# brdav/refign

Hardware: AMD Instinct MI355X
Metric: image-pairs/s (align+seg fwd+bwd, 1080x1920) (higher is better)
Workload: dtype bf16

## Files before the change

include/refign_hip.h:

```cpp
#ifndef REFIGN_HIP_H
#define REFIGN_HIP_H

#ifdef __cplusplus
extern "C" {
#endif

#define RFN_OK 0
#define RFN_EINVAL (-1)
#define RFN_ELAUNCH (-2)
#define RFN_ENOTSUP (-3)
#define RFN_ENONDET (-4)

#define RFN_ABI_VERSION 4

typedef void* rfn_stream_t;

int rfn_abi_version(void);
const char* rfn_last_error(void);

int rfn_set_deterministic(int on);
int rfn_get_deterministic(void);

int rfn_corr_fwd_f32(const float* in1, const float* in2, float* out, int B, int C, int iH, int iW,
                     int kH, int kW, int patchH, int patchW, int padH, int padW, int dilH, int dilW,
// ... 7 lines not shown
                     rfn_stream_t stream);
int rfn_corr_bwd_f64(const double* in1, const double* in2, const double* grad_out, double* grad_in1,
                     double* grad_in2, int B, int C, int iH, int iW, int kH, int kW, int patchH, int patchW,
                     int padH, int padW, int dilH, int dilW, int dpH, int dpW, int dH, int dW,
                     rfn_stream_t stream);

int rfn_corr_fwd_f16(const void* in1, const void* in2, void* out, int B, int C, int iH, int iW,
                     int kH, int kW, int patchH, int patchW, int padH, int padW, int dilH, int dilW,
                     int dpH, int dpW, int dH, int dW, rfn_stream_t stream);
int rfn_corr_bwd_f16(const void* in1, const void* in2, const void* grad_out, void* grad_in1,
                     void* grad_in2, int B, int C, int iH, int iW, int kH, int kW, int patchH, int patchW,
                     int padH, int padW, int dilH, int dilW, int dpH, int dpW, int dH, int dW,
                     rfn_stream_t stream);

int rfn_local_corr_layer_f32(const float* feature_target, const float* feature_source, const float* flow,
                             float* out, int B, int C, int H, int W, rfn_stream_t stream);

long rfn_local_corr_layer_split_workspace_bytes(int B, int H, int W, int splits);
int rfn_local_corr_layer_split_f32(const float* feature_target, const float* feature_source, float* out,
                                   float* workspace, int B, int C, int H, int W, int splits, rfn_stream_t stream);

int rfn_global_corr_layer_f32(const float* feature_source, const float* feature_target, float* out,
                              float* workspace, int B, int C, int Hs, int Ws, int Ht, int Wt,
                              int cyclic_consistency, rfn_stream_t stream);

int rfn_warp_f32(const float* x, const float* flow, float* out, unsigned char* mask, int B, int C, int H,
                 int W, rfn_stream_t stream);
int rfn_warp_bwd_f32(const float* x, const float* flow, const float* grad_out, float* grad_x, float* grad_flow, int B,
                     int C, int H, int W, rfn_stream_t stream);

int rfn_area_resize_f32(const float* x, float* out, int planes, int H, int W, int OH, int OW, rfn_stream_t stream);

int rfn_l2norm_channels_f32(const float* x, float* out, int B, int C, int HW, rfn_stream_t stream);

int rfn_l2norm_channels_nhwc16_f32(const void* x, float* out, int B, int C, int HW, int dtype, rfn_stream_t stream);
int rfn_maxpool2x2_nhwc16(const void* x, void* y, int B, int H, int W, int C, int dtype, rfn_stream_t stream);
int rfn_retile_copy(const void* src, void* dst, int B, int h, int w, int k, int units16, int src_stride16, int backward,
                    rfn_stream_t stream);

unsigned long rfn_refine_workspace_bytes(int B);
int rfn_refine_f32(const float* logits_trg, const float* logits_ref, const unsigned char* warp_mask,
                   const float* certs, float* out, void* workspace, int B, int C, int H, int W, float gamma,
                   int flags, rfn_stream_t stream);

int rfn_label_majority(const long* gt, long* out, int B, int H, int W, int scale, int n_classes, int ignore_index,
                       float min_ratio, rfn_stream_t stream);

int rfn_align_tail_f32(const float* logits_ref, const float* flow_q, const float* logvar_q, float* warped,
                       unsigned char* mask, float* cert, float* flow_up, int B, int C, int H, int W, int h,
                       int w, rfn_stream_t stream);

int rfn_dwconv3x3_nhwc_fwd(const void* x, const float* weight, const float* bias, void* y, int B, int H, int W,
                           int C, int dilation, int dtype, int flip, rfn_stream_t stream);
int rfn_dwconv3x3_nhwc_fwd_stats(const void* x, const float* weight, const float* bias, void* y, double* sums, int B, int H,
                                 int W, int C, int dilation, int dtype, rfn_stream_t stream);
int rfn_dwconv3x3_nhwc_stats(const void* x, const float* weight, const float* bias, double* sums, int B, int H, int W, int C,
                             int dilation, int dtype, rfn_stream_t stream);
int rfn_dwconv3x3_bn_act_nhwc_fwd(const void* x, const float* weight, const float* bias, const float* gamma, const float* beta,
                                  const double* sums, float* running_mean, float* running_var, void* y, int B, int H, int W,
                                  int C, int dilation, float eps, float momentum, int relu, int dtype, rfn_stream_t stream);

int rfn_dwconv3x3_tri_usable(int B, int H, int W, int C, int g);
int rfn_dwconv3x3_tri_stats(const void* x, const float* weight3, const float* bias3, double* sums3, int B, int H, int W, int C, int g,
                            rfn_stream_t stream);
int rfn_dwconv3x3_tri_bn_act_fwd(const void* x, const float* weight3, const float* bias3, const float* const* gamma3,
                                 const float* const* beta3, const double* sums3, float* const* running_mean3,
                                 float* const* running_var3, void* const* y3, int B, int H, int W, int C, int g, const float* eps3,
                                 const float* momentum3, int relu, rfn_stream_t stream);
int rfn_dwconv3x3_tri_stats_f16(const void* x, const float* weight3, const float* bias3, double* sums3, int B, int H, int W, int C,
                                int g, rfn_stream_t stream);
int rfn_dwconv3x3_tri_bn_act_fwd_f16(const void* x, const float* weight3, const float* bias3, const float* const* gamma3,
                                     const float* const* beta3, const double* sums3, float* const* running_mean3,
                                     float* const* running_var3, void* const* y3, int B, int H, int W, int C, int g, const float* eps3,
                                     const float* momentum3, int relu, rfn_stream_t stream);
int rfn_dwconv3x3_gelu_nhwc_fwd(const void* x, const float* weight, const float* bias, void* y_pre, void* y_act, int B,
                                int H, int W, int C, int dtype, rfn_stream_t stream);
unsigned long rfn_dwconv3x3_bwd_weight_workspace_bytes(int C);
int rfn_dwconv3x3_nhwc_bwd_weight(const void* x, const void* grad_y, float* grad_weight, float* grad_bias,
                                  void* workspace, int B, int H, int W, int C, int dilation, int dtype, int flags,
                                  rfn_stream_t stream);
int rfn_dwconv3x3_nhwc_bwd(const void* x, const void* grad_y, const float* weight_tap_major, void* grad_x, float* grad_weight,
                           float* grad_bias, void* workspace, int B, int H, int W, int C, int dilation, int dtype, int flags,
                           rfn_stream_t stream);

int rfn_layernorm_fwd(const void* x, const float* gamma, const float* beta, void* y, float* mean, float* rstd,
                      long rows, int C, float eps, int in_dtype, int out_dtype, rfn_stream_t stream);
unsigned long rfn_layernorm_bwd_workspace_bytes(int C);
int rfn_layernorm_bwd(const void* x, const void* grad_y, const float* gamma, const float* mean, const float* rstd,
                      void* grad_x, float* grad_gamma, float* grad_beta, void* workspace, long rows, int C,
                      int x_dtype, int gy_dtype, int accumulate, rfn_stream_t stream);
int rfn_layernorm_bwd_add(const void* x, const void* grad_y, const void* add, const float* gamma, const float* mean,
                          const float* rstd, void* grad_x, float* grad_gamma, float* grad_beta, void* workspace, long rows, int C,
                          int x_dtype, int gy_dtype, int accumulate, rfn_stream_t stream);
int rfn_layernorm_bwd_add2(const void* x, const void* grad_y, const void* grad_y2, const void* add, const float* gamma,
                           const float* mean, const float* rstd, void* grad_x, float* grad_gamma, float* grad_beta, void* workspace,
                           long rows, int C, int x_dtype, int gy_dtype, int accumulate, rfn_stream_t stream);

int rfn_uncertainty9_weights_len(void);
int rfn_uncertainty9_frontend_f32(const float* corr, const float* weights, float* out, int B, int H, int W,
                                  rfn_stream_t stream);
int rfn_uncertainty9_frontend_f16mm(const float* corr, const float* weights, float* out, int B, int H, int W,
                                    rfn_stream_t stream);

unsigned long rfn_sum_rows_workspace_bytes(long S, long n);
int rfn_sum_rows(const void* x, float* out, void* workspace, long S, long n, int x_dtype, int accumulate,
                 rfn_stream_t stream);
int rfn_linear_param_grads(const void* grad_y, float* grad_bias, void* workspace, long T, long N, int acc_bias,
                           const void* w_partials, float* grad_weight, int S, long NK, int acc_weight, int dtype,
                           rfn_stream_t stream);

int rfn_multi_cast_chunk_elems(void);
int rfn_multi_permute_chunk_elems(void);
int rfn_multi_permute_cast_f32(const void* table, int nchunks, rfn_stream_t stream);
int rfn_multi_cast_f32_bf16(const void* table, int nchunks, rfn_stream_t stream);
int rfn_multi_cast_f32_f16(const void* table, int nchunks, rfn_stream_t stream);
int rfn_multi_ema_f32(const void* table, int nchunks, float momentum, rfn_stream_t stream);
int rfn_multi_transpose_cast_f32_bf16(const void* table, int ntiles, rfn_stream_t stream);
int rfn_multi_transpose_cast_f32_f16(const void* table, int ntiles, rfn_stream_t stream);
int rfn_multi_transpose_tile(void);
int rfn_multi_adamw_f32(const void* table, int nchunks, const float* group_args, int ngroups, rfn_stream_t stream);
int rfn_amp_unscale_f32(float* grads, long n, const float* scale, float* found_inf, rfn_stream_t stream);
int rfn_multi_adamw_amp_f32(const void* table, int nchunks, const double* group_args, int ngroups, const float* found_inf,
                            const float* step, rfn_stream_t stream);
int rfn_amp_update_scale(float* scale, int* growth_tracker, const float* found_inf, float* step, float growth_factor,
                         float backoff_factor, int growth_interval, rfn_stream_t stream);

int rfn_upsample_concat_nhwc(const void* src0, const void* src1, const void* src2, const void* src3, const int* hs,
                             const int* ws, const int* cs, int nlev, void* out, int n, int H, int W, int dtype,
                             rfn_stream_t stream);
int rfn_upsample_concat_nhwc_bwd(const void* grad_out, void* grad0, void* grad1, void* grad2, void* grad3, const int* hs,
                                 const int* ws, const int* cs, int nlev, int n, int H, int W, int dtype,
                                 rfn_stream_t stream);

int rfn_patchify_tokens(const void* src, void* dst, int B, int H, int W, int C, int r, int dtype, int inverse,
                        rfn_stream_t stream);

int rfn_patchify_tokens_cmajor(const void* src, void* dst, int B, int H, int W, int C, int r, int dtype, int inverse,
                               rfn_stream_t stream);

int rfn_gemm_nt(const void* X, const void* W, const void* bias, const void* res, const float* rowscale,
                int rows_per_sample, int act, void* Y, long M, long N, long K, long ldx, long ldw, long ldy, int dtype,
                rfn_stream_t stream);
int rfn_conv2d_nhwc(const void* X, const void* W, const void* bias, const void* res, int act, void* Y, int B, int H,
                    int Wd, int C, int N, int KH, int KW, int stride, int pad, int dil, long ldw, long ldy, int dtype,
                    rfn_stream_t stream);
int rfn_gemm_tn(const void* G, const void* X, float* P, long T, long N, long K, long ldg, long ldx, int rows_per_slab,
                int accumulate, float* grad_bias, const float* rowscale, int rows_per_sample, int dtype,
                rfn_stream_t stream);
int rfn_gemm_tn_grouped(int count, const void* const* G, const void* const* X, float* const* P, float* const* grad_bias,
                        const float* const* rowscale, const long* T, const long* N, const long* K, const long* ldg,
                        const long* ldx, const int* rows_per_slab, const int* rows_per_sample, int dtype, rfn_stream_t stream);

int rfn_attn_pack(const void* src, long batch_stride, long row_stride, int B, int heads, int nrows, int nblk, void* rpack,
                  void* tpack, const void* src2, void* rpack2, void* tpack2, rfn_stream_t stream);
int rfn_attn_fwd(const void* Q, long q_batch_stride, long q_row_stride, const void* k_rpack, const void* v_tpack, void* O,
                 long o_batch_stride, long o_row_stride, float* lse2, int B, int heads, int Nq, int Nkv, int nkblk,
                 int nqpad, float scale, int kv_pack_heads, int dtype, rfn_stream_t stream);
int rfn_attn_bwd_dq(const void* Q, long q_batch_stride, long q_row_stride, const void* dO, const void* O,
                    long o_batch_stride, long o_row_stride, const void* k_rpack, const void* v_rpack, const void* k_tpack,
                    const float* lse2, float* delta, void* dQ, long dq_batch_stride, long dq_row_stride, int B, int heads,
                    int Nq, int Nkv, int nkblk, int nqpad, float scale, int kv_pack_heads, int dtype,
                    rfn_stream_t stream);
int rfn_attn_bwd_dkv(const void* K, const void* V, long kv_batch_stride, long kv_row_stride, const void* q_rpack,
                     const void* q_tpack, const void* do_rpack, const void* do_tpack, const float* lse2,
                     const float* delta, float* accT, void* dKV, int B, int heads, int Nq, int Nkv, int nqblk, int nqpad,
                     int nkpad, int blocks_per_chunk, float scale, int dtype, rfn_stream_t stream);

int rfn_attn32_fwd(const float* Q, long q_batch_stride, long q_row_stride, const float* KV, long kv_batch_stride,
                   long kv_row_stride, float* O, long o_batch_stride, long o_row_stride, float* lse2, int B, int heads,
                   int head_dim, int Nq, int Nkv, int nqpad, float scale, rfn_stream_t stream);
int rfn_attn32_bwd(const float* Q, long q_batch_stride, long q_row_stride, const float* KV, long kv_batch_stride,
                   long kv_row_stride, const float* dO, const float* O, long o_batch_stride, long o_row_stride,
                   const float* lse2, float* delta, float* dQ, long dq_batch_stride, long dq_row_stride, float* dKV,
                   long dkv_batch_stride, long dkv_row_stride, int B, int heads, int head_dim, int Nq, int Nkv, int nqpad,
                   int query_chunks, float scale, rfn_stream_t stream);

int rfn_split3_bf16(const float* x, long x_row_stride, void* out, long out_row_stride, long term_stride, long rows, int K,
                    int Kp, int order, rfn_stream_t stream);
int rfn_split3_cat_bf16(const float* const* parts, const long* strides, const int* channels, int nparts, void* out, int B, int H,
                        int W, int Cp, rfn_stream_t stream);

int rfn_ffn_fc1_dw_gelu_bf16(const void* x, const void* w1, const void* b1, const float* wdw_tap, const float* bdw, void* a,
                             int views, int H, int W, int C, int HID, rfn_stream_t stream);
int rfn_ffn_fc1_dw_gelu_f16(const void* x, const void* w1, const void* b1, const float* wdw_tap, const float* bdw, void* a,
                            int views, int H, int W, int C, int HID, rfn_stream_t stream);

int rfn_bn_stats_fwd(const void* x, double* sums, long T, int C, int dtype, rfn_stream_t stream);
int rfn_bn_apply_fwd(const void* x, const float* gamma, const float* beta, void* y, const double* sums, float* running_mean,
                     float* running_var, long T, int C, float eps, float momentum, int relu, int dtype, rfn_stream_t stream);
int rfn_bn_apply_fwd_ld(const void* x, const float* gamma, const float* beta, void* y, long ld_y, const double* sums,
                        float* running_mean, float* running_var, long T, int C, float eps, float momentum, int relu, int dtype,
                        rfn_stream_t stream);
int rfn_bn_stats_bwd(const void* x, const void* grad_y, const double* fwd_sums, const float* gamma, const float* beta,
                     float* bwd_sums, long T, int C, float eps, int relu, int dtype, rfn_stream_t stream);
int rfn_bn_apply_bwd(const void* x, const void* grad_y, const double* fwd_sums, const float* bwd_sums, const float* gamma,
                     const float* beta, void* grad_x, long T, int C, float eps, int relu, int dtype, rfn_stream_t stream);
int rfn_bn_train_fwd(const void* x, const float* gamma, const float* beta, void* y, double* sums, float* running_mean,
                     float* running_var, long T, int C, float eps, float momentum, int relu, int dtype,
                     rfn_stream_t stream);
int rfn_bn_train_bwd(const void* x, const void* grad_y, const double* fwd_sums, const float* gamma, const float* beta,
                     void* grad_x, float* bwd_sums, long T, int C, float eps, int relu, int dtype, rfn_stream_t stream);

int rfn_upsample_ce(const void* logits, const long* target, const float* weight, float* grad_lo, double* loss_sum, int B,
                    int C, int h, int w, int H, int W, int ignore_index, int dtype, int round16, rfn_stream_t stream);

int rfn_slide_argmax_confmat(const void* crop_logits, int dtype, int B, int C, int h, int w, const int* boxes, int nbox, int H,
                             int W, const long* target, int ignore_index, unsigned char* labels, long* confmat,
                             rfn_stream_t stream);

int rfn_gemm_nt_o32(const void* X, const void* W, const float* bias, const float* res, const float* rowscale,
                    int rows_per_sample, int act, float* Y, long M, long N, long K, long ldx, long ldw, long ldy,
                    rfn_stream_t stream);
int rfn_conv2d_nhwc_o32(const void* X, const void* W, const float* bias, int act, float* Y, int B, int H, int Wd, int C, int N,
                        int KH, int KW, int stride, int pad, int dil, long ldw, long ldy, int transposed,
                        rfn_stream_t stream);
int rfn_conv2d_nhwc_dgrad(const void* GY, const void* Wt, void* DX, int B, int H, int W, int C, int N, int KH, int KW,
                          int stride, int pad, int dil, long ldw, long ldy, int dtype, rfn_stream_t stream);
int rfn_conv2d_nhwc_wgrad(const void* GY, const void* X, float* P, float* grad_bias, int B, int H, int W, int C, int N, int KH,
                          int KW, int stride, int pad, int dil, long ldg, long Kpad, int rows_per_slab, int accumulate,
                          int dtype, rfn_stream_t stream);

int rfn_dacs_mix_jitter(const float* src, const float* trg, const long* gt_src, const long* pseudo_label,
                        const float* pseudo_weight, float* mixed_img, long* mixed_lbl, float* mixed_weight, double* mean_ws,
                        int B, int H, int W, const long* class_bits, const int* jitter_on, const int* order,
                        const float* factor, const float* hue, const float* mean3, const float* std3,
                        rfn_stream_t stream);
int rfn_dacs_blur(const float* x, float* tmp, float* y, int B, int C, int H, int W, int ksize_y, int ksize_x, const int* blur_on,
                  const double* sigma_y, const double* sigma_x, rfn_stream_t stream);

int rfn_crop_label_hist_u8(const void* label, int H, int W, const int* boxes, int K, int* hist, rfn_stream_t stream);
int rfn_crop_flip_norm_u8(const void* image, const void* label, int C, int H, int W, int top, int left, int h, int w, int flip,
                          const float* mean3, const float* std3, float* out_image, long* out_label, rfn_stream_t stream);

int rfn_resize_crop_flip_norm_u8(const void* image_hwc, int H, int W, int Hd, int Wd, const int* bounds_x, const int* coef_x, int kmax_x,
                                 const int* bounds_y, const int* coef_y, int kmax_y, int top, int left, int h, int w, int flip,
                                 const float* mean3, const float* std3, float* out_image, rfn_stream_t stream);
int rfn_resize_u8(const void* image_hwc, int H, int W, int Hd, int Wd, const int* bounds_x, const int* coef_x, int kmax_x,
                  const int* bounds_y, const int* coef_y, int kmax_y, void* out_chw, rfn_stream_t stream);
int rfn_resize_nearest_u8(const void* label, int H, int W, int Hd, int Wd, const int* ytab, const int* xtab, void* out,
                          rfn_stream_t stream);

int rfn_resize_filter_u8(const void* image_hwc, int H, int W, int Hd, int Wd, int filter, const int* bounds_x, const int* coef_x,
                         int kmax_x, const int* bounds_y, const int* coef_y, int kmax_y, void* out_chw, rfn_stream_t stream);
int rfn_resize_filter_crop_flip_norm_pad_u8(const void* image_hwc, int H, int W, int Hd, int Wd, int filter, const int* bounds_x,
                                            const int* coef_x, int kmax_x, const int* bounds_y, const int* coef_y, int kmax_y, int top,
                                            int left, int h, int w, int flip, const float* mean3, const float* std3, float* out_image,
                                            int Hf, int Wf, rfn_stream_t stream);

int rfn_sparse_epe_f32(const float* flow, const float* conf, const float* pts_src, const float* pts_trg, const int* offsets, int B,
// ... 69 lines not shown
```

refign_amd/csrc/attn.hip:

```cpp
#include <cstdlib>

#include "common.h"
#include "mfma.h"

namespace rfn {

constexpr int kPackBlock = 4096;
constexpr float kLog2e = 1.4426950408889634f;

__global__ __launch_bounds__(256) void attn_pack_kernel(const uint16_t* __restrict__ src0, const uint16_t* __restrict__ src1,
                                                        long sb, long sr, int heads, int nrows, int nblk,
                                                        unsigned char* __restrict__ rpack0, unsigned char* __restrict__ tpack0,
                                                        unsigned char* __restrict__ rpack1, unsigned char* __restrict__ tpack1) {
  __shared__ unsigned tile[32][33];
  const uint16_t* src = blockIdx.z ? src1 : src0;
  unsigned char* rpack = blockIdx.z ? rpack1 : rpack0;
  unsigned char* tpack = blockIdx.z ? tpack1 : tpack0;
  const int blk = blockIdx.x, bh = blockIdx.y;
  const int b = bh / heads, hd = bh % heads;
  const int t = threadIdx.x, row = t >> 3, dc = t & 7;
  const int grow = blk * 32 + row;
  u32x4 v = {0u, 0u, 0u, 0u};
  if (grow < nrows) v = *(const u32x4*)(src + (long)b * sb + (long)grow * sr + hd * 64 + dc * 8);
  unsigned char* rb = rpack + ((long)bh * nblk + blk) * kPackBlock;
  if (rpack != nullptr) *(u32x4*)(rb + (dc * 32 + row) * 16) = v;
  if (tpack == nullptr) return;
  tile[row][dc * 4 + 0] = v[0];
  tile[row][dc * 4 + 1] = v[1];
  tile[row][dc * 4 + 2] = v[2];
  tile[row][dc * 4 + 3] = v[3];
  __syncthreads();
  const int rq = t >> 5, dp = t & 31;
  unsigned r0 = tile[4 * rq + 0][dp], r1 = tile[4 * rq + 1][dp], r2 = tile[4 * rq + 2][dp], r3 = tile[4 * rq + 3][dp];
  u32x4 o;
  o[0] = (r0 & 0xffffu) | (r1 << 16);
  o[1] = (r2 & 0xffffu) | (r3 << 16);
  o[2] = (r0 >> 16) | (r1 & 0xffff0000u);
  o[3] = (r2 >> 16) | (r3 & 0xffff0000u);
  unsigned char* tb = tpack + ((long)bh * nblk + blk) * kPackBlock;
  *(u32x4*)(tb + (rq * 64 + 2 * dp) * 8) = o;
}

template <int DT>
__device__ __forceinline__ void load_row_frags(const uint16_t* base, long row_stride, int row, int nrows, int g,
                                               typename Elem<DT>::vec8 (&f)[4]) {
  const bool ok = row < nrows;
  const uint16_t* p = base + (long)(ok ? row : 0) * row_stride + 8 * g;
#pragma unroll
  for (int ks = 0; ks < 4; ++ks) {
    u32x4 v = {0u, 0u, 0u, 0u};
    if (ok) v = *(const u32x4*)(p + 16 * ks);
    f[ks] = __builtin_bit_cast(typename Elem<DT>::vec8, v);
  }
}

template <int DT>
__device__ __forceinline__ void store_rows64(const f32x16 (&acc)[2], float mul, uint16_t* rowptr, bool ok, int g) {
#pragma unroll
  for (int db = 0; db < 2; ++db) {
    u32x2 pk[4];
#pragma unroll
    for (int k = 0; k < 4; ++k)
      pk[k] = pack4<DT>(acc[db][4 * k] * mul, acc[db][4 * k + 1] * mul, acc[db][4 * k + 2] * mul, acc[db][4 * k + 3] * mul);
#pragma unroll
    for (int p = 0; p < 2; ++p) {
      auto r0 = __builtin_amdgcn_permlane32_swap(pk[2 * p][0], pk[2 * p + 1][0], false, false);
      auto r1 = __builtin_amdgcn_permlane32_swap(pk[2 * p][1], pk[2 * p + 1][1], false, false);
      if (ok) {
        u32x4 o = {r0[0], r1[0], r0[1], r1[1]};
        *(u32x4*)(rowptr + db * 32 + 16 * p + 8 * g) = o;
      }
    }
  }
}

template <int DT>
__device__ __forceinline__ void to_operands(const float (&p)[16], typename Elem<DT>::vec8 (&b)[2]) {
#pragma unroll
  for (int m = 0; m < 2; ++m)
    b[m] = join8<DT>(pack4<DT>(p[8 * m], p[8 * m + 1], p[8 * m + 2], p[8 * m + 3]),
                     pack4<DT>(p[8 * m + 4], p[8 * m + 5], p[8 * m + 6], p[8 * m + 7]));
}

template <int DT>
__global__ __launch_bounds__(256) void attn_fwd_kernel(const uint16_t* __restrict__ Q, long qsb, long qsr,
                                                       const unsigned char* __restrict__ Kr,
                                                       const unsigned char* __restrict__ Vt, uint16_t* __restrict__ O,
                                                       long osb, long osr, float* __restrict__ lse2, int heads, int Nq,
                                                       int Nkv, int nblk, int nqpad, float scale, int pheads) {
  using E = Elem<DT>;
  using vec8 = typename E::vec8;
  constexpr int STAGE = 4 * kPackBlock;
  __shared__ __attribute__((aligned(16))) unsigned char smem[2 * STAGE];
  const int lane = threadIdx.x & 63, wave = threadIdx.x >> 6, g = lane >> 5, col = lane & 31;
  const int bh = blockIdx.y, b = bh / heads, hd = bh % heads;
  const int q = blockIdx.x * 128 + wave * 32 + col;
  const float c = scale * kLog2e;
// ... 346 lines not shown
        return join8<DT>(*(const u32x2*)(pq + (4 * m + g) * 512), *(const u32x2*)(pq + (4 * m + 2 + g) * 512));
      };
#pragma unroll
      for (int idx = 0; idx < 4; ++idx) tf[idx] = tfrag(idx);
      __builtin_amdgcn_sched_barrier(0);
      float p[16], ds[16];
#pragma unroll
      for (int r = 0; r < 16; ++r) {
        float pr = __builtin_amdgcn_exp2f(__builtin_fmaf(s[r], c, -l4[r >> 2][r & 3]));
        if (!kok) pr = 0.f;
        p[r] = pr;
        ds[r] = pr * (dp[r] - d4[r >> 2][r & 3]);
      }
      vec8 pb[2], sb[2];
      to_operands<DT>(p, pb);
      to_operands<DT>(ds, sb);
#pragma unroll
      for (int idx = 0; idx < 8; ++idx) {
        const int m = idx >> 2, db = (idx >> 1) & 1;
        if (idx & 1) dk[db] = E::mma(tf[idx & 3], sb[m], dk[db]);
        else dv[db] = E::mma(tf[idx & 3], pb[m], dv[db]);
        if (idx + 4 < 8) tf[idx & 3] = tfrag(idx + 4);
        __builtin_amdgcn_sched_barrier(0);
      }
    }
  }
  if (kok) {
    float* ak = accT + (long)blockIdx.y * chunk_stride + (long)bh * 2 * 64 * nkpad + key;
    float* av = ak + (long)64 * nkpad;
#pragma unroll
    for (int db = 0; db < 2; ++db)
#pragma unroll
      for (int r = 0; r < 16; ++r) {
        const int d = db * 32 + (r & 3) + 8 * (r >> 2) + 4 * g;
        if (chunk_stride != 0) {
          ak[(long)d * nkpad] = dk[db][r] * scale;
          av[(long)d * nkpad] = dv[db][r];
        } else {
          atomicAdd(ak + (long)d * nkpad, dk[db][r] * scale);
          atomicAdd(av + (long)d * nkpad, dv[db][r]);
        }
      }
  }
}

template <int DT>
__global__ __launch_bounds__(256) void attn_dkv_finish_kernel(const float* __restrict__ accT, uint16_t* __restrict__ dkv,
                                                              int heads, int Nkv, int nkpad, long total, int chunks = 1,
                                                              long chunk_stride = 0) {
  using S = typename Elem<DT>::scalar;
  const long i = (long)blockIdx.x * 256 + threadIdx.x;
  if (i >= total) return;
  const int d = (int)(i & 63);
  long r = i >> 6;
  const int hd = (int)(r % heads);
  r /= heads;
  const int which = (int)(r & 1);
  r >>= 1;
  const int key = (int)(r % Nkv);
  const int b = (int)(r / Nkv);
  const float* p = accT + (((long)(b * heads + hd) * 2 + which) * 64 + d) * nkpad + key;
  float v = p[0];
  for (int c = 1; c < chunks; ++c) v += p[(long)c * chunk_stride];
  const S o = (S)v;
  dkv[i] = __builtin_bit_cast(uint16_t, o);
}

}

extern "C" {

using namespace rfn;

#define ATTN_DT_OK(dt) RFN_REQUIRE((dt) == 1 || (dt) == 2, "attention: dtype %d (1 = bf16, 2 = f16)", (dt))

int rfn_attn_pack(const void* src, long batch_stride, long row_stride, int B, int heads, int nrows, int nblk, void* rpack,
                  void* tpack, const void* src2, void* rpack2, void* tpack2, rfn_stream_t stream) {
  RFN_REQUIRE(src && (rpack || tpack), "attn_pack: null pointer");
  RFN_REQUIRE(src2 == nullptr || rpack2 || tpack2, "attn_pack: second tensor without outputs");
  RFN_REQUIRE(B > 0 && heads > 0 && nrows > 0 && nblk * 32 >= nrows, "attn_pack: B=%d heads=%d rows=%d nblk=%d", B, heads,
              nrows, nblk);
  RFN_REQUIRE(row_stride % 8 == 0 && batch_stride % 8 == 0, "attn_pack: strides must be multiples of 8 elements");
  dim3 grid(nblk, B * heads, src2 ? 2 : 1);
  hipLaunchKernelGGL(attn_pack_kernel, grid, dim3(256), 0, (hipStream_t)stream, (const uint16_t*)src,
                     (const uint16_t*)src2, batch_stride, row_stride, heads, nrows, nblk, (unsigned char*)rpack,
                     (unsigned char*)tpack, (unsigned char*)rpack2, (unsigned char*)tpack2);
  return check_launch("attn_pack");
}

int rfn_attn_fwd(const void* Q, long q_batch_stride, long q_row_stride, const void* k_rpack, const void* v_tpack, void* O,
                 long o_batch_stride, long o_row_stride, float* lse2, int B, int heads, int Nq, int Nkv, int nkblk,
                 int nqpad, float scale, int kv_pack_heads, int dtype, rfn_stream_t stream) {
  ATTN_DT_OK(dtype);
  RFN_REQUIRE(Q && k_rpack && v_tpack && O && lse2, "attn_fwd: null pointer");
  RFN_REQUIRE(B > 0 && heads > 0 && Nq > 0 && Nkv > 0 && nkblk % 2 == 0 && nkblk * 32 >= Nkv && nqpad >= Nq,
              "attn_fwd: B=%d heads=%d Nq=%d Nkv=%d nkblk=%d nqpad=%d", B, heads, Nq, Nkv, nkblk, nqpad);
  RFN_REQUIRE(q_row_stride % 8 == 0 && o_row_stride % 8 == 0 && q_batch_stride % 8 == 0 && o_batch_stride % 8 == 0,
              "attn_fwd: strides must be multiples of 8 elements");
  RFN_REQUIRE(kv_pack_heads >= heads, "attn_fwd: kv_pack_heads");
  dim3 grid(cdiv(Nq, 128), B * heads);
  if (dtype == 1)
    hipLaunchKernelGGL(attn_fwd_kernel<1>, grid, dim3(256), 0, (hipStream_t)stream, (const uint16_t*)Q, q_batch_stride,
                       q_row_stride, (const unsigned char*)k_rpack, (const unsigned char*)v_tpack, (uint16_t*)O,
                       o_batch_stride, o_row_stride, lse2, heads, Nq, Nkv, nkblk, nqpad, scale, kv_pack_heads);
  else
    hipLaunchKernelGGL(attn_fwd_kernel<2>, grid, dim3(256), 0, (hipStream_t)stream, (const uint16_t*)Q, q_batch_stride,
                       q_row_stride, (const unsigned char*)k_rpack, (const unsigned char*)v_tpack, (uint16_t*)O,
                       o_batch_stride, o_row_stride, lse2, heads, Nq, Nkv, nkblk, nqpad, scale, kv_pack_heads);
  return check_launch("attn_fwd");
}

int rfn_attn_bwd_dq(const void* Q, long q_batch_stride, long q_row_stride, const void* dO, const void* O,
                    long o_batch_stride, long o_row_stride, const void* k_rpack, const void* v_rpack, const void* k_tpack,
                    const float* lse2, float* delta, void* dQ, long dq_batch_stride, long dq_row_stride, int B, int heads,
                    int Nq, int Nkv, int nkblk, int nqpad, float scale, int kv_pack_heads, int dtype,
                    rfn_stream_t stream) {
  ATTN_DT_OK(dtype);
  RFN_REQUIRE(Q && dO && O && k_rpack && v_rpack && k_tpack && lse2 && delta && dQ, "attn_bwd_dq: null pointer");
  RFN_REQUIRE(B > 0 && heads > 0 && Nq > 0 && Nkv > 0 && nkblk % 2 == 0 && nkblk * 32 >= Nkv && nqpad >= Nq,
              "attn_bwd_dq: B=%d heads=%d Nq=%d Nkv=%d nkblk=%d nqpad=%d", B, heads, Nq, Nkv, nkblk, nqpad);
  dim3 grid(cdiv(Nq, 128), B * heads);
#define RFN_DQ_LAUNCH(D)                                                                                                \
  hipLaunchKernelGGL(attn_bwd_dq_kernel<D>, grid, dim3(256), 0, (hipStream_t)stream, (const uint16_t*)Q, q_batch_stride, \
                     q_row_stride, (const uint16_t*)dO, (const uint16_t*)O, o_batch_stride, o_row_stride,               \
                     (const unsigned char*)k_rpack, (const unsigned char*)v_rpack, (const unsigned char*)k_tpack, lse2,  \
                     delta, (uint16_t*)dQ, dq_batch_stride, dq_row_stride, heads, Nq, Nkv, nkblk, nqpad, scale,          \
                     kv_pack_heads)
  if (dtype == 1) RFN_DQ_LAUNCH(1); else RFN_DQ_LAUNCH(2);
#undef RFN_DQ_LAUNCH
  return check_launch("attn_bwd_dq");
}

static int attn_bwd_dkv_impl(bool det, const void* K, const void* V, long kv_batch_stride, long kv_row_stride, const void* q_rpack,
                             const void* q_tpack, const void* do_rpack, const void* do_tpack, const float* lse2,
                             const float* delta, float* accT, void* dKV, int B, int heads, int Nq, int Nkv, int nqblk, int nqpad,
                             int nkpad, int blocks_per_chunk, float scale, int dtype, rfn_stream_t stream) {
  ATTN_DT_OK(dtype);
  RFN_REQUIRE(K && V && q_rpack && q_tpack && do_rpack && do_tpack && lse2 && delta && accT && dKV,
              "attn_bwd_dkv: null pointer");
  RFN_REQUIRE(B > 0 && heads > 0 && Nq > 0 && Nkv > 0 && nqblk * 32 >= Nq && nqpad >= nqblk * 32 && nkpad >= Nkv &&
                  nkpad % 32 == 0 && blocks_per_chunk > 0,
              "attn_bwd_dkv: B=%d heads=%d Nq=%d Nkv=%d nqblk=%d nqpad=%d nkpad=%d chunk=%d", B, heads, Nq, Nkv, nqblk,
              nqpad, nkpad, blocks_per_chunk);
  hipStream_t s = (hipStream_t)stream;
  const long image = (long)B * heads * 2 * 64 * nkpad, chunk_stride = det ? image : 0;
  if (!det)
    if (int rc = zero_async(accT, (size_t)image * sizeof(float), s)) return rc;
  dim3 grid(cdiv(Nkv, 256), cdiv(nqblk, blocks_per_chunk), B * heads);
  const int chunks = det ? (int)grid.y : 1;
  static const int ring = 2;
#define RFN_DKV_LAUNCH_(D, R)                                                                                           \
  hipLaunchKernelGGL((attn_bwd_dkv_kernel<D, R>), grid, dim3(512), 0, s, (const uint16_t*)K, (const uint16_t*)V,            \
                     kv_batch_stride, kv_row_stride, (const unsigned char*)q_rpack, (const unsigned char*)q_tpack,      \
                     (const unsigned char*)do_rpack, (const unsigned char*)do_tpack, lse2, delta, accT, heads, Nq, Nkv,  \
                     nqblk, nqpad, nkpad, blocks_per_chunk, scale, chunk_stride)
#define RFN_DKV_LAUNCH(D)                                                                                               \
  switch (ring) {                                                                                                       \
    case 4: RFN_DKV_LAUNCH_(D, 4); break;                                                                               \
    default: RFN_DKV_LAUNCH_(D, 2); break;                                                                              \
  }
  if (dtype == 1) { RFN_DKV_LAUNCH(1) } else { RFN_DKV_LAUNCH(2) }
#undef RFN_DKV_LAUNCH
#undef RFN_DKV_LAUNCH_
  int rc = check_launch("attn_bwd_dkv");
  if (rc != RFN_OK) return rc;
  const long total = (long)B * Nkv * 2 * heads * 64;
  if (dtype == 1)
    hipLaunchKernelGGL(attn_dkv_finish_kernel<1>, dim3(cdiv(total, 256)), dim3(256), 0, s, accT, (uint16_t*)dKV, heads,
                       Nkv, nkpad, total, chunks, chunk_stride);
  else
    hipLaunchKernelGGL(attn_dkv_finish_kernel<2>, dim3(cdiv(total, 256)), dim3(256), 0, s, accT, (uint16_t*)dKV, heads,
                       Nkv, nkpad, total, chunks, chunk_stride);
  return check_launch("attn_dkv_finish");
}

int rfn_attn_bwd_dkv(const void* K, const void* V, long kv_batch_stride, long kv_row_stride, const void* q_rpack,
                     const void* q_tpack, const void* do_rpack, const void* do_tpack, const float* lse2,
                     const float* delta, float* accT, void* dKV, int B, int heads, int Nq, int Nkv, int nqblk, int nqpad,
                     int nkpad, int blocks_per_chunk, float scale, int dtype, rfn_stream_t stream) {
  RFN_REFUSE_NONDET(true, "rfn_attn_bwd_dkv", "attn_bwd_dkv_kernel, fp32 atomics (use rfn_attn_bwd_dkv_det)");
  return attn_bwd_dkv_impl(false, K, V, kv_batch_stride, kv_row_stride, q_rpack, q_tpack, do_rpack, do_tpack, lse2, delta, accT,
                           dKV, B, heads, Nq, Nkv, nqblk, nqpad, nkpad, blocks_per_chunk, scale, dtype, stream);
}

int rfn_attn_bwd_dkv_det(const void* K, const void* V, long kv_batch_stride, long kv_row_stride, const void* q_rpack,
                         const void* q_tpack, const void* do_rpack, const void* do_tpack, const float* lse2,
                         const float* delta, float* accT, void* dKV, int B, int heads, int Nq, int Nkv, int nqblk, int nqpad,
                         int nkpad, int blocks_per_chunk, float scale, int dtype, rfn_stream_t stream) {
  return attn_bwd_dkv_impl(true, K, V, kv_batch_stride, kv_row_stride, q_rpack, q_tpack, do_rpack, do_tpack, lse2, delta, accT,
                           dKV, B, heads, Nq, Nkv, nqblk, nqpad, nkpad, blocks_per_chunk, scale, dtype, stream);
}

}
```

refign_amd/csrc/dwconv.hip:

```cpp
#include <hip/hip_bf16.h>

#include <type_traits>

#include "common.h"
#include "mfma.h"

namespace rfn {

template <typename T>
struct VecIO;

template <>
struct VecIO<float> {
  static constexpr int N = 4;
  typedef float4 Raw;
  __device__ static Raw load_raw(const float* p) { return *reinterpret_cast<const float4*>(p); }
  __device__ static void unpack(const Raw& t, float (&v)[4]) { v[0] = t.x; v[1] = t.y; v[2] = t.z; v[3] = t.w; }
  typedef float Pair __attribute__((ext_vector_type(2)));
  __device__ static void unpack2(const Raw& t, Pair (&v)[2]) { v[0] = Pair{t.x, t.y}; v[1] = Pair{t.z, t.w}; }
  __device__ static void load(const float* p, float (&v)[4]) {
    const float4 t = *reinterpret_cast<const float4*>(p);
    v[0] = t.x; v[1] = t.y; v[2] = t.z; v[3] = t.w;
  }
  __device__ static void store(float* p, const float (&v)[4]) {
    *reinterpret_cast<float4*>(p) = make_float4(v[0], v[1], v[2], v[3]);
  }
  __device__ static float rnd(float v) { return v; }
};

template <>
struct VecIO<__hip_bfloat16> {
  static constexpr int N = 8;
  typedef uint4 Raw;
  __device__ static Raw load_raw(const __hip_bfloat16* p) { return *reinterpret_cast<const uint4*>(p); }
  __device__ static void unpack(const Raw& t, float (&v)[8]) {
    const unsigned w[4] = {t.x, t.y, t.z, t.w};
#pragma unroll
    for (int i = 0; i < 4; ++i) {
      v[2 * i] = __uint_as_float(w[i] << 16);
      v[2 * i + 1] = __uint_as_float(w[i] & 0xffff0000u);
    }
  }
  typedef float Pair __attribute__((ext_vector_type(2)));
  __device__ static void unpack2(const Raw& t, Pair (&v)[4]) {
    const unsigned w[4] = {t.x, t.y, t.z, t.w};
#pragma unroll
    for (int i = 0; i < 4; ++i) v[i] = Pair{__uint_as_float(w[i] << 16), __uint_as_float(w[i] & 0xffff0000u)};
  }
  __device__ static void load(const __hip_bfloat16* p, float (&v)[8]) {
    const uint4 t = *reinterpret_cast<const uint4*>(p);
    const unsigned w[4] = {t.x, t.y, t.z, t.w};
#pragma unroll
    for (int i = 0; i < 4; ++i) {
      v[2 * i] = __uint_as_float(w[i] << 16);
      v[2 * i + 1] = __uint_as_float(w[i] & 0xffff0000u);
    }
  }
  __device__ static unsigned pack(float lo, float hi) { return bf16x2_bits(lo, hi); }
  __device__ static void store(__hip_bfloat16* p, const float (&v)[8]) {
    uint4 t;
    t.x = pack(v[0], v[1]); t.y = pack(v[2], v[3]); t.z = pack(v[4], v[5]); t.w = pack(v[6], v[7]);
    *reinterpret_cast<uint4*>(p) = t;
  }
  __device__ static float rnd(float v) { return __uint_as_float(bf16_bits(v) << 16); }
};

template <>
struct VecIO<_Float16> {
  static constexpr int N = 8;
  typedef uint4 Raw;
  __device__ static Raw load_raw(const _Float16* p) { return *reinterpret_cast<const uint4*>(p); }
  __device__ static void unpack(const Raw& t, float (&v)[8]) {
    const unsigned w[4] = {t.x, t.y, t.z, t.w};
#pragma unroll
    for (int i = 0; i < 4; ++i) {
      v[2 * i] = f16_lo(w[i]);
      v[2 * i + 1] = f16_hi(w[i]);
    }
  }
  typedef float Pair __attribute__((ext_vector_type(2)));
  __device__ static void unpack2(const Raw& t, Pair (&v)[4]) {
    const unsigned w[4] = {t.x, t.y, t.z, t.w};
#pragma unroll
    for (int i = 0; i < 4; ++i) v[i] = Pair{f16_lo(w[i]), f16_hi(w[i])};
  }
  __device__ static void load(const _Float16* p, float (&v)[8]) { unpack(load_raw(p), v); }
// ... 497 lines not shown
      for (int p = 0; p < kPX; ++p)
        xraw[p] = mask_raw(IO::load_raw(xp + (size_t)min(w0 + p * dil, W - 1) * C), w0 + p * dil < W);
#pragma unroll
      for (int p = 0; p < kPX; ++p) IO::unpack2(xraw[p], xv[p]);
    }
    f32x2 acc[GX ? kPX : 1][V2];
    if constexpr (GX) {
#pragma unroll
      for (int p = 0; p < kPX; ++p)
#pragma unroll
        for (int i = 0; i < V2; ++i) acc[p][i] = f32x2{0.0f, 0.0f};
    }
#pragma unroll
    for (int ky = 0; ky < 3; ++ky) {
      const int yy = h + (ky - 1) * dil;
      const bool rowok = yy >= 0 && yy < H;
      const T* gr = gy + img + (size_t)min(max(yy, 0), H - 1) * W * C;
      typename IO::Raw raw[kPX + 2];
#pragma unroll
      for (int j = 0; j < kPX + 2; ++j) {
        const int xx = w0 + (j - 1) * dil;
        raw[j] = mask_raw(IO::load_raw(gr + (size_t)min(max(xx, 0), W - 1) * C), rowok && xx >= 0 && xx < W);
      }
#pragma unroll
      for (int j = 0; j < kPX + 2; ++j) {
        f32x2 v[V2];
        IO::unpack2(raw[j], v);
        if (ky == 1 && j >= 1 && j <= kPX) {
#pragma unroll
          for (int i = 0; i < V2; ++i) ab[i] += v[i];
        }
#pragma unroll
        for (int kx = 0; kx < 3; ++kx) {
          const int p = j - kx;
          if (p < 0 || p >= kPX) continue;
#pragma unroll
          for (int i = 0; i < V2; ++i) {
            if constexpr (GX) acc[p][i] = __builtin_elementwise_fma(wr[ky * 3 + kx][i], v[i], acc[p][i]);
            aw[ky * 3 + kx][i] = __builtin_elementwise_fma(xv[p][i], v[i], aw[ky * 3 + kx][i]);
          }
        }
      }
    }
    if constexpr (GX) {
      T* gp = gx + img + (size_t)h * W * C;
#pragma unroll
      for (int p = 0; p < kPX; ++p)
        if (w0 + p * dil < W) {
          float o[V];
#pragma unroll
          for (int i = 0; i < V2; ++i) { o[2 * i] = acc[p][i].x; o[2 * i + 1] = acc[p][i].y; }
          IO::store(gp + (size_t)(w0 + p * dil) * C, o);
        }
    }
  }
  __shared__ float red[5][256][V];
  float* wrow = ws + (size_t)wsrow * 10 * C;
  for (int pass = 0; pass < 2; ++pass) {
    __syncthreads();
#pragma unroll
    for (int kk = 0; kk < 5; ++kk) {
      const int k = pass * 5 + kk;
#pragma unroll
      for (int i = 0; i < V; ++i) {
        const f32x2 t = (k < 9) ? aw[k < 9 ? 8 - k : 0][i / 2] : ab[i / 2];
        red[kk][threadIdx.x][i] = (i & 1) ? t.y : t.x;
      }
    }
    __syncthreads();
    for (int o = threadIdx.x; o < 5 * cvb * V; o += 256) {
      const int kk = o / (cvb * V), rem = o - kk * cvb * V, cvj = rem / V, i = rem - cvj * V;
      if (cvbase + cvj >= CV) continue;
      float sum = 0.0f;
      for (int p = 0; p < pl; ++p) sum += red[kk][p * cvb + cvj][i];
      wrow[(size_t)(pass * 5 + kk) * C + (cvbase + cvj) * V + i] = sum;
    }
  }
}

__global__ __launch_bounds__(256) void dwconv3x3_bwd_weight_reduce_kernel(const float* __restrict__ ws,
                                                                          float* __restrict__ dw,
                                                                          float* __restrict__ db, int C, int stripes,
                                                                          int flags) {
  __shared__ float part[8][32];
  const int lane = threadIdx.x & 31, seg = threadIdx.x >> 5;
  const int idx = blockIdx.x * 32 + lane;
  float s = 0.0f;
  if (idx < 10 * C) {
#pragma unroll 4
    for (int t = seg; t < stripes; t += 8) s += ws[(size_t)t * 10 * C + idx];
  }
  part[seg][lane] = s;
  __syncthreads();
  if (seg != 0 || idx >= 10 * C) return;
  s = ((part[0][lane] + part[1][lane]) + (part[2][lane] + part[3][lane])) +
      ((part[4][lane] + part[5][lane]) + (part[6][lane] + part[7][lane]));
  float* dst;
  if (idx < 9 * C) {
    const int k = idx / C, c = idx - k * C;
    dst = (flags & 2) ? dw + c * 9 + k : dw + idx;
  } else {
    if (db == nullptr) return;
    dst = db + (idx - 9 * C);
  }
  *dst = (flags & 1) ? *dst + s : s;
}

static inline int pick_cvb(int CV) { return CV >= 64 ? 64 : (CV >= 32 ? 32 : (CV >= 16 ? 16 : 8)); }

struct SlicedGeom {
  bool on;
  int cvb, grid;
};
static inline SlicedGeom sliced_geom(int CV, long nslots) {
  static const int enabled = 1;
  static const int per_xcd = 64;
  if (!enabled || CV % 8 != 0 || CV / 8 < 16 || CV / 8 > 64) return SlicedGeom{false, 0, 0};
  const int cvb = CV / 8, pl = 256 / cvb;
  const int j = (int)std::max<long>(1, std::min<long>(cdiv(nslots, pl), per_xcd));
  return SlicedGeom{true, cvb, 8 * j};
}
constexpr int kMaxStripes = 128;

template <typename T>
static int launch_fwd_gelu(const void* x, const float* w, const float* bias, void* y, void* ya, int B, int H, int W,
                           int C, hipStream_t st, float xs = 1.f, float oq = 1.f) {
  constexpr int V = VecIO<T>::N;
  const int CV = C / V;
  const long nquads = (long)B * H * ((W + kPX - 1) / kPX);
  if (SlicedGeom sg = sliced_geom(CV, nquads); sg.on) {
    hipLaunchKernelGGL((dwconv3x3_fwd_kernel<T, false, true>), dim3(sg.grid), dim3(256), 0, st, (const T*)x, w, bias,
                       (T*)y, B, H, W, C, 1, sg.cvb, (T*)ya, xs, oq, 1);
    return check_launch("dwconv3x3_fwd_kernel<gelu, sliced>");
  }
  const int cvb = pick_cvb(CV), gx = cdiv(CV, cvb), pl = 256 / cvb;
  const int gy = (int)std::max<long>(1, std::min<long>(cdiv(nquads, pl), (256L * 16) / gx));
  hipLaunchKernelGGL((dwconv3x3_fwd_kernel<T, false, true>), dim3(gx, gy), dim3(256), 0, st, (const T*)x, w, bias,
                     (T*)y, B, H, W, C, 1, cvb, (T*)ya, xs, oq);
  return check_launch("dwconv3x3_fwd_kernel<gelu>");
}

struct RollGeom {
  bool sliced;
  int cvb, gx, gy, seg, rows;
  long nitems;
};
static RollGeom roll_geom(int B, int H, int W, int C, int dil) {
  RollGeom g{};
  const int CV = C / kRV, Hd = cdiv(H, dil);
  const int WQ = dil * cdiv(cdiv(W, dil), kPX);
  const SlicedGeom sg = sliced_geom(C / 8, 1L << 30);
  int pl;
  long lanes;
  if (sg.on) {
    g.sliced = true, g.cvb = 2 * sg.cvb, pl = 256 / g.cvb;
    lanes = (long)(sg.grid / 8) * pl;
  } else {
    g.cvb = pick_cvb(CV), g.gx = cdiv(CV, g.cvb), pl = 256 / g.cvb;
    lanes = (256L * 16) / g.gx * pl;
  }
  const long per_seg = (long)B * dil * WQ;
  const long want = std::max<long>(1, cdiv(4 * lanes, per_seg));
  g.seg = (int)std::min<long>(Hd, std::max<long>(8, cdiv(Hd, want)));
  g.nitems = per_seg * cdiv(Hd, g.seg);
  if (sg.on) {
    g.rows = (int)std::max<long>(1, std::min<long>(cdiv(g.nitems, pl), sg.grid / 8));
    g.gx = 8 * g.rows, g.gy = 1;
  } else {
    g.rows = g.gy = (int)std::max<long>(1, std::min<long>(cdiv(g.nitems, pl), (256L * 16) / g.gx));
  }
  return g;
}

template <typename T, int STATS, bool BNE>
static int launch_roll(const void* x, const float* w, const float* bias, void* y, double* sums, int B, int H, int W, int C,
                       int dil, hipStream_t st, BnEpi bn, double* spart) {
  static void* zero_line = nullptr;
  if (zero_line == nullptr && hipGetSymbolAddress(&zero_line, HIP_SYMBOL(g_zero_line_dw)) != hipSuccess)
    return fail(RFN_ELAUNCH, "dwconv3x3_roll_kernel: zero line symbol");
  const RollGeom g = roll_geom(B, H, W, C, dil);
  RFN_REQUIRE(g.nitems < (1L << 30) && (long)dil * W * C * (long)sizeof(T) < (1L << 32),
              "dwconv3x3_roll_kernel: B=%d H=%d W=%d C=%d dilation=%d too large", B, H, W, C, dil);
  hipLaunchKernelGGL((dwconv3x3_roll_kernel<T, STATS, BNE, kRollDepth<T>>), dim3(g.gx, g.gy), dim3(256), 0, st, (const T*)x, w, bias, (T*)y, B, H,
                     W, C, dil, g.cvb, g.seg, g.sliced ? 1 : 0, sums, bn, spart, (const void*)zero_line);
  if (int rc = check_launch("dwconv3x3_roll_kernel")) return rc;
  if (spart != nullptr) return ordered_colsum_f64(spart, sums, g.rows, 2 * C, st);
  return RFN_OK;
}

template <typename T, int STATS, bool BNE>
static int launch_fwd_stats(const void* x, const float* w, const float* bias, void* y, double* sums, int B, int H, int W, int C,
                            int dil, hipStream_t st, BnEpi bn = BnEpi{}, double* spart = nullptr) {
  if constexpr (STATS == 2 || BNE) {
    return launch_roll<T, STATS, BNE>(x, w, bias, y, sums, B, H, W, C, dil, st, bn, spart);
  } else {
    constexpr int V = VecIO<T>::N;
    const int CV = C / V;
    const int WQ = dil * (((W + dil - 1) / dil + kPX - 1) / kPX);
    int rows;
    if (SlicedGeom sg = sliced_geom(CV, (long)B * dil * ((H + dil - 1) / dil) * WQ); sg.on) {
      hipLaunchKernelGGL((dwconv3x3_fwd_kernel<T, false, false, STATS>), dim3(sg.grid), dim3(256), 0, st, (const T*)x, w, bias,
                         (T*)y, B, H, W, C, dil, sg.cvb, (T*)nullptr, 1.f, 1.f, 1, sums, spart);
      if (int rc = check_launch("dwconv3x3_fwd_kernel<sliced, stats>")) return rc;
      rows = sg.grid / 8;
    } else {
      const int cvb = pick_cvb(CV), gx = cdiv(CV, cvb), pl = 256 / cvb;
      const long nquads = (long)B * H * WQ;
      const int gy = (int)std::max<long>(1, std::min<long>(cdiv(nquads, pl), (256L * 16) / gx));
      hipLaunchKernelGGL((dwconv3x3_fwd_kernel<T, false, false, STATS>), dim3(gx, gy), dim3(256), 0, st, (const T*)x, w, bias,
                         (T*)y, B, H, W, C, dil, cvb, (T*)nullptr, 1.f, 1.f, 0, sums, spart);
      if (int rc = check_launch("dwconv3x3_fwd_kernel<stats>")) return rc;
      rows = gy;
    }
    if (spart != nullptr) return ordered_colsum_f64(spart, sums, rows, 2 * C, st);
    return RFN_OK;
  }
}

static int dw_stats_rows(int B, int H, int W, int C, int dil) {
  const int CV = C / 8;
  const int WQ = dil * (((W + dil - 1) / dil + kPX - 1) / kPX);
  const int roll = roll_geom(B, H, W, C, dil).rows;
  if (SlicedGeom sg = sliced_geom(CV, (long)B * dil * ((H + dil - 1) / dil) * WQ); sg.on) return std::max(roll, sg.grid / 8);
  const int cvb = pick_cvb(CV), gx = cdiv(CV, cvb), pl = 256 / cvb;
  return std::max(roll, (int)std::max<long>(1, std::min<long>(cdiv((long)B * H * WQ, pl), (256L * 16) / gx)));
}

template <typename T>
static int launch_fwd(const void* x, const float* w, const float* bias, void* y, int B, int H, int W, int C, int dil,
                      int flip, hipStream_t st) {
  constexpr int V = VecIO<T>::N;
  const int CV = C / V;
  const int WQ = dil * (((W + dil - 1) / dil + kPX - 1) / kPX);
  if (SlicedGeom sg = sliced_geom(CV, (long)B * dil * ((H + dil - 1) / dil) * WQ); sg.on) {
    if (flip)
      hipLaunchKernelGGL((dwconv3x3_fwd_kernel<T, true>), dim3(sg.grid), dim3(256), 0, st, (const T*)x, w, bias, (T*)y, B,
                         H, W, C, dil, sg.cvb, (T*)nullptr, 1.f, 1.f, 1);
    else
      hipLaunchKernelGGL((dwconv3x3_fwd_kernel<T, false>), dim3(sg.grid), dim3(256), 0, st, (const T*)x, w, bias, (T*)y,
                         B, H, W, C, dil, sg.cvb, (T*)nullptr, 1.f, 1.f, 1);
    return check_launch("dwconv3x3_fwd_kernel<sliced>");
  }
  const int cvb = pick_cvb(CV), gx = cdiv(CV, cvb), pl = 256 / cvb;
  const long nquads = (long)B * H * WQ;
  const int gy = (int)std::max<long>(1, std::min<long>(cdiv(nquads, pl), (256L * 16) / gx));
  if (flip)
    hipLaunchKernelGGL((dwconv3x3_fwd_kernel<T, true>), dim3(gx, gy), dim3(256), 0, st, (const T*)x, w, bias, (T*)y, B,
                       H, W, C, dil, cvb);
  else
    hipLaunchKernelGGL((dwconv3x3_fwd_kernel<T, false>), dim3(gx, gy), dim3(256), 0, st, (const T*)x, w, bias, (T*)y,
                       B, H, W, C, dil, cvb);
  return check_launch("dwconv3x3_fwd_kernel");
}

template <typename T>
static int launch_bwd(const void* x, const void* gy, const float* w, void* gx, float* dw, float* db, float* ws, int B, int H,
                      int W, int C, int dil, int flags, hipStream_t st) {
  constexpr int V = BwdIO<T>::N, V16 = 16 / (int)sizeof(T);
  const int CV = C / V;
  const int WQ = dil * (((W + dil - 1) / dil + kPX - 1) / kPX);
  int rows;
  if (SlicedGeom sg = sliced_geom(C / V16, 1L << 30); sg.on) {
    const int cvb = sg.cvb * (V16 / V), pl = 256 / cvb;
    rows = (int)std::max<long>(1, std::min<long>(cdiv((long)B * dil * ((H + dil - 1) / dil) * WQ, pl), sg.grid / 8));
    if (gx != nullptr)
      hipLaunchKernelGGL((dwconv3x3_bwd_kernel<T, true>), dim3(8 * rows), dim3(256), 0, st, (const T*)x, (const T*)gy, w, (T*)gx,
                         ws, B, H, W, C, dil, cvb, 1);
    else
      hipLaunchKernelGGL((dwconv3x3_bwd_kernel<T, false>), dim3(8 * rows), dim3(256), 0, st, (const T*)x, (const T*)gy, w,
                         (T*)nullptr, ws, B, H, W, C, dil, cvb, 1);
  } else {
    int cvb = pick_cvb(CV);
    while (cvb > 8 && cdiv(CV, cvb) < 4) cvb >>= 1;
    const int gxb = cdiv(CV, cvb), pl = 256 / cvb;
    const long nquads = (long)B * H * WQ;
    rows = (int)std::max<long>(1, std::min<long>(std::min<long>(kMaxStripes, cdiv(nquads, pl)), std::max<long>(1, (256L * 8) / gxb)));
    if (gx != nullptr)
      hipLaunchKernelGGL((dwconv3x3_bwd_kernel<T, true>), dim3(gxb, rows), dim3(256), 0, st, (const T*)x, (const T*)gy, w,
                         (T*)gx, ws, B, H, W, C, dil, cvb, 0);
    else
      hipLaunchKernelGGL((dwconv3x3_bwd_kernel<T, false>), dim3(gxb, rows), dim3(256), 0, st, (const T*)x, (const T*)gy, w,
                         (T*)nullptr, ws, B, H, W, C, dil, cvb, 0);
  }
  if (int rc = check_launch("dwconv3x3_bwd_kernel")) return rc;
  hipLaunchKernelGGL(dwconv3x3_bwd_weight_reduce_kernel, dim3(cdiv(10L * C, 32)), dim3(256), 0, st, ws, dw, db, C, rows, flags);
  return check_launch("dwconv3x3_bwd_weight_reduce_kernel");
}


constexpr int kTriPitch = 80, kTriMaxPix = 944, kTriScratch = 4 * 4 * 16 * 4;

struct TriArgs {
  const float* w;
  const float* bias;
  double* sums;
  const float* gamma[3];
  const float* beta[3];
  float* running_mean[3];
  float* running_var[3];
  float eps[3], momentum[3];
  void* y[3];
  int relu, ablate;
};

template <int M, int MODE, typename T>
__device__ __forceinline__ void tri_branch(const unsigned char* __restrict__ img, float* __restrict__ scratch, const TriArgs& a,
                                           int b, int B, int H, int W, int C, int g, int py, int px, int Hs, int Ws, int c0, int cv,
                                           int pl, bool first_block, bool stat_block) {
  typedef float f2 __attribute__((ext_vector_type(2)));
  constexpr int k = M - 1;
  const int c = c0 + cv * 8;
  f2 wr[9][4], bs[4];
#pragma unroll
  for (int t = 0; t < 9; ++t) {
    const float* wp = a.w + ((size_t)k * 9 + t) * C + c;
    const float4 lo = *reinterpret_cast<const float4*>(wp), hi = *reinterpret_cast<const float4*>(wp + 4);
    wr[t][0] = f2{lo.x, lo.y}; wr[t][1] = f2{lo.z, lo.w}; wr[t][2] = f2{hi.x, hi.y}; wr[t][3] = f2{hi.z, hi.w};
  }
#pragma unroll
  for (int i = 0; i < 4; ++i)
    bs[i] = a.bias != nullptr ? f2{a.bias[(size_t)k * C + c + 2 * i], a.bias[(size_t)k * C + c + 2 * i + 1]} : f2{0.f, 0.f};
  float bsc[8], bsh[8], st0[8], st1[8];
  if constexpr (MODE == 1) {
    const double* sm = a.sums + (size_t)k * (2 * C + 1);
    const double cnt = sm[2 * C], inv = 1.0 / cnt;
#pragma unroll
    for (int i = 0; i < 8; ++i) {
      const double m = sm[c + i] * inv;
      const float var = (float)fmax(sm[C + c + i] * inv - m * m, 0.0), mean = (float)m;
      const float ga = a.gamma[k] != nullptr ? a.gamma[k][c + i] : 1.f, be = a.beta[k] != nullptr ? a.beta[k][c + i] : 0.f;
      bsc[i] = rsqrtf(var + a.eps[k]) * ga;
      bsh[i] = be - mean * bsc[i];
      if (stat_block && pl == 0 && a.running_mean[k] != nullptr) {
        const float n = (float)cnt;
        a.running_mean[k][c + i] = (1.f - a.momentum[k]) * a.running_mean[k][c + i] + a.momentum[k] * mean;
        a.running_var[k][c + i] = (1.f - a.momentum[k]) * a.running_var[k][c + i] + a.momentum[k] * var * (n / fmaxf(n - 1.f, 1.f));
      }
    }
  } else {
#pragma unroll
    for (int i = 0; i < 8; ++i) st0[i] = st1[i] = 0.f;
  }
  const int QW = (Ws + 3) >> 2, nq = Hs * QW;
  for (int q = pl; q < nq; q += 64) {
    const int ys = q / QW, x0 = 4 * (q - ys * QW);
    f2 acc[4][4];
#pragma unroll
    for (int p = 0; p < 4; ++p)
#pragma unroll
      for (int i = 0; i < 4; ++i) acc[p][i] = bs[i];
#pragma unroll
    for (int ky = 0; ky < 3; ++ky) {
      const int yy = ys + (ky - 1) * M;
      const bool rowok = yy >= 0 && yy < Hs;
      const unsigned char* rowp = img + (size_t)min(max(yy, 0), Hs - 1) * Ws * kTriPitch + cv * 16;
#pragma unroll
      for (int o = 0; o < 4 + 2 * M; ++o) {
        const int xx = x0 - M + o;
        uint4 raw = *reinterpret_cast<const uint4*>(rowp + min(max(xx, 0), Ws - 1) * kTriPitch);
        if (!(rowok && xx >= 0 && xx < Ws)) raw = make_uint4(0u, 0u, 0u, 0u);
        f2 v[4];
        VecIO<T>::unpack2(raw, v);
#pragma unroll
        for (int p = 0; p < 4; ++p) {
          const int d = o - p;
          if (d != 0 && d != M && d != 2 * M) continue;
          const int kx = d / M;
#pragma unroll
// ... 190 lines not shown
  return dtype == 1 ? launch_fwd_stats<__hip_bfloat16, 1, false>(x, weight, bias, y, sums, B, H, W, C, dilation, st)
                    : launch_fwd_stats<_Float16, 1, false>(x, weight, bias, y, sums, B, H, W, C, dilation, st);
}

unsigned long rfn_dwconv3x3_stats_det_workspace_bytes(int B, int H, int W, int C, int dilation) {
  if (B <= 0 || H <= 0 || W <= 0 || C <= 0 || C % 8 != 0 || dilation <= 0) return 0;
  return (unsigned long)dw_stats_rows(B, H, W, C, dilation) * 2 * C * sizeof(double);
}

int rfn_dwconv3x3_nhwc_fwd_stats_det(const void* x, const float* weight, const float* bias, void* y, double* sums, void* workspace,
                                     int B, int H, int W, int C, int dilation, int dtype, rfn_stream_t stream) {
  RFN_REQUIRE(x && weight && y && sums && workspace, "rfn_dwconv3x3_nhwc_fwd_stats_det: null pointer");
  RFN_REQUIRE(B > 0 && H > 0 && W > 0 && C > 0 && dilation > 0, "rfn_dwconv3x3_nhwc_fwd_stats_det: bad size");
  RFN_REQUIRE((dtype == 1 || dtype == 2) && C % 8 == 0, "rfn_dwconv3x3_nhwc_fwd_stats_det: bf16 / f16 (dtype 1 / 2), C %% 8 == 0");
  hipStream_t st = (hipStream_t)stream;
  return dtype == 1 ? launch_fwd_stats<__hip_bfloat16, 1, false>(x, weight, bias, y, sums, B, H, W, C, dilation, st, BnEpi{}, (double*)workspace)
                    : launch_fwd_stats<_Float16, 1, false>(x, weight, bias, y, sums, B, H, W, C, dilation, st, BnEpi{}, (double*)workspace);
}

int rfn_dwconv3x3_nhwc_stats_det(const void* x, const float* weight, const float* bias, double* sums, void* workspace, int B, int H,
                                 int W, int C, int dilation, int dtype, rfn_stream_t stream) {
  RFN_REQUIRE(x && weight && sums && workspace, "rfn_dwconv3x3_nhwc_stats_det: null pointer");
  RFN_REQUIRE(B > 0 && H > 0 && W > 0 && C > 0 && dilation > 0, "rfn_dwconv3x3_nhwc_stats_det: bad size");
  RFN_REQUIRE((dtype == 1 || dtype == 2) && C % 8 == 0, "rfn_dwconv3x3_nhwc_stats_det: bf16 / f16 (dtype 1 / 2), C %% 8 == 0");
  hipStream_t st = (hipStream_t)stream;
  return dtype == 1 ? launch_fwd_stats<__hip_bfloat16, 2, false>(x, weight, bias, nullptr, sums, B, H, W, C, dilation, st, BnEpi{}, (double*)workspace)
                    : launch_fwd_stats<_Float16, 2, false>(x, weight, bias, nullptr, sums, B, H, W, C, dilation, st, BnEpi{}, (double*)workspace);
}

int rfn_dwconv3x3_nhwc_stats(const void* x, const float* weight, const float* bias, double* sums, int B, int H, int W, int C,
                             int dilation, int dtype, rfn_stream_t stream) {
  RFN_REQUIRE(x && weight && sums, "rfn_dwconv3x3_nhwc_stats: null pointer");
  RFN_REQUIRE(B > 0 && H > 0 && W > 0 && C > 0 && dilation > 0, "rfn_dwconv3x3_nhwc_stats: bad size");
  RFN_REQUIRE((dtype == 1 || dtype == 2) && C % 8 == 0, "rfn_dwconv3x3_nhwc_stats: bf16 / f16 (dtype 1 / 2), C %% 8 == 0");
  RFN_REFUSE_NONDET(true, "rfn_dwconv3x3_nhwc_stats", "dwconv3x3_roll_kernel<stats>, fp64 atomics (use rfn_dwconv3x3_nhwc_stats_det)");
  hipStream_t st = (hipStream_t)stream;
  if (int rc = zero_async(sums, (2 * (size_t)C + 1) * sizeof(double), st)) return rc;
  return dtype == 1 ? launch_fwd_stats<__hip_bfloat16, 2, false>(x, weight, bias, nullptr, sums, B, H, W, C, dilation, st)
                    : launch_fwd_stats<_Float16, 2, false>(x, weight, bias, nullptr, sums, B, H, W, C, dilation, st);
}

int rfn_dwconv3x3_bn_act_nhwc_fwd(const void* x, const float* weight, const float* bias, const float* gamma, const float* beta,
                                  const double* sums, float* running_mean, float* running_var, void* y, int B, int H, int W,
                                  int C, int dilation, float eps, float momentum, int relu, int dtype, rfn_stream_t stream) {
  RFN_REQUIRE(x && weight && sums && y, "rfn_dwconv3x3_bn_act_nhwc_fwd: null pointer");
  RFN_REQUIRE(B > 0 && H > 0 && W > 0 && C > 0 && dilation > 0, "rfn_dwconv3x3_bn_act_nhwc_fwd: bad size");
  RFN_REQUIRE((dtype == 1 || dtype == 2) && C % 8 == 0 && (relu == 0 || relu == 1),
              "rfn_dwconv3x3_bn_act_nhwc_fwd: bf16 / f16, C %% 8 == 0, relu 0 / 1");
  BnEpi bn{gamma, beta, running_mean, running_var, eps, momentum, relu};
  if (dtype == 2)
    return launch_fwd_stats<_Float16, 0, true>(x, weight, bias, y, const_cast<double*>(sums), B, H, W, C, dilation,
                                               (hipStream_t)stream, bn);
  return launch_fwd_stats<__hip_bfloat16, 0, true>(x, weight, bias, y, const_cast<double*>(sums), B, H, W, C, dilation,
                                                   (hipStream_t)stream, bn);
}

int rfn_dwconv3x3_gelu_nhwc_fwd(const void* x, const float* weight, const float* bias, void* y_pre, void* y_act, int B,
                                int H, int W, int C, int dtype, rfn_stream_t stream) {
  RFN_REQUIRE(x && weight && y_act, "rfn_dwconv3x3_gelu_nhwc_fwd: null pointer");
  RFN_REQUIRE(B > 0 && H > 0 && W > 0 && C > 0, "rfn_dwconv3x3_gelu_nhwc_fwd: bad size");
  if (dtype == 0) {
    RFN_REQUIRE(C % 4 == 0, "rfn_dwconv3x3_gelu_nhwc_fwd: C must be a multiple of 4 for f32 (got %d)", C);
    return launch_fwd_gelu<float>(x, weight, bias, y_pre, y_act, B, H, W, C, (hipStream_t)stream);
  }
  RFN_REQUIRE(C % 8 == 0, "rfn_dwconv3x3_gelu_nhwc_fwd: C must be a multiple of 8 for 16-bit activations (got %d)", C);
  return dt_one(dtype, "rfn_dwconv3x3_gelu_nhwc_fwd", [&](auto t) {
    return launch_fwd_gelu<typename decltype(t)::type>(x, weight, bias, y_pre, y_act, B, H, W, C, (hipStream_t)stream);
  });
}

int rfn_dwconv3x3_gelu_nhwc_fwd_f8(const void* x8, const float* weight, const float* bias, void* y8, int B, int H, int W, int C,
                                   float x_scale, float out_q, rfn_stream_t stream) {
  RFN_REQUIRE(x8 && weight && y8, "rfn_dwconv3x3_gelu_nhwc_fwd_f8: null pointer");
  RFN_REQUIRE(B > 0 && H > 0 && W > 0 && C > 0 && C % 8 == 0, "rfn_dwconv3x3_gelu_nhwc_fwd_f8: bad size (C %% 8)");
  return launch_fwd_gelu<f8e4m3>(x8, weight, bias, nullptr, y8, B, H, W, C, (hipStream_t)stream, x_scale, out_q);
}

unsigned long rfn_dwconv3x3_bwd_weight_workspace_bytes(int C) {
  return (unsigned long)kMaxStripes * 10ul * (unsigned long)(C > 0 ? C : 0) * sizeof(float);
}

static int dw_bwd(const char* who, const void* x, const void* grad_y, const float* weight, void* grad_x, float* grad_weight,
                  float* grad_bias, void* workspace, int B, int H, int W, int C, int dilation, int dtype, int flags,
                  hipStream_t st) {
  RFN_REQUIRE(x && grad_y && grad_weight && workspace, "%s: null pointer", who);
  RFN_REQUIRE(B > 0 && H > 0 && W > 0 && C > 0 && dilation > 0, "%s: bad size", who);
  if (dtype == 0) {
    RFN_REQUIRE(C % 4 == 0, "%s: C must be a multiple of 4 for f32", who);
    return launch_bwd<float>(x, grad_y, weight, grad_x, grad_weight, grad_bias, (float*)workspace, B, H, W, C, dilation, flags, st);
  }
  RFN_REQUIRE(C % 8 == 0, "%s: C must be a multiple of 8 for 16-bit activations", who);
  return dt_one(dtype, who, [&](auto t) {
    return launch_bwd<typename decltype(t)::type>(x, grad_y, weight, grad_x, grad_weight, grad_bias, (float*)workspace, B, H, W, C,
                                                  dilation, flags, st);
  });
}

int rfn_dwconv3x3_nhwc_bwd_weight(const void* x, const void* grad_y, float* grad_weight, float* grad_bias,
                                  void* workspace, int B, int H, int W, int C, int dilation, int dtype, int flags,
                                  rfn_stream_t stream) {
  return dw_bwd("rfn_dwconv3x3_nhwc_bwd_weight", x, grad_y, nullptr, nullptr, grad_weight, grad_bias, workspace, B, H, W, C,
                dilation, dtype, flags, (hipStream_t)stream);
}

int rfn_dwconv3x3_nhwc_bwd(const void* x, const void* grad_y, const float* weight_tap_major, void* grad_x, float* grad_weight,
                           float* grad_bias, void* workspace, int B, int H, int W, int C, int dilation, int dtype, int flags,
                           rfn_stream_t stream) {
  RFN_REQUIRE(weight_tap_major && grad_x, "rfn_dwconv3x3_nhwc_bwd: null pointer");
  return dw_bwd("rfn_dwconv3x3_nhwc_bwd", x, grad_y, weight_tap_major, grad_x, grad_weight, grad_bias, workspace, B, H, W, C,
                dilation, dtype, flags, (hipStream_t)stream);
}

}
```

refign_amd/csrc/layernorm.hip:

```cpp
#include <hip/hip_bf16.h>

#include "common.h"
#include "mfma.h"

namespace rfn {

constexpr int kLnMaxPerLane = 16;
constexpr int kLnMaxBlocks = 256;

template <typename T>
__device__ __forceinline__ float ld(const T* p);
template <>
__device__ __forceinline__ float ld<float>(const float* p) { return *p; }
template <>
__device__ __forceinline__ float ld<__hip_bfloat16>(const __hip_bfloat16* p) {
  return __uint_as_float(((unsigned)*reinterpret_cast<const unsigned short*>(p)) << 16);
}
template <>
__device__ __forceinline__ float ld<_Float16>(const _Float16* p) { return (float)*p; }
template <typename T>
__device__ __forceinline__ void st(T* p, float v);
template <>
__device__ __forceinline__ void st<_Float16>(_Float16* p, float v) { *p = (_Float16)v; }
template <>
__device__ __forceinline__ void st<float>(float* p, float v) { *p = v; }
template <>
__device__ __forceinline__ void st<__hip_bfloat16>(__hip_bfloat16* p, float v) {
  *reinterpret_cast<unsigned short*>(p) = (unsigned short)bf16_bits(v);
}

template <>
__device__ __forceinline__ void st<f8e4m3>(f8e4m3* p, float v) { p->v = (unsigned char)(quant4(v, 0.f, 0.f, 0.f) & 0xffu); }

template <typename TI, typename TO, int NPL>
__global__ __launch_bounds__(256) void layernorm_fwd_kernel(const TI* __restrict__ x, const float* __restrict__ gamma,
                                                            const float* __restrict__ beta, TO* __restrict__ y,
                                                            float* __restrict__ mean, float* __restrict__ rstd,
                                                            long rows, int C, float eps) {
  const int lane = threadIdx.x & 63, wave = threadIdx.x >> 6;
  float g[NPL], b[NPL];
#pragma unroll
  for (int i = 0; i < NPL; ++i) {
    const int c = lane + 64 * i;
    g[i] = c < C ? gamma[c] : 0.0f;
    b[i] = c < C ? beta[c] : 0.0f;
  }
  const float invC = 1.0f / (float)C;
  for (long r = (long)blockIdx.x * 4 + wave; r < rows; r += (long)gridDim.x * 4) {
    const TI* xr = x + r * C;
    float v[NPL];
    float s = 0.0f;
#pragma unroll
    for (int i = 0; i < NPL; ++i) {
      const int c = lane + 64 * i;
      v[i] = c < C ? ld<TI>(xr + c) : 0.0f;
      s += v[i];
    }
    const float mu = wave_sum(s) * invC;
    float q = 0.0f;
#pragma unroll
    for (int i = 0; i < NPL; ++i) {
      const int c = lane + 64 * i;
      const float d = c < C ? v[i] - mu : 0.0f;
      q = fmaf(d, d, q);
    }
    const float rs = rsqrtf(wave_sum(q) * invC + eps);
    TO* yr = y + r * C;
#pragma unroll
    for (int i = 0; i < NPL; ++i) {
      const int c = lane + 64 * i;
      if (c < C) st<TO>(yr + c, fmaf((v[i] - mu) * rs, g[i], b[i]));
    }
    if (lane == 0) {
      mean[r] = mu;
      rstd[r] = rs;
    }
  }
}

template <typename TX, typename TG, int NPL>
__global__ __launch_bounds__(256) void layernorm_bwd_kernel(const TX* __restrict__ x, const TG* __restrict__ gy,
                                                            const float* __restrict__ gamma,
                                                            const float* __restrict__ mean,
                                                            const float* __restrict__ rstd, TX* __restrict__ dx,
                                                            float* __restrict__ ws, long rows, int C) {
  const int lane = threadIdx.x & 63, wave = threadIdx.x >> 6;
  float gm[NPL], dg[NPL], db[NPL];
#pragma unroll
  for (int i = 0; i < NPL; ++i) {
    const int c = lane + 64 * i;
    gm[i] = c < C ? gamma[c] : 0.0f;
// ... 180 lines not shown
  }
  const float invC = 1.0f / (float)C;
  for (long r0 = ((long)blockIdx.x * 4 + wave) * RPW; r0 < rows; r0 += (long)gridDim.x * 4 * RPW) {
    const long r = r0 + grp;
    const bool valid = r < rows;
    const float mu = valid ? mean[r] : 0.0f, rs = valid ? rstd[r] : 0.0f;
    float xh[NV][8], gg[NV][8], av[NV][8];
    float s1 = 0.0f, s2 = 0.0f;
#pragma unroll
    for (int j = 0; j < NV; ++j) {
      float xv[8], gv[8];
      if (valid && act[j]) {
        ld8<TX>(x + r * C + (sub + LPR * j) * 8, xv);
        ld8<TG>(gy + r * C + (sub + LPR * j) * 8, gv);
        if (gy2 != nullptr) {
          float g2[8];
          ld8<TG>(gy2 + r * C + (sub + LPR * j) * 8, g2);
#pragma unroll
          for (int i = 0; i < 8; ++i) gv[i] += g2[i];
        }
        if (add != nullptr) ld8<TX>(add + r * C + (sub + LPR * j) * 8, av[j]);
      } else {
#pragma unroll
        for (int i = 0; i < 8; ++i) { xv[i] = mu; gv[i] = 0.0f; }
      }
#pragma unroll
      for (int i = 0; i < 8; ++i) {
        xh[j][i] = (xv[i] - mu) * rs;
        gg[j][i] = gv[i] * gm[j][i];
        s1 += gg[j][i];
        s2 = fmaf(gg[j][i], xh[j][i], s2);
        dg[j][i] = fmaf(gv[i], xh[j][i], dg[j][i]);
        db[j][i] += gv[i];
      }
    }
    s1 = group_sum<LPR>(s1) * invC;
    s2 = group_sum<LPR>(s2) * invC;
#pragma unroll
    for (int j = 0; j < NV; ++j)
      if (valid && act[j]) {
        float o[8];
#pragma unroll
        for (int i = 0; i < 8; ++i) o[i] = rs * (gg[j][i] - s1 - xh[j][i] * s2);
        if (add != nullptr) {
#pragma unroll
          for (int i = 0; i < 8; ++i) o[i] += av[j][i];
        }
        st8<TX>(dx + r * C + (sub + LPR * j) * 8, o);
      }
  }
#pragma unroll
  for (int j = 0; j < NV; ++j)
#pragma unroll
    for (int i = 0; i < 8; ++i) {
#pragma unroll
      for (int o = LPR; o < 64; o <<= 1) {
        dg[j][i] += __shfl_xor(dg[j][i], o, 64);
        db[j][i] += __shfl_xor(db[j][i], o, 64);
      }
    }
  __shared__ float red[4][2][64 * 8 * NV];
  if (grp == 0) {
#pragma unroll
    for (int j = 0; j < NV; ++j)
#pragma unroll
      for (int i = 0; i < 8; ++i) {
        const int c = (sub + LPR * j) * 8 + i;
        red[wave][0][c] = dg[j][i];
        red[wave][1][c] = db[j][i];
      }
  }
  __syncthreads();
  float* row = ws + (size_t)blockIdx.x * 2 * C;
  for (int c = threadIdx.x; c < 2 * C; c += 256) {
    const int which = c / C, cc = c % C;
    row[c] = red[0][which][cc] + red[1][which][cc] + red[2][which][cc] + red[3][which][cc];
  }
}

__global__ __launch_bounds__(256) void layernorm_bwd_reduce_kernel(const float* __restrict__ ws,
                                                                   float* __restrict__ dgamma,
                                                                   float* __restrict__ dbeta, int C, int nblocks,
                                                                   int accumulate) {
  __shared__ float part[4][64];
  const int col = blockIdx.x * 64 + (threadIdx.x & 63), seg = threadIdx.x >> 6;
  float s = 0.0f;
  if (col < 2 * C) {
#pragma unroll 8
    for (int b = seg; b < nblocks; b += 4) s += ws[(size_t)b * 2 * C + col];
  }
  part[seg][threadIdx.x & 63] = s;
  __syncthreads();
  if (seg == 0 && col < 2 * C) {
    const float t = (part[0][threadIdx.x] + part[1][threadIdx.x]) + (part[2][threadIdx.x] + part[3][threadIdx.x]);
    float* dst = col < C ? dgamma + col : dbeta + (col - C);
    *dst = accumulate ? *dst + t : t;
  }
}

static inline int ln_grid(long rows, int cap) { return (int)std::max<long>(1, std::min<long>(cdiv(rows, 4), cap)); }

template <typename TI, typename TO>
static int ln_fwd_dispatch(const void* x, const float* g, const float* b, void* y, float* mean, float* rstd, long rows,
                           int C, float eps, hipStream_t st, float oscale = 1.f) {
  if (C % 8 == 0) {
#define RFN_LN_FWDV(LPR, NV)                                                                                         \
  hipLaunchKernelGGL((layernorm_fwd_vec_kernel<TI, TO, LPR, NV>),                                                    \
                     dim3((int)std::max<long>(1, std::min<long>(cdiv(rows, 4 * (64 / LPR)), 256 * 16))), dim3(256), \
                     0, st, (const TI*)x, g, b, (TO*)y, mean, rstd, rows, C, eps, oscale)
    if (C <= 64) RFN_LN_FWDV(8, 1);
    else if (C <= 128) RFN_LN_FWDV(16, 1);
    else if (C <= 256) RFN_LN_FWDV(32, 1);
    else if (C <= 512) RFN_LN_FWDV(64, 1);
    else RFN_LN_FWDV(64, 2);
#undef RFN_LN_FWDV
    return check_launch("layernorm_fwd_vec_kernel");
  }
  const int grid = ln_grid(rows, 256 * 16), npl = cdiv(C, 64);
#define RFN_LN_FWD(N)                                                                                             \
  hipLaunchKernelGGL((layernorm_fwd_kernel<TI, TO, N>), dim3(grid), dim3(256), 0, st, (const TI*)x, g, b, (TO*)y, \
                     mean, rstd, rows, C, eps)
  if (npl <= 1) RFN_LN_FWD(1);
  else if (npl <= 2) RFN_LN_FWD(2);
  else if (npl <= 4) RFN_LN_FWD(4);
  else if (npl <= 8) RFN_LN_FWD(8);
  else RFN_LN_FWD(16);
#undef RFN_LN_FWD
  return check_launch("layernorm_fwd_kernel");
}

template <typename TX, typename TG>
static int ln_bwd_dispatch(const void* x, const void* gy, const float* g, const float* mean, const float* rstd,
                           void* dx, float* dgamma, float* dbeta, float* ws, long rows, int C, int accumulate,
                           hipStream_t st, const void* add = nullptr, const void* gy2 = nullptr) {
  if ((add != nullptr || gy2 != nullptr) && C % 8 != 0) return fail(RFN_EINVAL, "rfn_layernorm_bwd_add: C %% 8 != 0");
  int grid = ln_grid(rows, kLnMaxBlocks);
  const int npl = cdiv(C, 64);
  if (C % 8 == 0) {
#define RFN_LN_BWDV(LPR, NV)                                                                                        \
  grid = (int)std::max<long>(1, std::min<long>(cdiv(rows, 4 * (64 / LPR)), kLnMaxBlocks));                         \
  hipLaunchKernelGGL((layernorm_bwd_vec_kernel<TX, TG, LPR, NV>), dim3(grid), dim3(256), 0, st, (const TX*)x,      \
                     (const TG*)gy, g, mean, rstd, (TX*)dx, ws, rows, C, (const TX*)add, (const TG*)gy2)
    if (C <= 64) { RFN_LN_BWDV(8, 1); }
    else if (C <= 128) { RFN_LN_BWDV(16, 1); }
    else if (C <= 256) { RFN_LN_BWDV(32, 1); }
    else if (C <= 512) { RFN_LN_BWDV(64, 1); }
    else { RFN_LN_BWDV(64, 2); }
#undef RFN_LN_BWDV
  } else {
#define RFN_LN_BWD(N)                                                                                              \
  hipLaunchKernelGGL((layernorm_bwd_kernel<TX, TG, N>), dim3(grid), dim3(256), 0, st, (const TX*)x, (const TG*)gy, \
                     g, mean, rstd, (TX*)dx, ws, rows, C)
  if (npl <= 1) RFN_LN_BWD(1);
  else if (npl <= 2) RFN_LN_BWD(2);
  else if (npl <= 4) RFN_LN_BWD(4);
  else if (npl <= 8) RFN_LN_BWD(8);
  else RFN_LN_BWD(16);
#undef RFN_LN_BWD
  }
  if (int rc = check_launch("layernorm_bwd_kernel")) return rc;
  hipLaunchKernelGGL(layernorm_bwd_reduce_kernel, dim3(cdiv(2L * C, 64)), dim3(256), 0, st, ws, dgamma, dbeta, C,
                     grid, accumulate);
  return check_launch("layernorm_bwd_reduce_kernel");
}

}

using namespace rfn;

extern "C" {

unsigned long rfn_layernorm_bwd_workspace_bytes(int C) {
  return (unsigned long)kLnMaxBlocks * 2ul * (unsigned long)(C > 0 ? C : 0) * sizeof(float);
}

int rfn_layernorm_fwd(const void* x, const float* gamma, const float* beta, void* y, float* mean, float* rstd,
                      long rows, int C, float eps, int in_dtype, int out_dtype, rfn_stream_t stream) {
  RFN_REQUIRE(x && gamma && beta && y && mean && rstd, "rfn_layernorm_fwd: null pointer");
  RFN_REQUIRE(rows > 0 && C > 0 && C <= 64 * kLnMaxPerLane, "rfn_layernorm_fwd: need 0 < C <= 1024 (got %d)", C);
  hipStream_t st = (hipStream_t)stream;
  return dt_pair(in_dtype, out_dtype, "rfn_layernorm_fwd", [&](auto ti, auto to) {
    return ln_fwd_dispatch<typename decltype(ti)::type, typename decltype(to)::type>(x, gamma, beta, y, mean, rstd, rows, C, eps, st);
  });
}

int rfn_layernorm_bwd_add(const void* x, const void* grad_y, const void* add, const float* gamma, const float* mean,
                          const float* rstd, void* grad_x, float* grad_gamma, float* grad_beta, void* workspace, long rows, int C,
                          int x_dtype, int gy_dtype, int accumulate, rfn_stream_t stream) {
  RFN_REQUIRE(x && grad_y && gamma && mean && rstd && grad_x && grad_gamma && grad_beta && workspace,
              "rfn_layernorm_bwd_add: null pointer");
  RFN_REQUIRE(rows > 0 && C > 0 && C % 8 == 0 && C <= 64 * kLnMaxPerLane, "rfn_layernorm_bwd_add: need C %% 8 == 0, C <= 1024 (got %d)", C);
  hipStream_t st = (hipStream_t)stream;
  float* ws = (float*)workspace;
  return dt_pair(x_dtype, gy_dtype, "rfn_layernorm_bwd_add", [&](auto tx, auto tg) {
    return ln_bwd_dispatch<typename decltype(tx)::type, typename decltype(tg)::type>(x, grad_y, gamma, mean, rstd, grad_x, grad_gamma,
                                                                                      grad_beta, ws, rows, C, accumulate, st, add);
  });
}

int rfn_layernorm_bwd_add2(const void* x, const void* grad_y, const void* grad_y2, const void* add, const float* gamma,
                           const float* mean, const float* rstd, void* grad_x, float* grad_gamma, float* grad_beta, void* workspace,
                           long rows, int C, int x_dtype, int gy_dtype, int accumulate, rfn_stream_t stream) {
  RFN_REQUIRE(x && grad_y && gamma && mean && rstd && grad_x && grad_gamma && grad_beta && workspace,
              "rfn_layernorm_bwd_add2: null pointer");
  RFN_REQUIRE(rows > 0 && C > 0 && C % 8 == 0 && C <= 64 * kLnMaxPerLane, "rfn_layernorm_bwd_add2: need C %% 8 == 0, C <= 1024 (got %d)", C);
  hipStream_t st = (hipStream_t)stream;
  float* ws = (float*)workspace;
  return dt_pair(x_dtype, gy_dtype, "rfn_layernorm_bwd_add2", [&](auto tx, auto tg) {
    return ln_bwd_dispatch<typename decltype(tx)::type, typename decltype(tg)::type>(x, grad_y, gamma, mean, rstd, grad_x, grad_gamma,
                                                                                      grad_beta, ws, rows, C, accumulate, st, add, grad_y2);
  });
}

int rfn_layernorm_fwd_f8(const void* x_bf16, const float* gamma, const float* beta, void* y8, long rows, int C, float eps,
                         float out_q, rfn_stream_t stream) {
  RFN_REQUIRE(x_bf16 && gamma && beta && y8, "rfn_layernorm_fwd_f8: null pointer");
  RFN_REQUIRE(rows > 0 && C > 0 && C % 8 == 0 && C <= 64 * kLnMaxPerLane, "rfn_layernorm_fwd_f8: need C %% 8 == 0, C <= 1024 (got %d)", C);
  return ln_fwd_dispatch<__hip_bfloat16, f8e4m3>(x_bf16, gamma, beta, y8, nullptr, nullptr, rows, C, eps, (hipStream_t)stream,
                                                 out_q);
}

int rfn_layernorm_bwd(const void* x, const void* grad_y, const float* gamma, const float* mean, const float* rstd,
                      void* grad_x, float* grad_gamma, float* grad_beta, void* workspace, long rows, int C,
                      int x_dtype, int gy_dtype, int accumulate, rfn_stream_t stream) {
  RFN_REQUIRE(x && grad_y && gamma && mean && rstd && grad_x && grad_gamma && grad_beta && workspace,
              "rfn_layernorm_bwd: null pointer");
  RFN_REQUIRE(rows > 0 && C > 0 && C <= 64 * kLnMaxPerLane, "rfn_layernorm_bwd: need 0 < C <= 1024 (got %d)", C);
  hipStream_t st = (hipStream_t)stream;
  float* ws = (float*)workspace;
  return dt_pair(x_dtype, gy_dtype, "rfn_layernorm_bwd", [&](auto tx, auto tg) {
    return ln_bwd_dispatch<typename decltype(tx)::type, typename decltype(tg)::type>(x, grad_y, gamma, mean, rstd, grad_x, grad_gamma,
                                                                                      grad_beta, ws, rows, C, accumulate, st);
  });
}

}
```

refign_amd/csrc/mfma_gemm.hip:

```cpp
#include <hip/hip_bf16.h>

#include <algorithm>
#include <cstdio>
#include <cstdlib>
#include <type_traits>

#include "common.h"
#include "mfma.h"

namespace rfn {

template <int I, int N, typename F> __device__ __forceinline__ void static_for(F&& f) {
  if constexpr (I < N) {
    f(std::integral_constant<int, I>{});
    static_for<I + 1, N>(f);
  }
}

struct GemmEpi {
  const uint16_t* bias;
  const uint16_t* res;
  const float* rowscale;
  int rows_per_sample;
  int act;
};

__device__ __forceinline__ float gelu_grad(float z) {
  const float x = fabsf(z) * 0.70710678118654752440f;
  const float t = 1.0f / (1.0f + 0.3275911f * x);
  const float e = __expf(-x * x);
  const float poly = t * (0.254829592f + t * (-0.284496736f + t * (1.421413741f + t * (-1.453152027f + t * 1.061405429f))));
  const float erf_abs = 1.0f - poly * e;
  const float cdf = 0.5f * (1.0f + (z < 0.f ? -erf_abs : erf_abs));
  return cdf + z * 0.3989422804014327f * e;
}

__device__ __forceinline__ float apply_act(float v, int act) {
  if (act == 1) return fmaxf(v, 0.f);
  if (act == 3) return v > 0.f ? v : 0.1f * v;
  return v;
}

int launch_conv3x3_halo(const void* X, const void* W, const void* bias, void* Y, int B, int H, int Wd, int C, int N, long ldw,
                        long ldy, int act, int dtype, int out32, hipStream_t s);

struct ConvGeom {
  int H, W, C, OH, OW, KH, KW, stride, pad, dil;
  int C8;
  unsigned c8_magic;
  unsigned kw_magic;
  const void* zero;
  int transposed, sshift;
};


template <int DT, int BM, int BN, int BK, int NS, bool GATHER, int NW = 4, bool OUT32 = false>
__global__ __launch_bounds__(NW * 64) void gemm_nt_kernel(const uint16_t* __restrict__ X, const uint16_t* __restrict__ W,
                                                      uint16_t* __restrict__ Y, int M, int N, int K, long ldx, long ldw,
                                                      long ldy, int tiles_n, int total_tiles, GemmEpi epi, ConvGeom cg) {
  using E = Elem<DT>;
  using vec8 = typename E::vec8;
  static_assert(BK == 32 || BK == 64, "K-step of 32 or 64");
  static_assert(NW == 4 || NW == 8, "4 or 8 waves");
  constexpr int WNW = NW / 2;
  constexpr int IB = BN / (32 * WNW);
  constexpr int JB = BM / 64;
  constexpr int ROWB = BK * 2;
  constexpr int PPR = BK / 8;
  constexpr int RPI = 64 / PPR;
  constexpr int XBYTES = BM * ROWB, WBYTES = BN * ROWB, STAGE = XBYTES + WBYTES;
  constexpr int XI = BM / (NW * RPI), WI = BN / (NW * RPI);
  constexpr int IPS = XI + WI;
  auto swizzle = [](int r) { return BK == 64 ? (r >> 1) & 7 : (r >> 2) & 3; };
  __shared__ __attribute__((aligned(16))) unsigned char smem[NS * STAGE];

  const int lane = threadIdx.x & 63, wave = threadIdx.x >> 6;
  const int wm = wave / WNW, wn = wave % WNW;
  const int G = gridDim.x;
  const int wg = xcd_remap(blockIdx.x, G);
  const int t_begin = wg;
  if (t_begin >= total_tiles) return;
  const int ntiles = (total_tiles - wg + G - 1) / G;
  const int nk = K / BK;

  const int drow = lane / PPR;
  const int dpiece = (lane % PPR) ^ swizzle(RPI * wave + drow);
  const unsigned char* xsrc[XI];
  const unsigned char* wsrc[WI];
  int iy0[GATHER ? XI : 1], ix0[GATHER ? XI : 1];
// ... 394 lines not shown
#pragma unroll
    for (int u = 0; u < GPT; ++u) {
      const int item = u * 256 + threadIdx.x, q = item / GP, cp = item % GP;
      const u32x4 o = transpose4(greg[u]);
      *(u32x4*)(gs + (q * BN + 2 * cp) * 8) = o;
      if (do_bias) {
        float f[4];
        unpack4<DT>(u32x2{o[0], o[1]}, f);
        bsum[0] += (f[0] + f[1]) + (f[2] + f[3]);
        unpack4<DT>(u32x2{o[2], o[3]}, f);
        bsum[1] += (f[0] + f[1]) + (f[2] + f[3]);
      }
    }
#pragma unroll
    for (int u = 0; u < XPT; ++u) {
      const int item = u * 256 + threadIdx.x, q = item / XP, cp = item % XP;
      *(u32x4*)(xs + (q * BK + 2 * cp) * 8) = transpose4(xreg[u]);
    }
  };

  f32x16 acc[IB][JB];
#pragma unroll
  for (int i = 0; i < IB; ++i)
#pragma unroll
    for (int j = 0; j < JB; ++j)
#pragma unroll
      for (int r = 0; r < 16; ++r) acc[i][j][r] = 0.f;

  const int g = lane >> 5, col = lane & 31;
  const int nit = (int)((tend - t0 + BT - 1) / BT);
  load_stage(0);
  write_stage(0);
  __syncthreads();
  for (int it = 0; it < nit; ++it) {
    const int buf = it & 1;
    if (it + 1 < nit) load_stage(it + 1);
    const unsigned char* gs = smem + buf * STAGE;
    const unsigned char* xs = gs + GBYTES;
#pragma unroll
    for (int ks = 0; ks < 2; ++ks) {
      const int qa = 4 * ks + g, qb = 4 * ks + 2 + g;
      typename E::vec8 af[IB], bf[JB];
#pragma unroll
      for (int i = 0; i < IB; ++i) {
        const int c = wn * (BN / 2) + i * 32 + col;
        af[i] = join8<DT>(*(const u32x2*)(gs + (qa * BN + c) * 8), *(const u32x2*)(gs + (qb * BN + c) * 8));
      }
#pragma unroll
      for (int j = 0; j < JB; ++j) {
        const int c = wk * (BK / 2) + j * 32 + col;
        bf[j] = join8<DT>(*(const u32x2*)(xs + (qa * BK + c) * 8), *(const u32x2*)(xs + (qb * BK + c) * 8));
      }
#pragma unroll
      for (int i = 0; i < IB; ++i)
#pragma unroll
        for (int j = 0; j < JB; ++j) acc[i][j] = E::mma(af[i], bf[j], acc[i][j]);
    }
    if (it + 1 < nit) write_stage(buf ^ 1);
    __syncthreads();
  }

  tn_store<IB, JB>(acc, P, accumulate, tt, N, K, wn, wk, g, col);
  if (do_bias) {
    float* red = (float*)smem;
    red[threadIdx.x * 2] = bsum[0];
    red[threadIdx.x * 2 + 1] = bsum[1];
    __syncthreads();
    if (threadIdx.x < BN) {
      const int cp = threadIdx.x >> 1, e = threadIdx.x & 1;
      float sum = 0.f;
      for (int t = cp; t < 256; t += GP) sum += red[t * 2 + e];
      if (accumulate == 2) gbias[(long)tt.slab * N + n0 + threadIdx.x] = sum;
      else atomicAdd(gbias + n0 + threadIdx.x, sum);
    }
  }
}

__device__ __forceinline__ u32x2 lds_read_tr16(unsigned addr) {
  u32x2 r;
  asm volatile("ds_read_b64_tr_b16 %0, %1" : "=v"(r) : "v"(addr) : "memory");
  return r;
}

template <int DT, int BN, int BK, int BT, bool GATHER = false, bool SEG = false>
__device__ __forceinline__ void gemm_tn_dma_body(const uint16_t* __restrict__ G, const uint16_t* __restrict__ X,
                                                 float* __restrict__ P, int T, int N, int K, long ldg, long ldx,
                                                 int R, int tiles_k, int accumulate, float* __restrict__ gbias,
                                                 const float* __restrict__ rowscale, int rows_per_sample,
                                                 const void* zero, const WgradGeom& wg, int bid, int nblocks) {
  using E = Elem<DT>;
  constexpr int IB = BN / 64, JB = BK / 64;
  constexpr int GROW = BN * 2, XROW = BK * 2;
  constexpr int GBYTES = BT * GROW, XBYTES = BT * XROW, STAGE = GBYTES + XBYTES;
  constexpr int GPPR = BN / 8, XPPR = BK / 8;
  constexpr int GI = BT * GPPR / 256, XI = BT * XPPR / 256;
  static_assert(GI >= 1 && XI >= 1 && (BN == 64 || BN == 128) && (BK == 64 || BK == 128), "tile");
  constexpr int kMaxScales = 64;
  __shared__ __attribute__((aligned(16))) unsigned char smem[2 * STAGE];
  __shared__ float sscale[kMaxScales];

  const int lane = threadIdx.x & 63, wave = threadIdx.x >> 6;
  const int wn = wave >> 1, wk = wave & 1;
  const TnTile tt = tn_tile<BN, BK>(bid, nblocks, N, tiles_k, R, T);
  const int slab = tt.slab, n0 = tt.n0, k0 = tt.k0;
  const long t0 = tt.t0, tend = tt.tend;
  static_assert(!(SEG && GATHER), "sample segments: plain operands only");
  auto gswz = [](int r) { return BN == 64 ? ((r >> 1) & 1) << 2 : (r & 3) << 2; };
  auto xswz = [](int r) { return BK == 64 ? ((r >> 1) & 1) << 2 : (r & 3) << 2; };

  const long s0 = SEG ? t0 / rows_per_sample : 0;
  auto seg_end = [&](long a) { return SEG ? min(tend, (a / rows_per_sample + 1) * rows_per_sample) : tend; };
  int nit = 0;
  if constexpr (SEG) {
    const long s1 = (tend - 1) / rows_per_sample;
    if ((int)threadIdx.x <= (int)(s1 - s0) && threadIdx.x < kMaxScales) sscale[threadIdx.x] = rowscale[s0 + threadIdx.x];
    for (long a = t0; a < tend;) {
      const long e = seg_end(a);
      nit += (int)((e - a + BT - 1) / BT);
      a = e;
    }
  } else {
    nit = (int)((tend - t0 + BT - 1) / BT);
  }
  TnTap tap[GATHER ? XI : 1];
  TnRow px[GATHER ? XI : 1];
  if constexpr (GATHER) {
#pragma unroll
    for (int u = 0; u < XI; ++u) {
      const int q = XI * wave + u, r = q * (64 / XPPR) + lane / XPPR, c = lane % XPPR;
      tap[u] = tn_tap(wg, (unsigned)(k0 + 8 * (c ^ xswz(r))));
      px[u].seek(wg, t0 + r);
    }
  }
  long itb = t0, iend = seg_end(t0);
  auto issue = [&](int it, int buf) {
    unsigned char* gs = smem + buf * STAGE;
    unsigned char* xs = gs + GBYTES;
    const long tb = SEG ? itb : t0 + (long)it * BT;
    const long tlim = SEG ? iend : tend;
    if constexpr (SEG) {
      itb += BT;
      if (itb >= iend) {
        itb = iend;
        iend = seg_end(iend);
      }
    }
#pragma unroll
    for (int u = 0; u < GI; ++u) {
      const int q = GI * wave + u, r = q * (64 / GPPR) + lane / GPPR, c = lane % GPPR;
      const long t = tb + r;
      const void* src = t < tlim ? (const void*)(G + t * ldg + n0 + 8 * (c ^ gswz(r))) : zero;
      lds_dma16(src, gs + q * 1024);
    }
#pragma unroll
    for (int u = 0; u < XI; ++u) {
      const int q = XI * wave + u, r = q * (64 / XPPR) + lane / XPPR, c = lane % XPPR;
      const long t = tb + r;
      const void* src;
      if constexpr (GATHER) {
        const int iy = px[u].oy * wg.stride + tap[u].dy, ix = px[u].ox * wg.stride + tap[u].dx;
        const bool ok = t < tend && tap[u].ok && (unsigned)iy < (unsigned)wg.H && (unsigned)ix < (unsigned)wg.W;
        src = ok ? (const void*)(X + (((long)px[u].b * wg.H + iy) * wg.W + ix) * wg.C + tap[u].c) : zero;
        px[u].advance(wg, BT);
      } else {
        src = t < tlim ? (const void*)(X + t * ldx + k0 + 8 * (c ^ xswz(r))) : zero;
      }
      lds_dma16(src, xs + q * 1024);
    }
  };

  f32x16 acc[IB][JB];
#pragma unroll
  for (int i = 0; i < IB; ++i)
#pragma unroll
    for (int j = 0; j < JB; ++j)
#pragma unroll
      for (int r = 0; r < 16; ++r) acc[i][j][r] = 0.f;
  float bsum[IB];
#pragma unroll
  for (int i = 0; i < IB; ++i) bsum[i] = 0.f;
  const bool do_bias = gbias != nullptr && k0 == 0 && wk == 0;
// ... 59 lines not shown
      for (int i = 0; i < IB; ++i) asm volatile("" : "+v"(a0[set][i]), "+v"(a1[set][i]));
#pragma unroll
      for (int j = 0; j < JB; ++j) asm volatile("" : "+v"(b0[set][j]), "+v"(b1[set][j]));
#pragma unroll
      for (int i = 0; i < IB; ++i) {
        if (do_bias) {
          float f[8];
          unpack4<DT>(a0[set][i], *(float(*)[4])&f[0]);
          unpack4<DT>(a1[set][i], *(float(*)[4])&f[4]);
          bsum[i] += ((f[0] + f[1]) + (f[2] + f[3])) + ((f[4] + f[5]) + (f[6] + f[7]));
        }
        af[i] = join8<DT>(a0[set][i], a1[set][i]);
      }
#pragma unroll
      for (int j = 0; j < JB; ++j) bf[j] = join8<DT>(b0[set][j], b1[set][j]);
#pragma unroll
      for (int i = 0; i < IB; ++i)
#pragma unroll
        for (int j = 0; j < JB; ++j) acc[i][j] = E::mma(af[i], bf[j], acc[i][j]);
    });
    if constexpr (SEG) {
      ctb += BT;
      if (ctb >= cend) {
        const float sc = sscale[min((long)(kMaxScales - 1), (cend - 1) / rows_per_sample - s0)];
#pragma unroll
        for (int i = 0; i < IB; ++i) {
          btot[i] = fmaf(sc, bsum[i], btot[i]);
          bsum[i] = 0.f;
#pragma unroll
          for (int j = 0; j < JB; ++j)
#pragma unroll
            for (int r = 0; r < 16; ++r) {
              tot[i][j][r] = fmaf(sc, acc[i][j][r], tot[i][j][r]);
              acc[i][j][r] = 0.f;
            }
        }
        ctb = cend;
        cend = seg_end(cend);
      }
    }
  }
  if constexpr (SEG) {
#pragma unroll
    for (int i = 0; i < IB; ++i) {
      bsum[i] = btot[i];
#pragma unroll
      for (int j = 0; j < JB; ++j) acc[i][j] = tot[i][j];
    }
  }

  tn_store<IB, JB>(acc, P, accumulate, tt, N, K, wn, wk, g, col);
  if (do_bias) {
#pragma unroll
    for (int i = 0; i < IB; ++i) {
      const float sum = half_sum(bsum[i]);
      if (g == 0) {
        if (accumulate == 2) gbias[(long)slab * N + n0 + wn * (BN / 2) + i * 32 + col] = sum;
        else atomicAdd(gbias + n0 + wn * (BN / 2) + i * 32 + col, sum);
      }
    }
  }
}

template <int DT, int BN, int BK, int BT, bool GATHER = false, bool SEG = false>
__global__ __launch_bounds__(256) void gemm_tn_dma_kernel(const uint16_t* __restrict__ G, const uint16_t* __restrict__ X,
                                                          float* __restrict__ P, int T, int N, int K, long ldg, long ldx,
                                                          int R, int tiles_k, int accumulate, float* __restrict__ gbias,
                                                          const float* __restrict__ rowscale, int rows_per_sample,
                                                          const void* zero, WgradGeom wg = WgradGeom{}) {
  gemm_tn_dma_body<DT, BN, BK, BT, GATHER, SEG>(G, X, P, T, N, K, ldg, ldx, R, tiles_k, accumulate, gbias, rowscale,
                                                rows_per_sample, zero, wg, (int)blockIdx.x, (int)gridDim.x);
}

constexpr int kTnGroupMax = 8;
struct TnProblem {
  const uint16_t* G;
  const uint16_t* X;
  float* P;
  float* gbias;
  const float* rowscale;
  long ldg, ldx;
  int T, N, K, R, tiles_k, rows_per_sample, first, nblk;
};
struct TnGroup {
  TnProblem p[kTnGroupMax];
  int count;
};

template <int DT, bool SEG>
__global__ __launch_bounds__(256) void gemm_tn_group_kernel(TnGroup grp, const void* zero) {
  int i = 0;
#pragma unroll
  for (int k = 1; k < kTnGroupMax; ++k)
    if (k < grp.count && (int)blockIdx.x >= grp.p[k].first) i = k;
  const TnProblem& q = grp.p[i];
  gemm_tn_dma_body<DT, 64, 64, 64, false, SEG>(q.G, q.X, q.P, q.T, q.N, q.K, q.ldg, q.ldx, q.R, q.tiles_k, 1, q.gbias, q.rowscale,
                                               q.rows_per_sample, zero, WgradGeom{}, (int)blockIdx.x - q.first, q.nblk);
}

__device__ uint4 g_zero_page[4];
static const void* zero_page() {
  static void* page = nullptr;
  if (page == nullptr && hipGetSymbolAddress(&page, HIP_SYMBOL(g_zero_page)) != hipSuccess) page = nullptr;
  return page;
}

int launch_nt2(const void* X, const void* W, void* Y, long M, long N, long K, long ldx, long ldw, long ldy, const void* bias,
               const void* res, const float* rowscale, int rows_per_sample, int bn2, long t2, hipStream_t s);

template <int DT, bool GATHER>
static int launch_nt(const void* X, const void* W, void* Y, long M, long N, long K, long ldx, long ldw, long ldy,
                     const GemmEpi& epi, ConvGeom cg, hipStream_t s, bool out32 = false) {
  if (GATHER) {
    cg.zero = zero_page();
    if (cg.zero == nullptr) return fail(RFN_ELAUNCH, "conv2d_nhwc: zero page symbol");
  }
  if constexpr (!GATHER && DT == 1) {
    constexpr long g2_min = 200;
    const int bn2 = N % 320 == 0 ? 320 : (N % 256 == 0 && K >= 256 ? 256 : 0);
    const long t2 = bn2 ? (long)cdiv(M, 192) * (N / bn2) : 0;
    if (bn2 && !out32 && K >= 192 && K % 64 == 0 && epi.act == 0 && t2 >= g2_min &&
        (M + 192) * ldy * 2 < (1L << 32) && ldx < (1L << 22) && ldw < (1L << 22) && (((size_t)X | (size_t)W | (size_t)Y) & 15) == 0 &&
        (epi.res == nullptr || ((size_t)epi.res & 15) == 0)) {
      return launch_nt2(X, W, Y, M, N, K, ldx, ldw, ldy, epi.bias, epi.res, epi.rowscale, epi.rows_per_sample, bn2, t2, s);
    }
  }
  constexpr long min_tiles = 2000;
  int bn = (N % 128 == 0) ? 128 : 64, bm = 128;
  if ((long)cdiv(M, 128) * cdiv(N, bn) < min_tiles) {
    bn = 64;
    if ((long)cdiv(M, 128) * cdiv(N, 64) < min_tiles) bm = 64;
  }
  if (N % 256 == 0 && (long)cdiv(M, 256) * (N / 256) >= (K >= 1024 ? 128 : 256)) bm = bn = 256;
  const int tiles_m = cdiv(M, bm), tiles_n = cdiv(N, bn);
  const long total = (long)tiles_m * tiles_n;
  const int ring = 2 * (bm + bn) * 128;
  const int per_cu = std::max(1, std::min(160 * 1024 / ring, 4));
  const bool persistent = K <= 256;
  const int slots = persistent ? 256 * per_cu : 0x7fffffff;
  dim3 grid((unsigned)std::min<long>(total, slots));
#define RFN_NT(BM_, BN_, NW_, OUT32_, GRID_, TILES_N_, TOTAL_)                                                            \
  hipLaunchKernelGGL((gemm_nt_kernel<DT, BM_, BN_, 64, 2, GATHER, NW_, OUT32_>), GRID_, dim3(64 * NW_), 0, s,              \
                     (const uint16_t*)X, (const uint16_t*)W, (uint16_t*)Y, (int)M, (int)N, (int)K, ldx, ldw, ldy, TILES_N_, \
                     (int)(TOTAL_), epi, cg)
  if (out32) {
    bn = (N % 128 == 0) ? 128 : 64;
    bm = bn;
    const int tn = cdiv(N, bn);
    const long tot = (long)cdiv(M, bm) * tn;
    dim3 g32((unsigned)tot);
    if (bn == 128) RFN_NT(128, 128, 4, true, g32, tn, tot);
    else RFN_NT(64, 64, 4, true, g32, tn, tot);
    return check_launch("gemm_nt (fp32 result)");
  }
  if (bm == 256) {
    grid = dim3((unsigned)std::min<long>(total, persistent ? 256 : 0x7fffffff));
    RFN_NT(256, 256, 8, false, grid, tiles_n, total);
  } else if (bn == 128) {
    RFN_NT(128, 128, 4, false, grid, tiles_n, total);
  } else if (bm == 128) {
    RFN_NT(128, 64, 4, false, grid, tiles_n, total);
  } else {
    RFN_NT(64, 64, 4, false, grid, tiles_n, total);
  }
#undef RFN_NT
  return check_launch("gemm_nt");
}

template <int DT, bool GATHER = false>
static int launch_tn(const void* G, const void* X, float* P, long T, long N, long K, long ldg, long ldx, int R,
                     int accumulate, float* gbias, const float* rowscale, int rps, hipStream_t s,
                     WgradGeom wg = WgradGeom{}) {
  const int S = cdiv(T, R);
// ... 113 lines not shown
  RFN_REQUIRE(X && W && Y, "conv2d_nhwc_o32: null operand");
  RFN_REQUIRE(B > 0 && H > 0 && Wd > 0 && C > 0 && C % 8 == 0 && N > 0 && N % 8 == 0, "conv2d_nhwc_o32: sizes (C %% 8, N %% 8)");
  RFN_REQUIRE(KH > 0 && KW > 0 && stride > 0 && dil > 0 && pad >= 0 && (!transposed || (stride & (stride - 1)) == 0),
              "conv2d_nhwc_o32: geometry");
  RFN_REQUIRE(act == 0 || act == 1 || act == 3, "conv2d_nhwc_o32: act");
  const ConvGeom cg = transposed ? conv_geom_dgrad(H, Wd, N, KH, KW, stride, pad, dil) : conv_geom(H, Wd, C, KH, KW, stride, pad, dil);
  RFN_REQUIRE(cg.H > 0 && cg.W > 0 && cg.OH > 0 && cg.OW > 0, "conv2d_nhwc_o32: empty output");
  const long K = conv_kpad(KH, KW, cg.C), M = (long)B * cg.OH * cg.OW, cols = transposed ? C : N;
  RFN_REQUIRE(ldw % 8 == 0 && ldw >= K && ldy % 4 == 0 && ldy >= cols && M < (1L << 31) && K / 8 < 65536, "conv2d_nhwc_o32: ld");
  GemmEpi epi{(const uint16_t*)bias, nullptr, nullptr, 1, act};
  hipStream_t s = (hipStream_t)stream;
  if (!transposed && KH == 3 && KW == 3 && stride == 1 && pad == 1 && dil == 1) {
    const int rc = launch_conv3x3_halo(X, W, bias, Y, B, H, Wd, C, N, ldw, ldy, act, 1, 1, s);
    if (rc != 1) return rc;
  }
  return launch_nt<1, true>(X, W, Y, M, cols, K, 0, ldw, ldy, epi, cg, s, true);
}

int rfn_conv2d_nhwc_dgrad(const void* GY, const void* Wt, void* DX, int B, int H, int Wd, int C, int N, int KH, int KW,
                          int stride, int pad, int dil, long ldw, long ldy, int dtype, rfn_stream_t stream) {
  using namespace rfn;
  RFN_REQUIRE(GY && Wt && DX, "conv2d_nhwc_dgrad: null operand");
  RFN_REQUIRE(dtype == 1 || dtype == 2, "conv2d_nhwc_dgrad: dtype %d (1 = bf16, 2 = f16)", dtype);
  RFN_REQUIRE(B > 0 && H > 0 && Wd > 0 && C > 0 && C % 8 == 0 && N > 0 && N % 8 == 0, "conv2d_nhwc_dgrad: B=%d H=%d W=%d C=%d "
              "N=%d (C %% 8, N %% 8)", B, H, Wd, C, N);
  RFN_REQUIRE(KH > 0 && KW > 0 && stride > 0 && (stride & (stride - 1)) == 0 && dil > 0 && pad >= 0,
              "conv2d_nhwc_dgrad: kernel %dx%d stride %d (power of two) pad %d dil %d", KH, KW, stride, pad, dil);
  const ConvGeom cg = conv_geom_dgrad(H, Wd, N, KH, KW, stride, pad, dil);
  const int OH = cg.H, OW = cg.W;
  RFN_REQUIRE(OH > 0 && OW > 0, "conv2d_nhwc_dgrad: empty output");
  const long K = conv_kpad(KH, KW, N), M = (long)B * H * Wd;
  RFN_REQUIRE(ldw % 8 == 0 && ldw >= K && ldy % 8 == 0 && ldy >= C, "conv2d_nhwc_dgrad: ldw=%ld (>= %ld, padded k) ldy=%ld", ldw,
              K, ldy);
  RFN_REQUIRE(M < (1L << 31) && K / 8 < 65536 && (long)OH * OW * N < (1L << 31), "conv2d_nhwc_dgrad: extent");
  GemmEpi epi{nullptr, nullptr, nullptr, 1, 0};
  hipStream_t s = (hipStream_t)stream;
  return dtype == 1 ? launch_nt<1, true>(GY, Wt, DX, M, C, K, 0, ldw, ldy, epi, cg, s)
                    : launch_nt<2, true>(GY, Wt, DX, M, C, K, 0, ldw, ldy, epi, cg, s);
}

int rfn_conv2d_nhwc_wgrad(const void* GY, const void* X, float* P, float* grad_bias, int B, int H, int Wd, int C, int N, int KH,
                          int KW, int stride, int pad, int dil, long ldg, long Kpad, int rows_per_slab, int accumulate,
                          int dtype, rfn_stream_t stream) {
  using namespace rfn;
  RFN_REQUIRE(GY && X && P, "conv2d_nhwc_wgrad: null operand");
  RFN_REQUIRE(dtype == 1 || dtype == 2, "conv2d_nhwc_wgrad: dtype %d", dtype);
  RFN_REQUIRE(B > 0 && H > 0 && Wd > 0 && C > 0 && C % 2 == 0 && N > 0 && N % 64 == 0, "conv2d_nhwc_wgrad: B=%d H=%d W=%d C=%d N=%d "
              "(C %% 2, N %% 64)", B, H, Wd, C, N);
  RFN_REQUIRE(KH > 0 && KW > 0 && stride > 0 && dil > 0 && pad >= 0, "conv2d_nhwc_wgrad: kernel %dx%d stride %d pad %d dil %d", KH,
              KW, stride, pad, dil);
  const WgradGeom wg = wgrad_geom(H, Wd, C, KH, KW, stride, pad, dil);
  RFN_REQUIRE(wg.OH > 0 && wg.OW > 0, "conv2d_nhwc_wgrad: empty output");
  const long T = (long)B * wg.OH * wg.OW;
  RFN_REQUIRE(Kpad % 64 == 0 && Kpad >= (long)KH * KW * C && ldg % 2 == 0 && ldg >= N, "conv2d_nhwc_wgrad: Kpad=%ld ldg=%ld", Kpad, ldg);
  RFN_REQUIRE(T < (1L << 31) && (long)B * H * Wd * C < (1L << 31) && rows_per_slab > 0 && rows_per_slab % 32 == 0,
              "conv2d_nhwc_wgrad: extent / rows_per_slab");
  RFN_REQUIRE(Kpad < 65536, "conv2d_nhwc_wgrad: Kpad=%ld", Kpad);
  RFN_REQUIRE(accumulate >= 0 && accumulate <= 2, "conv2d_nhwc_wgrad: accumulate %d (0, 1 or 2)", accumulate);
  RFN_REFUSE_NONDET(accumulate == 1 || (grad_bias != nullptr && accumulate != 2), "rfn_conv2d_nhwc_wgrad",
                    "gemm_tn kernels, fp32 atomics (use accumulate = 2)");
  hipStream_t s = (hipStream_t)stream;
  return dtype == 1 ? launch_tn<1, true>(GY, X, P, T, N, Kpad, ldg, 0, rows_per_slab, accumulate, grad_bias, nullptr, 0, s, wg)
                    : launch_tn<2, true>(GY, X, P, T, N, Kpad, ldg, 0, rows_per_slab, accumulate, grad_bias, nullptr, 0, s, wg);
}

int rfn_gemm_tn(const void* G, const void* X, float* P, long T, long N, long K, long ldg, long ldx, int rows_per_slab,
                int accumulate, float* grad_bias, const float* rowscale, int rows_per_sample, int dtype,
                rfn_stream_t stream) {
  using namespace rfn;
  RFN_REQUIRE(G && X && P, "gemm_tn: null operand");
  RFN_REQUIRE(rowscale == nullptr || rows_per_sample > 0, "gemm_tn: rowscale needs rows_per_sample");
  RFN_REQUIRE(dtype == 1 || dtype == 2, "gemm_tn: dtype %d", dtype);
  RFN_REQUIRE(T > 0 && T < (1L << 31) && rows_per_slab > 0 && rows_per_slab % 32 == 0,
              "gemm_tn: T=%ld rows_per_slab=%d (%% 32)", T, rows_per_slab);
  RFN_REQUIRE(N % 64 == 0 && K % 64 == 0 && ldg % 2 == 0 && ldx % 2 == 0, "gemm_tn: N=%ld K=%ld (%% 64)", N, K);
  RFN_REQUIRE(accumulate >= 0 && accumulate <= 2, "gemm_tn: accumulate %d (0, 1 or 2)", accumulate);
  RFN_REFUSE_NONDET(accumulate == 1 || (grad_bias != nullptr && accumulate != 2), "rfn_gemm_tn",
                    "gemm_tn kernels, fp32 atomics (use accumulate = 2)");
  hipStream_t s = (hipStream_t)stream;
  return dtype == 1 ? launch_tn<1>(G, X, P, T, N, K, ldg, ldx, rows_per_slab, accumulate, grad_bias, rowscale, rows_per_sample, s)
                    : launch_tn<2>(G, X, P, T, N, K, ldg, ldx, rows_per_slab, accumulate, grad_bias, rowscale, rows_per_sample, s);
}

int rfn_gemm_tn_grouped(int count, const void* const* G, const void* const* X, float* const* P, float* const* grad_bias,
                        const float* const* rowscale, const long* T, const long* N, const long* K, const long* ldg,
                        const long* ldx, const int* rows_per_slab, const int* rows_per_sample, int dtype, rfn_stream_t stream) {
  using namespace rfn;
  RFN_REQUIRE(count > 0 && count <= kTnGroupMax, "gemm_tn_grouped: 1 .. %d problems (got %d)", kTnGroupMax, count);
  RFN_REQUIRE(G && X && P && grad_bias && rowscale && T && N && K && ldg && ldx && rows_per_slab && rows_per_sample,
              "gemm_tn_grouped: null array");
  RFN_REQUIRE(dtype == 1 || dtype == 2, "gemm_tn_grouped: dtype %d", dtype);
  RFN_REFUSE_NONDET(true, "rfn_gemm_tn_grouped", "gemm_tn_group_kernel, fp32 atomics (use rfn_gemm_tn with accumulate = 2)");
  TnGroup grp{};
  grp.count = count;
  long blocks = 0;
  const bool seg = rowscale[0] != nullptr;
  for (int i = 0; i < count; ++i) {
    RFN_REQUIRE(G[i] && X[i] && P[i], "gemm_tn_grouped: null operand in problem %d", i);
    RFN_REQUIRE((rowscale[i] != nullptr) == seg, "gemm_tn_grouped: problems with and without a row scale in one group");
    RFN_REQUIRE(T[i] > 0 && T[i] < (1L << 31) && rows_per_slab[i] > 0 && rows_per_slab[i] % 32 == 0,
                "gemm_tn_grouped: T=%ld rows_per_slab=%d (%% 32)", T[i], rows_per_slab[i]);
    RFN_REQUIRE(N[i] % 64 == 0 && K[i] % 64 == 0 && N[i] > 0 && K[i] > 0, "gemm_tn_grouped: N=%ld K=%ld (%% 64)", N[i], K[i]);
    RFN_REQUIRE(ldx[i] % 8 == 0 && ldg[i] % 8 == 0 && ((size_t)X[i] & 15) == 0 && ((size_t)G[i] & 15) == 0,
                "gemm_tn_grouped: operands must be 16-byte aligned with row pitches that are multiples of 8");
    const long S = cdiv(T[i], (long)rows_per_slab[i]);
    if (seg) {
      RFN_REQUIRE(rows_per_sample[i] > 0, "gemm_tn_grouped: rowscale needs rows_per_sample");
      const long span = ((long)rows_per_slab[i] + rows_per_sample[i] - 1) / rows_per_sample[i] + 1;
      RFN_REQUIRE(span <= 64, "gemm_tn_grouped: more than 64 samples per slab");
    }
    const int nblk = (int)((N[i] / 64) * (K[i] / 64) * S);
    grp.p[i] = TnProblem{(const uint16_t*)G[i], (const uint16_t*)X[i], P[i], grad_bias[i], rowscale[i], ldg[i], ldx[i], (int)T[i],
                         (int)N[i], (int)K[i], rows_per_slab[i], (int)(K[i] / 64), rows_per_sample[i], (int)blocks, nblk};
    blocks += nblk;
    RFN_REQUIRE(blocks < (1L << 31), "gemm_tn_grouped: grid too large");
  }
  const void* zero = zero_page();
  if (zero == nullptr) return fail(RFN_ELAUNCH, "gemm_tn_grouped: zero page symbol");
  hipStream_t s = (hipStream_t)stream;
  dim3 grid((unsigned)blocks), block(256);
  if (dtype == 1) {
    if (seg) hipLaunchKernelGGL((gemm_tn_group_kernel<1, true>), grid, block, 0, s, grp, zero);
    else hipLaunchKernelGGL((gemm_tn_group_kernel<1, false>), grid, block, 0, s, grp, zero);
  } else {
    if (seg) hipLaunchKernelGGL((gemm_tn_group_kernel<2, true>), grid, block, 0, s, grp, zero);
    else hipLaunchKernelGGL((gemm_tn_group_kernel<2, false>), grid, block, 0, s, grp, zero);
  }
  return check_launch("gemm_tn_group_kernel");
}

}
```

refign_amd/dwconv.py:

```python
import os

import torch

from . import _lib, determinism
from ._tensor import DTYPE_CODE, ptr, require_device_tensor, workspace
from .params import as_dtype, derived, grad_sink

_DW_WS_STRIPES = 128


def _fwd(x, w_tap, bias, dilation, flip, stats=None):
    B, H, W, C = x.shape
    y = torch.empty_like(x)
    lib = _lib.load_library()
    if stats is not None and determinism.enabled():
        ws = workspace(lib.rfn_dwconv3x3_stats_det_workspace_bytes(B, H, W, C, dilation), x.device)
        _lib.call("rfn_dwconv3x3_nhwc_fwd_stats_det", x.device, ptr(x), ptr(w_tap), ptr(bias), ptr(y), ptr(stats), ptr(ws), B,
                  H, W, C, dilation, DTYPE_CODE[x.dtype])
        return y
    if stats is not None:
        _lib.call("rfn_dwconv3x3_nhwc_fwd_stats", x.device, ptr(x), ptr(w_tap), ptr(bias), ptr(y), ptr(stats), B, H, W, C,
                  dilation, DTYPE_CODE[x.dtype])
        return y
    _lib.call("rfn_dwconv3x3_nhwc_fwd", x.device, ptr(x), ptr(w_tap), ptr(bias), ptr(y), B, H, W, C, dilation, DTYPE_CODE[x.dtype],
              1 if flip else 0)
    return y


class _DWConv3x3(torch.autograd.Function):
    @staticmethod
    def forward(ctx, x, weight, bias, dilation, stats=None):
        if x.dtype not in DTYPE_CODE:
            x = x.float()
        x = require_device_tensor(x.contiguous(), "x")
        C = x.shape[-1]
        w_tap = derived(weight, "tap_major_f32", lambda t: t.float().reshape(C, 9).t().contiguous(),
                        lambda t: t.reshape(C, 9).t())
        b32 = None if bias is None else as_dtype(bias, torch.float32).detach().contiguous()
        ctx.save_for_backward(x, w_tap)
        ctx.dilation, ctx.has_bias = dilation, bias is not None
        ctx.wshape, ctx.wdtype = weight.shape, weight.dtype
        ctx.weight, ctx.bias = weight, bias
        return _fwd(x, w_tap, b32, dilation, False, stats)

    @staticmethod
    def backward(ctx, gy):
        x, w_tap = ctx.saved_tensors
        return _dwconv_backward(ctx, x, w_tap, gy.to(x.dtype).contiguous()) + (None,)


class _DWConv3x3Gelu(torch.autograd.Function):

    @staticmethod
    def forward(ctx, x, weight, bias, with_z=False):
        if x.dtype not in DTYPE_CODE:
            x = x.float()
        x = require_device_tensor(x.contiguous(), "x")
        B, H, W, C = x.shape
        w_tap = derived(weight, "tap_major_f32", lambda t: t.float().reshape(C, 9).t().contiguous(),
                        lambda t: t.reshape(C, 9).t())
        b32 = None if bias is None else as_dtype(bias, torch.float32).detach().contiguous()
        need = any(ctx.needs_input_grad)
        with_z = with_z and need
        ctx.set_materialize_grads(False)
        z = torch.empty_like(x) if need else None
        a = torch.empty_like(x)
        _lib.call("rfn_dwconv3x3_gelu_nhwc_fwd", x.device, ptr(x), ptr(w_tap), ptr(b32), ptr(z), ptr(a), B, H, W, C,
                  DTYPE_CODE[x.dtype])
        if need:
            ctx.save_for_backward(x, w_tap, z)
            ctx.has_bias, ctx.wshape, ctx.wdtype = bias is not None, weight.shape, weight.dtype
            ctx.weight, ctx.bias, ctx.dilation = weight, bias, 1
        if with_z:
            ctx.mark_non_differentiable(a)
            ctx.with_z = True
            return a, z
        ctx.with_z = False
        return a

    @staticmethod
    def backward(ctx, *grads):
        x, w_tap, z = ctx.saved_tensors
        if ctx.with_z:
            if grads[1] is None:
                return None, None, None, None
            gz = grads[1].to(z.dtype).contiguous()
        else:
            gz = torch.ops.aten.gelu_backward(grads[0].to(z.dtype).contiguous(), z)
        ctx.saved = (x, w_tap)
        return _dwconv_backward(ctx, x, w_tap, gz)[:3] + (None,)


def _dwconv_backward(ctx, x, w_tap, gy):
    B, H, W, C = x.shape
    gx = gw = gb = None
    need_params = ctx.needs_input_grad[1] or (ctx.has_bias and ctx.needs_input_grad[2])
    if ctx.needs_input_grad[0] and not need_params:
        gx = _fwd(gy, w_tap, None, ctx.dilation, True)
    if need_params:
        sw, sb = grad_sink(ctx.weight), grad_sink(ctx.bias) if ctx.has_bias else None
        direct = sw is not None and (sb is not None or not ctx.has_bias)
        if direct:
            dw, db = sw, sb
        else:
            dw = torch.empty((9, C), dtype=torch.float32, device=x.device)
            db = torch.empty((C,), dtype=torch.float32, device=x.device) if ctx.has_bias else None
        ws = workspace(_DW_WS_STRIPES * 10 * C * 4, x.device)
        tail = (ptr(dw), ptr(db), ptr(ws), B, H, W, C, ctx.dilation, DTYPE_CODE[x.dtype], 3 if direct else 0)
        if ctx.needs_input_grad[0]:
            gx = torch.empty_like(x)
            _lib.call("rfn_dwconv3x3_nhwc_bwd", x.device, ptr(x), ptr(gy), ptr(w_tap), ptr(gx), *tail)
        else:
            _lib.call("rfn_dwconv3x3_nhwc_bwd_weight", x.device, ptr(x), ptr(gy), *tail)
        if not direct:
            gw = dw.t().reshape(ctx.wshape).to(ctx.wdtype)
            gb = db
    return gx, gw, gb, None


def dwconv3x3_gelu_tokens(x, weight, bias, H, W, with_z=False):
    B, N, C = x.shape
    out = _DWConv3x3Gelu.apply(x.reshape(B, H, W, C), weight, bias, with_z)
    if isinstance(out, tuple):
        return out[0].reshape(B, N, C), out[1].reshape(B, N, C)
    return (out.reshape(B, N, C), None) if with_z else out.reshape(B, N, C)


FUSED_FFN = os.environ.get("RFN_FUSED_FFN", "1") != "0"


@torch.no_grad()
def ffn_fc1_dw_gelu(x, fc1, dw, H, W):
    B, N, C = x.shape
    HID = fc1.weight.shape[0]
    if not (FUSED_FFN and x.is_cuda and x.dtype in (torch.bfloat16, torch.float16) and x.is_contiguous() and N == H * W and C % 64 == 0
            and HID % 128 == 0 and fc1.bias is not None and dw.bias is not None and dw.weight.shape == (HID, 1, 3, 3)
            and dw.padding == (1, 1) and dw.stride == (1, 1) and dw.dilation == (1, 1)):
        return None
    w1, b1 = as_dtype(fc1.weight, x.dtype), as_dtype(fc1.bias, x.dtype)
    w_tap = derived(dw.weight, "tap_major_f32", lambda t: t.float().reshape(HID, 9).t().contiguous(), lambda t: t.reshape(HID, 9).t())
    bdw = as_dtype(dw.bias, torch.float32).detach().contiguous()
    a = torch.empty((B, N, HID), dtype=x.dtype, device=x.device)
    _lib.call("rfn_ffn_fc1_dw_gelu_f16" if x.dtype == torch.float16 else "rfn_ffn_fc1_dw_gelu_bf16", x.device, ptr(x), ptr(w1),
              ptr(b1), ptr(w_tap), ptr(bdw), ptr(a), B, H, W, C, HID)
    return a


def dwconv3x3_nhwc(x, weight, bias=None, dilation=1, stats=None):
    if x.dim() != 4 or weight.shape[0] != x.shape[-1]:
        raise RuntimeError("dwconv3x3_nhwc: x must be (B,H,W,C) and weight (C,1,3,3)")
    if stats is not None and not (x.dtype in (torch.bfloat16, torch.float16) and x.shape[-1] % 8 == 0 and stats.dtype == torch.float64
                                  and stats.is_contiguous() and stats.numel() == 2 * x.shape[-1] + 1):
        raise RuntimeError("dwconv3x3_nhwc(stats=...): bf16 / fp16 input with C % 8 == 0 and a float64 buffer of 2 C + 1 elements")
    return _DWConv3x3.apply(x, weight, bias, int(dilation), stats)


def _stats_only(x, w_tap, b32, dilation):
    B, H, W, C = x.shape
    sums = torch.empty(2 * C + 1, dtype=torch.float64, device=x.device)
    if determinism.enabled():
        ws = workspace(_lib.load_library().rfn_dwconv3x3_stats_det_workspace_bytes(B, H, W, C, dilation), x.device)
        _lib.call("rfn_dwconv3x3_nhwc_stats_det", x.device, ptr(x), ptr(w_tap), ptr(b32), ptr(sums), ptr(ws), B, H, W, C,
                  dilation, DTYPE_CODE[x.dtype])
    else:
        _lib.call("rfn_dwconv3x3_nhwc_stats", x.device, ptr(x), ptr(w_tap), ptr(b32), ptr(sums), B, H, W, C, dilation,
                  DTYPE_CODE[x.dtype])
    return sums


@torch.no_grad()
def dwconv3x3_stats_nhwc(x, weight, bias, dilation):
    C = x.shape[-1]
    w_tap = derived(weight, "tap_major_f32", lambda t: t.float().reshape(C, 9).t().contiguous(),
                    lambda t: t.reshape(C, 9).t())
    b32 = None if bias is None else as_dtype(bias, torch.float32).detach().contiguous()
    return _stats_only(x, w_tap, b32, int(dilation))


@torch.no_grad()
def dwconv3x3_bn_act_nhwc(x, weight, bias, dilation, bn, relu):
    from . import bn as bnk
    B, H, W, C = x.shape
    w_tap = derived(weight, "tap_major_f32", lambda t: t.float().reshape(C, 9).t().contiguous(),
                    lambda t: t.reshape(C, 9).t())
    b32 = None if bias is None else as_dtype(bias, torch.float32).detach().contiguous()
    g = None if bn.weight is None else as_dtype(bn.weight, torch.float32).detach().contiguous()
    be = None if bn.bias is None else as_dtype(bn.bias, torch.float32).detach().contiguous()
    y = torch.empty_like(x)
    sums = _stats_only(x, w_tap, b32, int(dilation))
# ... 66 lines not shown
```

refign_amd/layernorm.py:

```python
import torch
import torch.nn as nn
import torch.nn.functional as F

from . import _lib
from ._tensor import DTYPE_CODE, ptr, workspace
from .params import as_dtype, grad_sink

_LN_WS_ROWS = 256


class _LayerNormFn(torch.autograd.Function):
    @staticmethod
    def forward(ctx, x, weight, bias, eps, out_dtype):
        C = x.shape[-1]
        x2 = x.contiguous().view(-1, C)
        rows = x2.shape[0]
        w32 = as_dtype(weight, torch.float32).detach().contiguous()
        b32 = as_dtype(bias, torch.float32).detach().contiguous()
        y = torch.empty((rows, C), dtype=out_dtype, device=x.device)
        mean = torch.empty(rows, dtype=torch.float32, device=x.device)
        rstd = torch.empty(rows, dtype=torch.float32, device=x.device)
        _lib.call("rfn_layernorm_fwd", x.device, ptr(x2), ptr(w32), ptr(b32), ptr(y), ptr(mean), ptr(rstd), rows, C, float(eps),
                  DTYPE_CODE[x2.dtype], DTYPE_CODE[out_dtype])
        ctx.save_for_backward(x2, w32, mean, rstd)
        ctx.shape, ctx.wdtype = x.shape, weight.dtype
        ctx.weight, ctx.bias = weight, bias
        return y.view(x.shape)

    @staticmethod
    def backward(ctx, gy):
        return _ln_backward(ctx, gy, None)


def _ln_backward(ctx, gy, add, gy_b=None):
        x2, w32, mean, rstd = ctx.saved_tensors
        rows, C = x2.shape
        if gy is None:
            gy, gy_b = gy_b, None
        if gy is None:
            return (add, None, None, None, None)
        if gy.dtype not in DTYPE_CODE:
            gy = gy.float()
        gy2 = gy.contiguous().view(rows, C)
        if gy_b is not None:
            if C % 8 == 0:
                gy_b = gy_b.to(gy2.dtype).contiguous().view(rows, C)
            else:
                gy2, gy_b = gy2 + gy_b.to(gy2.dtype).contiguous().view(rows, C), None
        dx = torch.empty_like(x2)
        if add is not None:
            add = add.to(x2.dtype).contiguous().view(rows, C)
        sg, sb = grad_sink(ctx.weight), grad_sink(ctx.bias)
        direct = sg is not None and sb is not None
        dg = sg if direct else torch.empty(C, dtype=torch.float32, device=x2.device)
        db = sb if direct else torch.empty(C, dtype=torch.float32, device=x2.device)
        ws = workspace(_LN_WS_ROWS * 2 * C * 4, x2.device)
        tail = (ptr(w32), ptr(mean), ptr(rstd), ptr(dx), ptr(dg), ptr(db), ptr(ws), rows, C, DTYPE_CODE[x2.dtype],
                DTYPE_CODE[gy2.dtype], 1 if direct else 0)
        if gy_b is not None:
            _lib.call("rfn_layernorm_bwd_add2", x2.device, ptr(x2), ptr(gy2), ptr(gy_b), ptr(add), *tail)
            add = None
        elif add is not None and C % 8 == 0:
            _lib.call("rfn_layernorm_bwd_add", x2.device, ptr(x2), ptr(gy2), ptr(add), *tail)
            add = None
        else:
            _lib.call("rfn_layernorm_bwd", x2.device, ptr(x2), ptr(gy2), *tail)
        if add is not None:
            dx = dx + add
        if direct:
            return dx.view(ctx.shape), None, None, None, None
        return dx.view(ctx.shape), dg.to(ctx.wdtype), db.to(ctx.wdtype), None, None


class _LayerNormPassFn(torch.autograd.Function):

    @staticmethod
    def forward(ctx, x, weight, bias, eps, out_dtype):
        y = _LayerNormFn.forward(ctx, x, weight, bias, eps, out_dtype)
        return y, x.view_as(x)

    @staticmethod
    def backward(ctx, gy, gx_res):
        return _ln_backward(ctx, gy, gx_res)


class _LayerNormPass2Fn(torch.autograd.Function):

    @staticmethod
    def forward(ctx, x, weight, bias, eps, out_dtype):
        y = _LayerNormFn.forward(ctx, x, weight, bias, eps, out_dtype)
        return y, y.view_as(y), x.view_as(x)

    @staticmethod
    def backward(ctx, gy, gy_b, gx_res):
        return _ln_backward(ctx, gy, gx_res, gy_b)


def layer_norm_pass2(x, weight, bias, eps=1e-5):
    out_dtype = torch.get_autocast_dtype("cuda") if torch.is_autocast_enabled("cuda") else x.dtype
    if out_dtype not in DTYPE_CODE:
        out_dtype = x.dtype
    return _LayerNormPass2Fn.apply(x, weight, bias, eps, out_dtype)


def layer_norm_pass(x, weight, bias, eps=1e-5):
    out_dtype = torch.get_autocast_dtype("cuda") if torch.is_autocast_enabled("cuda") else x.dtype
    if out_dtype not in DTYPE_CODE:
        out_dtype = x.dtype
    return _LayerNormPassFn.apply(x, weight, bias, eps, out_dtype)


def layer_norm(x, weight, bias, eps=1e-5, out_dtype=None):
    if x.dtype not in DTYPE_CODE:
        x = x.float()
    if out_dtype is None:
        out_dtype = torch.get_autocast_dtype("cuda") if torch.is_autocast_enabled("cuda") else x.dtype
        if out_dtype not in DTYPE_CODE:
            out_dtype = x.dtype
    return _LayerNormFn.apply(x, weight, bias, eps, out_dtype)


class LayerNorm(nn.LayerNorm):
    def forward(self, x):
        if x.is_cuda and len(self.normalized_shape) == 1 and self.normalized_shape[0] <= 1024 \
                and self.weight is not None and self.bias is not None:
            return layer_norm(x, self.weight, self.bias, self.eps)
        return F.layer_norm(x, self.normalized_shape, self.weight, self.bias, self.eps)
```

refign_amd/mfma.py:

```python
import ctypes
import os

import torch

from . import _lib, determinism
from ._tensor import ptr
from ._tensor import DTYPE_CODE16 as _DT16

ENABLED = True

LIBRARY_CALLS = {}
_NOTE = True


def note_library(kind, *tensors):
    if not _NOTE or not tensors or not tensors[0].is_cuda:
        return
    key = (kind, str(tensors[0].dtype).replace("torch.", ""), tuple(tuple(t.shape) for t in tensors))
    n = LIBRARY_CALLS.get(key)
    if n is None and len(LIBRARY_CALLS) < 4096:
        if os.environ.get("RFN_LOG_LIBRARY", "0") == "1":
            print(f"[refign_amd] library fallback: {kind} {key[1]} {key[2]}", flush=True)
        LIBRARY_CALLS[key] = 1
    elif n is not None:
# ... 124 lines not shown
        want = min(want, max(4, _TN_ATOMICS // nk, -(-_TN_MIN_WGS // max(tiles, 1))))
    rows = -(-T // want)
    rows = max(256, -(-rows // 32) * 32)
    return rows


def _tn_domain(g, x, rowscale, rows_per_sample):
    if not (ENABLED and g.is_cuda and g.dtype in _DT16 and x.dtype == g.dtype and g.dim() == 2 and x.dim() == 2
            and g.stride(1) == 1 and x.stride(1) == 1 and g.stride(0) % 2 == 0 and x.stride(0) % 2 == 0
            and g.data_ptr() % 4 == 0 and x.data_ptr() % 4 == 0):
        return False
    T, N = g.shape
    K = x.shape[1]
    if x.shape[0] != T or N % 64 != 0 or K % 64 != 0 or T == 0:
        return False
    if rowscale is not None and not (rowscale.dtype == torch.float32 and rowscale.is_contiguous() and rows_per_sample > 0
                                     and rowscale.numel() * rows_per_sample >= T):
        return False
    return True


def gemm_tn(g, x, rows_per_slab=None, out=None, bias_out=None, rowscale=None, rows_per_sample=0):
    if not _tn_domain(g, x, rowscale, rows_per_sample):
        return None
    T, N = g.shape
    K = x.shape[1]
    if rows_per_slab is None:
        tile = 128 if (N % 128 == 0 and K % 128 == 0) else 64
        rows_per_slab = slab_rows(T, (N // tile) * (K // tile), N * K)
    S = -(-T // rows_per_slab)
    if out is not None:
        if not (out.dtype == torch.float32 and out.is_contiguous() and out.numel() == N * K and
                (bias_out is None or (bias_out.dtype == torch.float32 and bias_out.is_contiguous()
                                      and bias_out.numel() == N))):
            return None
        if determinism.enabled():
            return _gemm_tn_det(g, x, int(rows_per_slab), S, out, bias_out, rowscale, rows_per_sample)
        part = out
    else:
        part = torch.empty((S, N, K), dtype=torch.float32, device=g.device)
    _lib.call("rfn_gemm_tn", g.device, ptr(g), ptr(x), ptr(part), T, N, K, g.stride(0), x.stride(0), int(rows_per_slab),
              0 if out is None else 1, ptr(bias_out) if out is not None else None, ptr(rowscale), int(rows_per_sample),
              _DT16[g.dtype])
    return part


def _gemm_tn_det(g, x, rows_per_slab, S, out, bias_out, rowscale, rows_per_sample):
    from .params import sum_rows
    T, N = g.shape
    K = x.shape[1]
    part = torch.empty((S, N * K), dtype=torch.float32, device=g.device)
    bpart = torch.empty((S, N), dtype=torch.float32, device=g.device) if bias_out is not None else None
    _lib.call("rfn_gemm_tn", g.device, ptr(g), ptr(x), ptr(part), T, N, K, g.stride(0), x.stride(0), rows_per_slab, 2,
              ptr(bpart), ptr(rowscale), int(rows_per_sample), _DT16[g.dtype])
    sum_rows(part, out=out.view(-1), accumulate=True)
    if bpart is not None:
        sum_rows(bpart, out=bias_out.view(-1), accumulate=True)
    return out


GROUP_WGRADS = True
_TN_GROUP_MAX = 8
_WGRAD_QUEUE = None


def defer_gemm_tn(g, x, out, bias_out=None, rowscale=None, rows_per_sample=0):
    q = _WGRAD_QUEUE
    if q is None or determinism.enabled() or not _tn_domain(g, x, rowscale, rows_per_sample):
        return False
    T, N = g.shape
    K = x.shape[1]
    if not (out.dtype == torch.float32 and out.is_contiguous() and out.numel() == N * K and
            (bias_out is None or (bias_out.dtype == torch.float32 and bias_out.is_contiguous() and bias_out.numel() == N))):
        return False
    if g.stride(0) % 8 or x.stride(0) % 8 or g.data_ptr() % 16 or x.data_ptr() % 16:
        return False
    rows = slab_rows(T, (N // 64) * (K // 64), N * K)
    if rowscale is not None and (rows + rows_per_sample - 1) // rows_per_sample + 1 > 64:
        return False
    q.append((g, x, out, bias_out, rowscale, int(rows_per_sample), int(rows)))
    return True


def flush_wgrads():
    q = _WGRAD_QUEUE
    if not q:
        return
    items, q[:] = list(q), []
    classes = {}
    for it in items:
        classes.setdefault((it[4] is not None, it[0].dtype, it[0].device), []).append(it)
    vp, lg, it_ = ctypes.c_void_p, ctypes.c_long, ctypes.c_int
    for (seg, dt, dev), lst in classes.items():
        for a in range(0, len(lst), _TN_GROUP_MAX):
            grp = lst[a:a + _TN_GROUP_MAX]
            n = len(grp)
            arr = lambda ty, vals: (ty * n)(*vals)
            G = arr(vp, [t[0].data_ptr() for t in grp])
            X = arr(vp, [t[1].data_ptr() for t in grp])
            P = arr(vp, [t[2].data_ptr() for t in grp])
            Bv = arr(vp, [None if t[3] is None else t[3].data_ptr() for t in grp])
            R = arr(vp, [None if t[4] is None else t[4].data_ptr() for t in grp])
            T = arr(lg, [t[0].shape[0] for t in grp])
            N = arr(lg, [t[0].shape[1] for t in grp])
            K = arr(lg, [t[1].shape[1] for t in grp])
            ldg = arr(lg, [t[0].stride(0) for t in grp])
            ldx = arr(lg, [t[1].stride(0) for t in grp])
            rps = arr(it_, [t[6] for t in grp])
            rsa = arr(it_, [t[5] for t in grp])
            cast = lambda a_: ctypes.cast(a_, vp)
            _lib.call("rfn_gemm_tn_grouped", dev, n, cast(G), cast(X), cast(P), cast(Bv), cast(R), cast(T), cast(N), cast(K),
                      cast(ldg), cast(ldx), cast(rps), cast(rsa), _DT16[dt])


class deferred_wgrads:

    def __enter__(self):
        global _WGRAD_QUEUE
        self._outer = _WGRAD_QUEUE
        if GROUP_WGRADS and ENABLED and self._outer is None:
            _WGRAD_QUEUE = []
        return self

    def __exit__(self, *exc):
        global _WGRAD_QUEUE
        if self._outer is None and _WGRAD_QUEUE is not None:
            try:
                if exc[0] is None:
                    flush_wgrads()
            finally:
                _WGRAD_QUEUE = None
        return False


class _WgradMark(torch.autograd.Function):

    @staticmethod
    def forward(ctx, x):
        return x.view_as(x)

    @staticmethod
    def backward(ctx, g):
        flush_wgrads()
        return g


def wgrad_mark(x):
    return _WgradMark.apply(x) if (GROUP_WGRADS and torch.is_grad_enabled() and x.requires_grad) else x


_PACK_BLOCK = 4096


def _pack(src, batch_stride, row_stride, B, heads, nrows, nblk, want_r=True, want_t=True, src2=None):
    dev = src.device
    nbytes = B * heads * nblk * _PACK_BLOCK
    new = lambda want: torch.empty(nbytes, dtype=torch.uint8, device=dev) if want else None
    r, t = new(want_r), new(want_t)
    r2, t2 = (new(want_r), new(want_t)) if src2 is not None else (None, None)
    _lib.call("rfn_attn_pack", dev, ptr(src), batch_stride, row_stride, B, heads, nrows, nblk, ptr(r), ptr(t), ptr(src2),
              ptr(r2), ptr(t2))
    return (r, t), (r2, t2)


def _attn_ok(q, kv, heads):
    if not (ENABLED and q.is_cuda and q.dtype in _DT16 and kv.dtype == q.dtype and q.dim() == 3 and kv.dim() == 3):
        return False
    B, N, C = q.shape
    return (C == heads * 64 and kv.shape[0] == B and kv.shape[2] == 2 * C and q.is_contiguous() and kv.is_contiguous()
            and q.data_ptr() % 16 == 0 and kv.data_ptr() % 16 == 0)


def _dims(q, kv):
    B, N, C = q.shape
    Nkv = kv.shape[1]
    nkblk = -(-Nkv // 32)
    nkblk += nkblk & 1
    nqblk = -(-N // 32)
    return B, N, C, Nkv, nkblk, nqblk, nqblk * 32


def _fwd(q, kv, heads, scale, need_bwd):
    B, N, C, Nkv, nkblk, nqblk, nqpad = _dims(q, kv)
    dev = q.device
    (kvr, kvt), _ = _pack(kv, kv.stride(0), kv.stride(1), B, 2 * heads, Nkv, nkblk)
    voff = heads * nkblk * _PACK_BLOCK
    o = torch.empty_like(q)
    lse2 = torch.empty((B * heads, nqpad), dtype=torch.float32, device=dev)
    _lib.call("rfn_attn_fwd", dev, ptr(q), q.stride(0), q.stride(1), kvr.data_ptr(), kvt.data_ptr() + voff, ptr(o), o.stride(0),
              o.stride(1), ptr(lse2), B, heads, N, Nkv, nkblk, nqpad, float(scale), 2 * heads, _DT16[q.dtype])
    return o, lse2, (kvr, kvt)


def _chunk_blocks(nqblk, Nkv, BH):
    kblocks = -(-Nkv // 256)
    chunks = max(1, 128 // max(1, kblocks * BH))
    return max(4, -(-nqblk // chunks))


class _AttnFn(torch.autograd.Function):
    @staticmethod
    def forward(ctx, q, kv, heads, scale):
        need = q.requires_grad or kv.requires_grad
        o, lse2, packs = _fwd(q, kv, heads, scale, need)
        if need:
            ctx.save_for_backward(q, kv, o, lse2, *packs)
            ctx.heads, ctx.scale = heads, scale
        return o

    @staticmethod
    def backward(ctx, do):
        q, kv, o, lse2, kvr, kvt = ctx.saved_tensors
        heads, scale = ctx.heads, ctx.scale
        B, N, C, Nkv, nkblk, nqblk, nqpad = _dims(q, kv)
        dev = q.device
        if do.dtype != q.dtype:
            do = do.to(q.dtype)
        if not do.is_contiguous():
            do = do.contiguous()
        dt = _DT16[q.dtype]
        dq = torch.empty_like(q)
        delta = torch.empty_like(lse2)
        voff = heads * nkblk * _PACK_BLOCK
        _lib.call("rfn_attn_bwd_dq", dev, ptr(q), q.stride(0), q.stride(1), ptr(do), ptr(o), o.stride(0), o.stride(1),
                  kvr.data_ptr(), kvr.data_ptr() + voff, kvt.data_ptr(), ptr(lse2), ptr(delta), ptr(dq), dq.stride(0),
                  dq.stride(1), B, heads, N, Nkv, nkblk, nqpad, float(scale), 2 * heads, dt)
        (qr, qt), (gr, gt) = _pack(q, q.stride(0), q.stride(1), B, heads, N, nqblk, src2=do)
        nkpad = -(-Nkv // 32) * 32
        chunk = _chunk_blocks(nqblk, Nkv, B * heads)
        det = determinism.enabled()
        images = -(-nqblk // chunk) if det else 1
        accT = torch.empty(images * B * heads * 2 * 64 * nkpad, dtype=torch.float32, device=dev)
        dkv = torch.empty_like(kv)
        k_view, v_view = kv[:, :, :C], kv[:, :, C:]
        _lib.call("rfn_attn_bwd_dkv_det" if det else "rfn_attn_bwd_dkv", dev, ptr(k_view), ptr(v_view), kv.stride(0), kv.stride(1),
                  ptr(qr), ptr(qt), ptr(gr), ptr(gt), ptr(lse2), ptr(delta), ptr(accT), ptr(dkv), B, heads, N, Nkv, nqblk, nqpad,
                  nkpad, chunk, float(scale), dt)
        return dq, dkv, None, None


def attention(q, kv, heads, scale):
    if not _attn_ok(q, kv, heads):
        return None
    return _AttnFn.apply(q, kv, heads, scale)
```

refign_amd/seg.py:

```python
import math
import os
import random
from functools import partial, wraps
from typing import Callable, List, Optional, Union

import torch
import torch.nn as nn
import torch.nn.functional as F

from . import f8 as _f8
from . import linear as _linear
from . import determinism, mfma
from ._tensor import const_tensor
from ._tensor import DTYPE_CODE as _CE_DT
from .align import BaseHead
from .conv import Conv2d, patch_conv_tokens
from .layernorm import LayerNorm
from .layers import MLP, ConvBNReLU, DropPath
from .linear import Linear
from .upcat import upsample_concat
from .upsample import interpolate_bilinear

_MIT = {
    'mit_b0': ([32, 64, 160, 256], [2, 2, 2, 2]),
    'mit_b1': ([64, 128, 320, 512], [2, 2, 2, 2]),
    'mit_b2': ([64, 128, 320, 512], [3, 4, 6, 3]),
    'mit_b3': ([64, 128, 320, 512], [3, 4, 18, 3]),
    'mit_b4': ([64, 128, 320, 512], [3, 8, 27, 3]),
    'mit_b5': ([64, 128, 320, 512], [3, 6, 40, 3]),
}
_MIT_HEADS = [1, 2, 5, 8]
_MIT_SR = [8, 4, 2, 1]


_GRAD_READY_CB = None


class _GradMark(torch.autograd.Function):

    @staticmethod
    def forward(ctx, x, tag):
        ctx.tag = tag
        return x.view_as(x)

    @staticmethod
    def backward(ctx, g):
        cb = _GRAD_READY_CB
        if cb is not None:
            cb(ctx.tag)
        return g, None


def grad_mark(x, tag):
    return _GradMark.apply(x, tag) if (torch.is_grad_enabled() and x.requires_grad) else x


class DWConv(nn.Module):

    def __init__(self, dim=768):
        super().__init__()
        self.dwconv = nn.Conv2d(dim, dim, 3, 1, 1, bias=True, groups=dim)

    def forward(self, x, H, W):
        B, N, C = x.shape
        if x.is_cuda and C % 8 == 0:
            from .dwconv import dwconv3x3_tokens
            return dwconv3x3_tokens(x, self.dwconv.weight, self.dwconv.bias, H, W)
        y = self.dwconv(x.transpose(1, 2).reshape(B, C, H, W))
        return y.flatten(2).transpose(1, 2)


class Mlp(nn.Module):

    def __init__(self, in_features, hidden_features=None, out_features=None, act_layer=nn.GELU, drop=0.):
        super().__init__()
        out_features = out_features or in_features
        hidden_features = hidden_features or in_features
        self.fc1 = Linear(in_features, hidden_features)
        self.dwconv = DWConv(hidden_features)
        self.act = act_layer()
        self.fc2 = Linear(hidden_features, out_features)
        self.drop = nn.Dropout(drop)

    def forward(self, x, H, W, res=None, rowscale=None):
        if x.is_cuda and not torch.is_grad_enabled() and x.dtype in (torch.bfloat16, torch.float16) and type(self.act) is nn.GELU \
                and self.act.approximate == 'none' and self.drop.p == 0. and type(self.fc1) is Linear and not _f8.active():
            from .dwconv import ffn_fc1_dw_gelu
            a = ffn_fc1_dw_gelu(x, self.fc1, self.dwconv.dwconv, H, W)
            if a is not None:
                return self.fc2(a, res=res, rowscale=rowscale) if res is not None else self.fc2(a)
        x = self.fc1(x)
        if x.is_cuda and x.shape[-1] % 8 == 0 and type(self.act) is nn.GELU and self.act.approximate == 'none':
            from .dwconv import dwconv3x3_gelu_tokens
            dw = self.dwconv.dwconv
            if torch.is_grad_enabled() and x.requires_grad and self.drop.p == 0. and x.dtype in (torch.bfloat16, torch.float16) \
                    and os.environ.get("RFN_FUSED_GELU_BWD", "1") == "1":
                a, z = dwconv3x3_gelu_tokens(x, dw.weight, dw.bias, H, W, with_z=True)
                if res is not None:
                    return self.fc2(a, res=res, rowscale=rowscale, z=z)
                return self.fc2(a, z=z)
            x = self.drop(dwconv3x3_gelu_tokens(x, dw.weight, dw.bias, H, W))
        else:
            x = self.drop(self.act(self.dwconv(x, H, W)))
        if res is not None and self.drop.p == 0.:
            return self.fc2(x, res=res, rowscale=rowscale)
        y = self.drop(self.fc2(x))
        return y if res is None else _residual(res, y, rowscale)


_SDPA_BACKEND = None
_FUSED_UPCAT = True


def _fused_upcat_here():
    return _FUSED_UPCAT
_SR_AS_LINEAR = True


class Attention(nn.Module):

    def __init__(self, dim, num_heads=8, qkv_bias=False, qk_scale=None, attn_drop=0., proj_drop=0., sr_ratio=1):
        super().__init__()
        assert dim % num_heads == 0, f'dim {dim} should be divided by num_heads {num_heads}.'
        self.dim, self.num_heads = dim, num_heads
        self.scale = qk_scale or (dim // num_heads) ** -0.5
        self.q = Linear(dim, dim, bias=qkv_bias)
        self.kv = Linear(dim, dim * 2, bias=qkv_bias)
        self.attn_drop = nn.Dropout(attn_drop)
        self.proj = Linear(dim, dim)
# ... 673 lines not shown
```

Before: 16.92.

## Fold LN/dwconv column reductions into grouped wgrad launch and fuse accT zeroing into pack

Layernorm and depthwise-conv backward now write per-block partials and defer their column-sum reductions into a queue. These are then executed inside the grouped TN weight-gradient GEMM launch, cutting the number of small reduction kernels. The attention backward also clears the fp32 dK/dV accumulator inside the pack kernel rather than with a separate memset. A flush is added at grad-mark points, so the deferred work runs before the gradient-ready callbacks, at the cost of more complex ordering and extra host bookkeeping.

```diff
diff --git a/include/refign_hip.h b/include/refign_hip.h
--- a/include/refign_hip.h
+++ b/include/refign_hip.h
@@ -113,6 +113,9 @@
 int rfn_dwconv3x3_nhwc_bwd(const void* x, const void* grad_y, const float* weight_tap_major, void* grad_x, float* grad_weight,
                            float* grad_bias, void* workspace, int B, int H, int W, int C, int dilation, int dtype, int flags,
                            rfn_stream_t stream);
+int rfn_dwconv3x3_bwd_partial_rows(int B, int H, int W, int C, int dilation, int dtype);
+int rfn_dwconv3x3_nhwc_bwd_partial(const void* x, const void* grad_y, const float* weight_tap_major, void* grad_x, void* workspace,
+                                   int B, int H, int W, int C, int dilation, int dtype, rfn_stream_t stream);
 
 int rfn_layernorm_fwd(const void* x, const float* gamma, const float* beta, void* y, float* mean, float* rstd,
                       long rows, int C, float eps, int in_dtype, int out_dtype, rfn_stream_t stream);
@@ -126,6 +129,10 @@
 int rfn_layernorm_bwd_add2(const void* x, const void* grad_y, const void* grad_y2, const void* add, const float* gamma,
                            const float* mean, const float* rstd, void* grad_x, float* grad_gamma, float* grad_beta, void* workspace,
                            long rows, int C, int x_dtype, int gy_dtype, int accumulate, rfn_stream_t stream);
+int rfn_layernorm_bwd_partial_rows(long rows, int C);
+int rfn_layernorm_bwd_partial(const void* x, const void* grad_y, const void* grad_y2, const void* add, const float* gamma,
+                              const float* mean, const float* rstd, void* grad_x, void* workspace, long rows, int C, int x_dtype,
+                              int gy_dtype, rfn_stream_t stream);
 
 int rfn_uncertainty9_weights_len(void);
 int rfn_uncertainty9_frontend_f32(const float* corr, const float* weights, float* out, int B, int H, int W,
@@ -181,9 +188,17 @@
 int rfn_gemm_tn_grouped(int count, const void* const* G, const void* const* X, float* const* P, float* const* grad_bias,
                         const float* const* rowscale, const long* T, const long* N, const long* K, const long* ldg,
                         const long* ldx, const int* rows_per_slab, const int* rows_per_sample, int dtype, rfn_stream_t stream);
+int rfn_gemm_tn_grouped_colsum(int count, const void* const* G, const void* const* X, float* const* P, float* const* grad_bias,
+                               const float* const* rowscale, const long* T, const long* N, const long* K, const long* ldg,
+                               const long* ldx, const int* rows_per_slab, const int* rows_per_sample, int nred, const int* red_kind,
+                               const float* const* red_ws, float* const* red_dst0, float* const* red_dst1, const int* red_C,
+                               const int* red_rows, const int* red_flags, int dtype, rfn_stream_t stream);
 
 int rfn_attn_pack(const void* src, long batch_stride, long row_stride, int B, int heads, int nrows, int nblk, void* rpack,
                   void* tpack, const void* src2, void* rpack2, void* tpack2, rfn_stream_t stream);
+int rfn_attn_pack_zero(const void* src, long batch_stride, long row_stride, int B, int heads, int nrows, int nblk, void* rpack,
+                       void* tpack, const void* src2, void* rpack2, void* tpack2, void* zero, unsigned long zero_bytes,
+                       rfn_stream_t stream);
 int rfn_attn_fwd(const void* Q, long q_batch_stride, long q_row_stride, const void* k_rpack, const void* v_tpack, void* O,
                  long o_batch_stride, long o_row_stride, float* lse2, int B, int heads, int Nq, int Nkv, int nkblk,
                  int nqpad, float scale, int kv_pack_heads, int dtype, rfn_stream_t stream);
@@ -196,6 +211,10 @@
                      const void* q_tpack, const void* do_rpack, const void* do_tpack, const float* lse2,
                      const float* delta, float* accT, void* dKV, int B, int heads, int Nq, int Nkv, int nqblk, int nqpad,
                      int nkpad, int blocks_per_chunk, float scale, int dtype, rfn_stream_t stream);
+int rfn_attn_bwd_dkv_zeroed(const void* K, const void* V, long kv_batch_stride, long kv_row_stride, const void* q_rpack,
+                            const void* q_tpack, const void* do_rpack, const void* do_tpack, const float* lse2,
+                            const float* delta, float* accT, void* dKV, int B, int heads, int Nq, int Nkv, int nqblk, int nqpad,
+                            int nkpad, int blocks_per_chunk, float scale, int dtype, rfn_stream_t stream);
 
 int rfn_attn32_fwd(const float* Q, long q_batch_stride, long q_row_stride, const float* KV, long kv_batch_stride,
                    long kv_row_stride, float* O, long o_batch_stride, long o_row_stride, float* lse2, int B, int heads,
diff --git a/refign_amd/csrc/attn.hip b/refign_amd/csrc/attn.hip
--- a/refign_amd/csrc/attn.hip
+++ b/refign_amd/csrc/attn.hip
@@ -8,11 +8,19 @@
 constexpr int kPackBlock = 4096;
 constexpr float kLog2e = 1.4426950408889634f;
 
+template <bool ZERO>
 __global__ __launch_bounds__(256) void attn_pack_kernel(const uint16_t* __restrict__ src0, const uint16_t* __restrict__ src1,
                                                         long sb, long sr, int heads, int nrows, int nblk,
                                                         unsigned char* __restrict__ rpack0, unsigned char* __restrict__ tpack0,
-                                                        unsigned char* __restrict__ rpack1, unsigned char* __restrict__ tpack1) {
+                                                        unsigned char* __restrict__ rpack1, unsigned char* __restrict__ tpack1,
+                                                        u32x4* __restrict__ zero = nullptr, size_t n16 = 0) {
   __shared__ unsigned tile[32][33];
+  if constexpr (ZERO) {
+    const size_t wg = ((size_t)blockIdx.z * gridDim.y + blockIdx.y) * gridDim.x + blockIdx.x;
+    const size_t step = (size_t)gridDim.x * gridDim.y * gridDim.z * 256;
+    const u32x4 z = {0u, 0u, 0u, 0u};
+    for (size_t i = wg * 256 + threadIdx.x; i < n16; i += step) zero[i] = z;
+  }
   const uint16_t* src = blockIdx.z ? src1 : src0;
   unsigned char* rpack = blockIdx.z ? rpack1 : rpack0;
   unsigned char* tpack = blockIdx.z ? tpack1 : tpack0;
@@ -525,10 +533,27 @@
               nrows, nblk);
   RFN_REQUIRE(row_stride % 8 == 0 && batch_stride % 8 == 0, "attn_pack: strides must be multiples of 8 elements");
   dim3 grid(nblk, B * heads, src2 ? 2 : 1);
-  hipLaunchKernelGGL(attn_pack_kernel, grid, dim3(256), 0, (hipStream_t)stream, (const uint16_t*)src,
+  hipLaunchKernelGGL(attn_pack_kernel<false>, grid, dim3(256), 0, (hipStream_t)stream, (const uint16_t*)src,
                      (const uint16_t*)src2, batch_stride, row_stride, heads, nrows, nblk, (unsigned char*)rpack,
-                     (unsigned char*)tpack, (unsigned char*)rpack2, (unsigned char*)tpack2);
+                     (unsigned char*)tpack, (unsigned char*)rpack2, (unsigned char*)tpack2, (u32x4*)nullptr, (size_t)0);
   return check_launch("attn_pack");
+}
+
+int rfn_attn_pack_zero(const void* src, long batch_stride, long row_stride, int B, int heads, int nrows, int nblk, void* rpack,
+                       void* tpack, const void* src2, void* rpack2, void* tpack2, void* zero, unsigned long zero_bytes,
+                       rfn_stream_t stream) {
+  RFN_REQUIRE(src && (rpack || tpack), "attn_pack_zero: null pointer");
+  RFN_REQUIRE(src2 == nullptr || rpack2 || tpack2, "attn_pack_zero: second tensor without outputs");
+  RFN_REQUIRE(B > 0 && heads > 0 && nrows > 0 && nblk * 32 >= nrows, "attn_pack_zero: B=%d heads=%d rows=%d nblk=%d", B, heads,
+              nrows, nblk);
+  RFN_REQUIRE(row_stride % 8 == 0 && batch_stride % 8 == 0, "attn_pack_zero: strides must be multiples of 8 elements");
+  RFN_REQUIRE(zero && zero_bytes > 0 && zero_bytes % 16 == 0 && ((size_t)zero & 15) == 0,
+              "attn_pack_zero: the region to clear must be 16-byte aligned and a multiple of 16 bytes (%lu)", zero_bytes);
+  dim3 grid(nblk, B * heads, src2 ? 2 : 1);
+  hipLaunchKernelGGL(attn_pack_kernel<true>, grid, dim3(256), 0, (hipStream_t)stream, (const uint16_t*)src,
+                     (const uint16_t*)src2, batch_stride, row_stride, heads, nrows, nblk, (unsigned char*)rpack,
+                     (unsigned char*)tpack, (unsigned char*)rpack2, (unsigned char*)tpack2, (u32x4*)zero, (size_t)(zero_bytes / 16));
+  return check_launch("attn_pack_zero");
 }
 
 int rfn_attn_fwd(const void* Q, long q_batch_stride, long q_row_stride, const void* k_rpack, const void* v_tpack, void* O,
@@ -574,7 +599,7 @@
   return check_launch("attn_bwd_dq");
 }
 
-static int attn_bwd_dkv_impl(bool det, const void* K, const void* V, long kv_batch_stride, long kv_row_stride, const void* q_rpack,
+static int attn_bwd_dkv_impl(bool det, bool zero, const void* K, const void* V, long kv_batch_stride, long kv_row_stride, const void* q_rpack,
                              const void* q_tpack, const void* do_rpack, const void* do_tpack, const float* lse2,
                              const float* delta, float* accT, void* dKV, int B, int heads, int Nq, int Nkv, int nqblk, int nqpad,
                              int nkpad, int blocks_per_chunk, float scale, int dtype, rfn_stream_t stream) {
@@ -587,7 +612,7 @@
               nqpad, nkpad, blocks_per_chunk);
   hipStream_t s = (hipStream_t)stream;
   const long image = (long)B * heads * 2 * 64 * nkpad, chunk_stride = det ? image : 0;
-  if (!det)
+  if (!det && zero)
     if (int rc = zero_async(accT, (size_t)image * sizeof(float), s)) return rc;
   dim3 grid(cdiv(Nkv, 256), cdiv(nqblk, blocks_per_chunk), B * heads);
   const int chunks = det ? (int)grid.y : 1;
@@ -622,15 +647,24 @@
                      const float* delta, float* accT, void* dKV, int B, int heads, int Nq, int Nkv, int nqblk, int nqpad,
                      int nkpad, int blocks_per_chunk, float scale, int dtype, rfn_stream_t stream) {
   RFN_REFUSE_NONDET(true, "rfn_attn_bwd_dkv", "attn_bwd_dkv_kernel, fp32 atomics (use rfn_attn_bwd_dkv_det)");
-  return attn_bwd_dkv_impl(false, K, V, kv_batch_stride, kv_row_stride, q_rpack, q_tpack, do_rpack, do_tpack, lse2, delta, accT,
+  return attn_bwd_dkv_impl(false, true, K, V, kv_batch_stride, kv_row_stride, q_rpack, q_tpack, do_rpack, do_tpack, lse2, delta, accT,
                            dKV, B, heads, Nq, Nkv, nqblk, nqpad, nkpad, blocks_per_chunk, scale, dtype, stream);
+}
+
+int rfn_attn_bwd_dkv_zeroed(const void* K, const void* V, long kv_batch_stride, long kv_row_stride, const void* q_rpack,
+                            const void* q_tpack, const void* do_rpack, const void* do_tpack, const float* lse2,
+                            const float* delta, float* accT, void* dKV, int B, int heads, int Nq, int Nkv, int nqblk, int nqpad,
+                            int nkpad, int blocks_per_chunk, float scale, int dtype, rfn_stream_t stream) {
+  RFN_REFUSE_NONDET(true, "rfn_attn_bwd_dkv", "attn_bwd_dkv_kernel, fp32 atomics, reached through rfn_attn_bwd_dkv_zeroed (use rfn_attn_bwd_dkv_det)");
+  return attn_bwd_dkv_impl(false, false, K, V, kv_batch_stride, kv_row_stride, q_rpack, q_tpack, do_rpack, do_tpack, lse2, delta,
+                           accT, dKV, B, heads, Nq, Nkv, nqblk, nqpad, nkpad, blocks_per_chunk, scale, dtype, stream);
 }
 
 int rfn_attn_bwd_dkv_det(const void* K, const void* V, long kv_batch_stride, long kv_row_stride, const void* q_rpack,
                          const void* q_tpack, const void* do_rpack, const void* do_tpack, const float* lse2,
                          const float* delta, float* accT, void* dKV, int B, int heads, int Nq, int Nkv, int nqblk, int nqpad,
                          int nkpad, int blocks_per_chunk, float scale, int dtype, rfn_stream_t stream) {
-  return attn_bwd_dkv_impl(true, K, V, kv_batch_stride, kv_row_stride, q_rpack, q_tpack, do_rpack, do_tpack, lse2, delta, accT,
+  return attn_bwd_dkv_impl(true, false, K, V, kv_batch_stride, kv_row_stride, q_rpack, q_tpack, do_rpack, do_tpack, lse2, delta, accT,
                            dKV, B, heads, Nq, Nkv, nqblk, nqpad, nkpad, blocks_per_chunk, scale, dtype, stream);
 }
 
diff --git a/refign_amd/csrc/colsum.h b/refign_amd/csrc/colsum.h
--- /dev/null
+++ b/refign_amd/csrc/colsum.h
@@ -0,0 +1,59 @@
+#pragma once
+#include "common.h"
+
+namespace rfn {
+
+constexpr int kLnMaxBlocks = 256;
+constexpr int kMaxStripes = 128;
+
+constexpr int kColsumLn = 0, kColsumDw = 1;
+
+inline int ln_reduce_grid(int C) { return cdiv(2L * C, 64); }
+inline int dw_reduce_grid(int C) { return cdiv(10L * C, 32); }
+
+__device__ __forceinline__ void ln_bwd_reduce_body(const float* __restrict__ ws, float* __restrict__ dgamma,
+                                                   float* __restrict__ dbeta, int C, int nblocks, int accumulate,
+                                                   int bid, float* part) {
+  const int lane = threadIdx.x & 63, seg = threadIdx.x >> 6;
+  const int col = bid * 64 + lane;
+  float s = 0.0f;
+  if (col < 2 * C) {
+#pragma unroll 8
+    for (int b = seg; b < nblocks; b += 4) s += ws[(size_t)b * 2 * C + col];
+  }
+  part[seg * 64 + lane] = s;
+  __syncthreads();
+  if (seg == 0 && col < 2 * C) {
+    const float t = (part[lane] + part[64 + lane]) + (part[128 + lane] + part[192 + lane]);
+    float* dst = col < C ? dgamma + col : dbeta + (col - C);
+    *dst = accumulate ? *dst + t : t;
+  }
+}
+
+__device__ __forceinline__ void dw_bwd_weight_reduce_body(const float* __restrict__ ws, float* __restrict__ dw,
+                                                          float* __restrict__ db, int C, int stripes, int flags, int bid,
+                                                          float* part) {
+  const int lane = threadIdx.x & 31, seg = threadIdx.x >> 5;
+  const int idx = bid * 32 + lane;
+  float s = 0.0f;
+  if (idx < 10 * C) {
+#pragma unroll 4
+    for (int t = seg; t < stripes; t += 8) s += ws[(size_t)t * 10 * C + idx];
+  }
+  part[seg * 32 + lane] = s;
+  __syncthreads();
+  if (seg != 0 || idx >= 10 * C) return;
+  s = ((part[lane] + part[32 + lane]) + (part[64 + lane] + part[96 + lane])) +
+      ((part[128 + lane] + part[160 + lane]) + (part[192 + lane] + part[224 + lane]));
+  float* dst;
+  if (idx < 9 * C) {
+    const int k = idx / C, c = idx - k * C;
+    dst = (flags & 2) ? dw + c * 9 + k : dw + idx;
+  } else {
+    if (db == nullptr) return;
+    dst = db + (idx - 9 * C);
+  }
+  *dst = (flags & 1) ? *dst + s : s;
+}
+
+}
diff --git a/refign_amd/csrc/dwconv.hip b/refign_amd/csrc/dwconv.hip
--- a/refign_amd/csrc/dwconv.hip
+++ b/refign_amd/csrc/dwconv.hip
@@ -2,6 +2,7 @@
 
 #include <type_traits>
 
+#include "colsum.h"
 #include "common.h"
 #include "mfma.h"
 
@@ -665,28 +666,8 @@
                                                                           float* __restrict__ dw,
                                                                           float* __restrict__ db, int C, int stripes,
                                                                           int flags) {
-  __shared__ float part[8][32];
-  const int lane = threadIdx.x & 31, seg = threadIdx.x >> 5;
-  const int idx = blockIdx.x * 32 + lane;
-  float s = 0.0f;
-  if (idx < 10 * C) {
-#pragma unroll 4
-    for (int t = seg; t < stripes; t += 8) s += ws[(size_t)t * 10 * C + idx];
-  }
-  part[seg][lane] = s;
-  __syncthreads();
-  if (seg != 0 || idx >= 10 * C) return;
-  s = ((part[0][lane] + part[1][lane]) + (part[2][lane] + part[3][lane])) +
-      ((part[4][lane] + part[5][lane]) + (part[6][lane] + part[7][lane]));
-  float* dst;
-  if (idx < 9 * C) {
-    const int k = idx / C, c = idx - k * C;
-    dst = (flags & 2) ? dw + c * 9 + k : dw + idx;
-  } else {
-    if (db == nullptr) return;
-    dst = db + (idx - 9 * C);
-  }
-  *dst = (flags & 1) ? *dst + s : s;
+  __shared__ float part[256];
+  dw_bwd_weight_reduce_body(ws, dw, db, C, stripes, flags, (int)blockIdx.x, part);
 }
 
 static inline int pick_cvb(int CV) { return CV >= 64 ? 64 : (CV >= 32 ? 32 : (CV >= 16 ? 16 : 8)); }
@@ -703,7 +684,6 @@
   const int j = (int)std::max<long>(1, std::min<long>(cdiv(nslots, pl), per_xcd));
   return SlicedGeom{true, cvb, 8 * j};
 }
-constexpr int kMaxStripes = 128;
 
 template <typename T>
 static int launch_fwd_gelu(const void* x, const float* w, const float* bias, void* y, void* ya, int B, int H, int W,
@@ -836,16 +816,34 @@
   return check_launch("dwconv3x3_fwd_kernel");
 }
 
+struct BwdGeom {
+  bool sliced;
+  int cvb, gxb, rows;
+};
 template <typename T>
-static int launch_bwd(const void* x, const void* gy, const float* w, void* gx, float* dw, float* db, float* ws, int B, int H,
-                      int W, int C, int dil, int flags, hipStream_t st) {
+static BwdGeom bwd_geom(int B, int H, int W, int C, int dil) {
   constexpr int V = BwdIO<T>::N, V16 = 16 / (int)sizeof(T);
   const int CV = C / V;
   const int WQ = dil * (((W + dil - 1) / dil + kPX - 1) / kPX);
-  int rows;
   if (SlicedGeom sg = sliced_geom(C / V16, 1L << 30); sg.on) {
     const int cvb = sg.cvb * (V16 / V), pl = 256 / cvb;
-    rows = (int)std::max<long>(1, std::min<long>(cdiv((long)B * dil * ((H + dil - 1) / dil) * WQ, pl), sg.grid / 8));
+    const int rows = (int)std::max<long>(1, std::min<long>(cdiv((long)B * dil * ((H + dil - 1) / dil) * WQ, pl), sg.grid / 8));
+    return BwdGeom{true, cvb, 0, rows};
+  }
+  int cvb = pick_cvb(CV);
+  while (cvb > 8 && cdiv(CV, cvb) < 4) cvb >>= 1;
+  const int gxb = cdiv(CV, cvb), pl = 256 / cvb;
+  const long nquads = (long)B * H * WQ;
+  const int rows = (int)std::max<long>(1, std::min<long>(std::min<long>(kMaxStripes, cdiv(nquads, pl)), std::max<long>(1, (256L * 8) / gxb)));
+  return BwdGeom{false, cvb, gxb, rows};
+}
+
+template <typename T>
+static int launch_bwd(const void* x, const void* gy, const float* w, void* gx, float* dw, float* db, float* ws, int B, int H,
+                      int W, int C, int dil, int flags, hipStream_t st, bool reduce = true) {
+  const BwdGeom bg = bwd_geom<T>(B, H, W, C, dil);
+  const int rows = bg.rows, cvb = bg.cvb;
+  if (bg.sliced) {
     if (gx != nullptr)
       hipLaunchKernelGGL((dwconv3x3_bwd_kernel<T, true>), dim3(8 * rows), dim3(256), 0, st, (const T*)x, (const T*)gy, w, (T*)gx,
                          ws, B, H, W, C, dil, cvb, 1);
@@ -853,20 +851,16 @@
       hipLaunchKernelGGL((dwconv3x3_bwd_kernel<T, false>), dim3(8 * rows), dim3(256), 0, st, (const T*)x, (const T*)gy, w,
                          (T*)nullptr, ws, B, H, W, C, dil, cvb, 1);
   } else {
-    int cvb = pick_cvb(CV);
-    while (cvb > 8 && cdiv(CV, cvb) < 4) cvb >>= 1;
-    const int gxb = cdiv(CV, cvb), pl = 256 / cvb;
-    const long nquads = (long)B * H * WQ;
-    rows = (int)std::max<long>(1, std::min<long>(std::min<long>(kMaxStripes, cdiv(nquads, pl)), std::max<long>(1, (256L * 8) / gxb)));
     if (gx != nullptr)
-      hipLaunchKernelGGL((dwconv3x3_bwd_kernel<T, true>), dim3(gxb, rows), dim3(256), 0, st, (const T*)x, (const T*)gy, w,
+      hipLaunchKernelGGL((dwconv3x3_bwd_kernel<T, true>), dim3(bg.gxb, rows), dim3(256), 0, st, (const T*)x, (const T*)gy, w,
                          (T*)gx, ws, B, H, W, C, dil, cvb, 0);
     else
-      hipLaunchKernelGGL((dwconv3x3_bwd_kernel<T, false>), dim3(gxb, rows), dim3(256), 0, st, (const T*)x, (const T*)gy, w,
+      hipLaunchKernelGGL((dwconv3x3_bwd_kernel<T, false>), dim3(bg.gxb, rows), dim3(256), 0, st, (const T*)x, (const T*)gy, w,
                          (T*)nullptr, ws, B, H, W, C, dil, cvb, 0);
   }
   if (int rc = check_launch("dwconv3x3_bwd_kernel")) return rc;
-  hipLaunchKernelGGL(dwconv3x3_bwd_weight_reduce_kernel, dim3(cdiv(10L * C, 32)), dim3(256), 0, st, ws, dw, db, C, rows, flags);
+  if (!reduce) return RFN_OK;
+  hipLaunchKernelGGL(dwconv3x3_bwd_weight_reduce_kernel, dim3(dw_reduce_grid(C)), dim3(256), 0, st, ws, dw, db, C, rows, flags);
   return check_launch("dwconv3x3_bwd_weight_reduce_kernel");
 }
 
@@ -1223,17 +1217,18 @@
 
 static int dw_bwd(const char* who, const void* x, const void* grad_y, const float* weight, void* grad_x, float* grad_weight,
                   float* grad_bias, void* workspace, int B, int H, int W, int C, int dilation, int dtype, int flags,
-                  hipStream_t st) {
-  RFN_REQUIRE(x && grad_y && grad_weight && workspace, "%s: null pointer", who);
+                  hipStream_t st, bool reduce = true) {
+  RFN_REQUIRE(x && grad_y && (grad_weight || !reduce) && workspace, "%s: null pointer", who);
   RFN_REQUIRE(B > 0 && H > 0 && W > 0 && C > 0 && dilation > 0, "%s: bad size", who);
   if (dtype == 0) {
     RFN_REQUIRE(C % 4 == 0, "%s: C must be a multiple of 4 for f32", who);
-    return launch_bwd<float>(x, grad_y, weight, grad_x, grad_weight, grad_bias, (float*)workspace, B, H, W, C, dilation, flags, st);
+    return launch_bwd<float>(x, grad_y, weight, grad_x, grad_weight, grad_bias, (float*)workspace, B, H, W, C, dilation, flags, st,
+                             reduce);
   }
   RFN_REQUIRE(C % 8 == 0, "%s: C must be a multiple of 8 for 16-bit activations", who);
   return dt_one(dtype, who, [&](auto t) {
     return launch_bwd<typename decltype(t)::type>(x, grad_y, weight, grad_x, grad_weight, grad_bias, (float*)workspace, B, H, W, C,
-                                                  dilation, flags, st);
+                                                  dilation, flags, st, reduce);
   });
 }
 
@@ -1252,4 +1247,21 @@
                 dilation, dtype, flags, (hipStream_t)stream);
 }
 
-}
+int rfn_dwconv3x3_bwd_partial_rows(int B, int H, int W, int C, int dilation, int dtype) {
+  if (!(B > 0 && H > 0 && W > 0 && C > 0 && dilation > 0) || (dtype == 0 ? C % 4 : C % 8) != 0) return 0;
+  switch (dtype) {
+    case 0: return bwd_geom<float>(B, H, W, C, dilation).rows;
+    case 1: return bwd_geom<__hip_bfloat16>(B, H, W, C, dilation).rows;
+    case 2: return bwd_geom<_Float16>(B, H, W, C, dilation).rows;
+  }
+  return 0;
+}
+
+int rfn_dwconv3x3_nhwc_bwd_partial(const void* x, const void* grad_y, const float* weight_tap_major, void* grad_x, void* workspace,
+                                   int B, int H, int W, int C, int dilation, int dtype, rfn_stream_t stream) {
+  RFN_REQUIRE((weight_tap_major != nullptr) == (grad_x != nullptr), "rfn_dwconv3x3_nhwc_bwd_partial: weight_tap_major and grad_x go together");
+  return dw_bwd("rfn_dwconv3x3_nhwc_bwd_partial", x, grad_y, weight_tap_major, grad_x, nullptr, nullptr, workspace, B, H, W, C,
+                dilation, dtype, 0, (hipStream_t)stream, false);
+}
+
+}
diff --git a/refign_amd/csrc/layernorm.hip b/refign_amd/csrc/layernorm.hip
--- a/refign_amd/csrc/layernorm.hip
+++ b/refign_amd/csrc/layernorm.hip
@@ -1,12 +1,12 @@
 #include <hip/hip_bf16.h>
 
+#include "colsum.h"
 #include "common.h"
 #include "mfma.h"
 
 namespace rfn {
 
 constexpr int kLnMaxPerLane = 16;
-constexpr int kLnMaxBlocks = 256;
 
 template <typename T>
 __device__ __forceinline__ float ld(const T* p);
@@ -353,20 +353,8 @@
                                                                    float* __restrict__ dgamma,
                                                                    float* __restrict__ dbeta, int C, int nblocks,
                                                                    int accumulate) {
-  __shared__ float part[4][64];
-  const int col = blockIdx.x * 64 + (threadIdx.x & 63), seg = threadIdx.x >> 6;
-  float s = 0.0f;
-  if (col < 2 * C) {
-#pragma unroll 8
-    for (int b = seg; b < nblocks; b += 4) s += ws[(size_t)b * 2 * C + col];
-  }
-  part[seg][threadIdx.x & 63] = s;
-  __syncthreads();
-  if (seg == 0 && col < 2 * C) {
-    const float t = (part[0][threadIdx.x] + part[1][threadIdx.x]) + (part[2][threadIdx.x] + part[3][threadIdx.x]);
-    float* dst = col < C ? dgamma + col : dbeta + (col - C);
-    *dst = accumulate ? *dst + t : t;
-  }
+  __shared__ float part[256];
+  ln_bwd_reduce_body(ws, dgamma, dbeta, C, nblocks, accumulate, (int)blockIdx.x, part);
 }
 
 static inline int ln_grid(long rows, int cap) { return (int)std::max<long>(1, std::min<long>(cdiv(rows, 4), cap)); }
@@ -400,16 +388,21 @@
   return check_launch("layernorm_fwd_kernel");
 }
 
+static int ln_bwd_rows(long rows, int C) {
+  if (C % 8 != 0) return ln_grid(rows, kLnMaxBlocks);
+  const int lpr = C <= 64 ? 8 : C <= 128 ? 16 : C <= 256 ? 32 : 64;
+  return (int)std::max<long>(1, std::min<long>(cdiv(rows, 4 * (64 / lpr)), kLnMaxBlocks));
+}
+
 template <typename TX, typename TG>
 static int ln_bwd_dispatch(const void* x, const void* gy, const float* g, const float* mean, const float* rstd,
                            void* dx, float* dgamma, float* dbeta, float* ws, long rows, int C, int accumulate,
-                           hipStream_t st, const void* add = nullptr, const void* gy2 = nullptr) {
+                           hipStream_t st, const void* add = nullptr, const void* gy2 = nullptr, bool reduce = true) {
   if ((add != nullptr || gy2 != nullptr) && C % 8 != 0) return fail(RFN_EINVAL, "rfn_layernorm_bwd_add: C %% 8 != 0");
-  int grid = ln_grid(rows, kLnMaxBlocks);
+  const int grid = ln_bwd_rows(rows, C);
   const int npl = cdiv(C, 64);
   if (C % 8 == 0) {
 #define RFN_LN_BWDV(LPR, NV)                                                                                        \
-  grid = (int)std::max<long>(1, std::min<long>(cdiv(rows, 4 * (64 / LPR)), kLnMaxBlocks));                         \
   hipLaunchKernelGGL((layernorm_bwd_vec_kernel<TX, TG, LPR, NV>), dim3(grid), dim3(256), 0, st, (const TX*)x,      \
                      (const TG*)gy, g, mean, rstd, (TX*)dx, ws, rows, C, (const TX*)add, (const TG*)gy2)
     if (C <= 64) { RFN_LN_BWDV(8, 1); }
@@ -430,8 +423,9 @@
 #undef RFN_LN_BWD
   }
   if (int rc = check_launch("layernorm_bwd_kernel")) return rc;
-  hipLaunchKernelGGL(layernorm_bwd_reduce_kernel, dim3(cdiv(2L * C, 64)), dim3(256), 0, st, ws, dgamma, dbeta, C,
-                     grid, accumulate);
+  if (!reduce) return RFN_OK;
+  hipLaunchKernelGGL(layernorm_bwd_reduce_kernel, dim3(ln_reduce_grid(C)), dim3(256), 0, st, ws, dgamma, dbeta, C, grid,
+                     accumulate);
   return check_launch("layernorm_bwd_reduce_kernel");
 }
 
@@ -483,6 +477,24 @@
   });
 }
 
+int rfn_layernorm_bwd_partial_rows(long rows, int C) {
+  return rows > 0 && C > 0 && C <= 64 * kLnMaxPerLane ? ln_bwd_rows(rows, C) : 0;
+}
+
+int rfn_layernorm_bwd_partial(const void* x, const void* grad_y, const void* grad_y2, const void* add, const float* gamma,
+                              const float* mean, const float* rstd, void* grad_x, void* workspace, long rows, int C, int x_dtype,
+                              int gy_dtype, rfn_stream_t stream) {
+  RFN_REQUIRE(x && grad_y && gamma && mean && rstd && grad_x && workspace, "rfn_layernorm_bwd_partial: null pointer");
+  RFN_REQUIRE(rows > 0 && C > 0 && C <= 64 * kLnMaxPerLane, "rfn_layernorm_bwd_partial: need 0 < C <= 1024 (got %d)", C);
+  RFN_REQUIRE(C % 8 == 0 || (grad_y2 == nullptr && add == nullptr), "rfn_layernorm_bwd_partial: grad_y2 / add need C %% 8 == 0 (got %d)", C);
+  hipStream_t st = (hipStream_t)stream;
+  float* ws = (float*)workspace;
+  return dt_pair(x_dtype, gy_dtype, "rfn_layernorm_bwd_partial", [&](auto tx, auto tg) {
+    return ln_bwd_dispatch<typename decltype(tx)::type, typename decltype(tg)::type>(x, grad_y, gamma, mean, rstd, grad_x, nullptr,
+                                                                                      nullptr, ws, rows, C, 0, st, add, grad_y2, false);
+  });
+}
+
 int rfn_layernorm_fwd_f8(const void* x_bf16, const float* gamma, const float* beta, void* y8, long rows, int C, float eps,
                          float out_q, rfn_stream_t stream) {
   RFN_REQUIRE(x_bf16 && gamma && beta && y8, "rfn_layernorm_fwd_f8: null pointer");
diff --git a/refign_amd/csrc/mfma_gemm.hip b/refign_amd/csrc/mfma_gemm.hip
--- a/refign_amd/csrc/mfma_gemm.hip
+++ b/refign_amd/csrc/mfma_gemm.hip
@@ -5,6 +5,7 @@
 #include <cstdlib>
 #include <type_traits>
 
+#include "colsum.h"
 #include "common.h"
 #include "mfma.h"
 
@@ -565,6 +566,11 @@
   return r;
 }
 
+template <int BYTES>
+__device__ __forceinline__ unsigned char* tn_smem() {
+  __shared__ __attribute__((aligned(16))) unsigned char smem[BYTES];
+  return smem;
+}
 template <int DT, int BN, int BK, int BT, bool GATHER = false, bool SEG = false>
 __device__ __forceinline__ void gemm_tn_dma_body(const uint16_t* __restrict__ G, const uint16_t* __restrict__ X,
                                                  float* __restrict__ P, int T, int N, int K, long ldg, long ldx,
@@ -579,7 +585,7 @@
   constexpr int GI = BT * GPPR / 256, XI = BT * XPPR / 256;
   static_assert(GI >= 1 && XI >= 1 && (BN == 64 || BN == 128) && (BK == 64 || BK == 128), "tile");
   constexpr int kMaxScales = 64;
-  __shared__ __attribute__((aligned(16))) unsigned char smem[2 * STAGE];
+  unsigned char* const smem = tn_smem<2 * STAGE>();
   __shared__ float sscale[kMaxScales];
 
   const int lane = threadIdx.x & 63, wave = threadIdx.x >> 6;
@@ -805,13 +811,32 @@
   long ldg, ldx;
   int T, N, K, R, tiles_k, rows_per_sample, first, nblk;
 };
+struct TnColsum {
+  const float* ws;
+  float* dst0;
+  float* dst1;
+  int kind, C, rows, flags, first, nblk;
+};
 struct TnGroup {
   TnProblem p[kTnGroupMax];
-  int count;
+  TnColsum r[kTnGroupMax];
+  int count, nred, red_first;
 };
 
 template <int DT, bool SEG>
 __global__ __launch_bounds__(256) void gemm_tn_group_kernel(TnGroup grp, const void* zero) {
+  if ((int)blockIdx.x >= grp.red_first) {
+    int j = 0;
+#pragma unroll
+    for (int k = 1; k < kTnGroupMax; ++k)
+      if (k < grp.nred && (int)blockIdx.x >= grp.r[k].first) j = k;
+    const TnColsum& c = grp.r[j];
+    float* part = reinterpret_cast<float*>(tn_smem<2 * (64 * 128 + 64 * 128)>());
+    const int bid = (int)blockIdx.x - c.first;
+    if (c.kind == kColsumLn) ln_bwd_reduce_body(c.ws, c.dst0, c.dst1, c.C, c.rows, c.flags & 1, bid, part);
+    else dw_bwd_weight_reduce_body(c.ws, c.dst0, c.dst1, c.C, c.rows, c.flags, bid, part);
+    return;
+  }
   int i = 0;
 #pragma unroll
   for (int k = 1; k < kTnGroupMax; ++k)
@@ -1091,41 +1116,58 @@
                     : launch_tn<2>(G, X, P, T, N, K, ldg, ldx, rows_per_slab, accumulate, grad_bias, rowscale, rows_per_sample, s);
 }
 
-int rfn_gemm_tn_grouped(int count, const void* const* G, const void* const* X, float* const* P, float* const* grad_bias,
-                        const float* const* rowscale, const long* T, const long* N, const long* K, const long* ldg,
-                        const long* ldx, const int* rows_per_slab, const int* rows_per_sample, int dtype, rfn_stream_t stream) {
+static int gemm_tn_grouped_impl(const char* who, int count, const void* const* G, const void* const* X, float* const* P,
+                                float* const* grad_bias, const float* const* rowscale, const long* T, const long* N, const long* K,
+                                const long* ldg, const long* ldx, const int* rows_per_slab, const int* rows_per_sample, int nred,
+                                const int* red_kind, const float* const* red_ws, float* const* red_dst0, float* const* red_dst1,
+                                const int* red_C, const int* red_rows, const int* red_flags, int dtype, rfn_stream_t stream) {
   using namespace rfn;
-  RFN_REQUIRE(count > 0 && count <= kTnGroupMax, "gemm_tn_grouped: 1 .. %d problems (got %d)", kTnGroupMax, count);
-  RFN_REQUIRE(G && X && P && grad_bias && rowscale && T && N && K && ldg && ldx && rows_per_slab && rows_per_sample,
-              "gemm_tn_grouped: null array");
-  RFN_REQUIRE(dtype == 1 || dtype == 2, "gemm_tn_grouped: dtype %d", dtype);
-  RFN_REFUSE_NONDET(true, "rfn_gemm_tn_grouped", "gemm_tn_group_kernel, fp32 atomics (use rfn_gemm_tn with accumulate = 2)");
+  RFN_REQUIRE(count >= 0 && count <= kTnGroupMax && nred >= 0 && nred <= kTnGroupMax && count + nred > 0,
+              "%s: 0 .. %d problems and 0 .. %d column sums, not both 0 (got %d, %d)", who, kTnGroupMax, kTnGroupMax, count, nred);
+  RFN_REQUIRE(count == 0 || (G && X && P && grad_bias && rowscale && T && N && K && ldg && ldx && rows_per_slab && rows_per_sample),
+              "%s: null array", who);
+  RFN_REQUIRE(nred == 0 || (red_kind && red_ws && red_dst0 && red_dst1 && red_C && red_rows && red_flags), "%s: null array", who);
+  RFN_REQUIRE(dtype == 1 || dtype == 2, "%s: dtype %d", who, dtype);
+  RFN_REFUSE_NONDET(count > 0, who, "gemm_tn_group_kernel, fp32 atomics (use rfn_gemm_tn with accumulate = 2)");
   TnGroup grp{};
   grp.count = count;
+  grp.nred = nred;
   long blocks = 0;
-  const bool seg = rowscale[0] != nullptr;
+  const bool seg = count > 0 && rowscale[0] != nullptr;
   for (int i = 0; i < count; ++i) {
-    RFN_REQUIRE(G[i] && X[i] && P[i], "gemm_tn_grouped: null operand in problem %d", i);
-    RFN_REQUIRE((rowscale[i] != nullptr) == seg, "gemm_tn_grouped: problems with and without a row scale in one group");
+    RFN_REQUIRE(G[i] && X[i] && P[i], "%s: null operand in problem %d", who, i);
+    RFN_REQUIRE((rowscale[i] != nullptr) == seg, "%s: problems with and without a row scale in one group", who);
     RFN_REQUIRE(T[i] > 0 && T[i] < (1L << 31) && rows_per_slab[i] > 0 && rows_per_slab[i] % 32 == 0,
-                "gemm_tn_grouped: T=%ld rows_per_slab=%d (%% 32)", T[i], rows_per_slab[i]);
-    RFN_REQUIRE(N[i] % 64 == 0 && K[i] % 64 == 0 && N[i] > 0 && K[i] > 0, "gemm_tn_grouped: N=%ld K=%ld (%% 64)", N[i], K[i]);
+                "%s: T=%ld rows_per_slab=%d (%% 32)", who, T[i], rows_per_slab[i]);
+    RFN_REQUIRE(N[i] % 64 == 0 && K[i] % 64 == 0 && N[i] > 0 && K[i] > 0, "%s: N=%ld K=%ld (%% 64)", who, N[i], K[i]);
     RFN_REQUIRE(ldx[i] % 8 == 0 && ldg[i] % 8 == 0 && ((size_t)X[i] & 15) == 0 && ((size_t)G[i] & 15) == 0,
-                "gemm_tn_grouped: operands must be 16-byte aligned with row pitches that are multiples of 8");
+                "%s: operands must be 16-byte aligned with row pitches that are multiples of 8", who);
     const long S = cdiv(T[i], (long)rows_per_slab[i]);
     if (seg) {
-      RFN_REQUIRE(rows_per_sample[i] > 0, "gemm_tn_grouped: rowscale needs rows_per_sample");
+      RFN_REQUIRE(rows_per_sample[i] > 0, "%s: rowscale needs rows_per_sample", who);
       const long span = ((long)rows_per_slab[i] + rows_per_sample[i] - 1) / rows_per_sample[i] + 1;
-      RFN_REQUIRE(span <= 64, "gemm_tn_grouped: more than 64 samples per slab");
-    }
-    const int nblk = (int)((N[i] / 64) * (K[i] / 64) * S);
+      RFN_REQUIRE(span <= 64, "%s: more than 64 samples per slab", who);
+    }
+    const long nblk = (N[i] / 64) * (K[i] / 64) * S;
+    RFN_REQUIRE(blocks + nblk < (1L << 31), "%s: grid too large", who);
     grp.p[i] = TnProblem{(const uint16_t*)G[i], (const uint16_t*)X[i], P[i], grad_bias[i], rowscale[i], ldg[i], ldx[i], (int)T[i],
-                         (int)N[i], (int)K[i], rows_per_slab[i], (int)(K[i] / 64), rows_per_sample[i], (int)blocks, nblk};
+                         (int)N[i], (int)K[i], rows_per_slab[i], (int)(K[i] / 64), rows_per_sample[i], (int)blocks, (int)nblk};
     blocks += nblk;
-    RFN_REQUIRE(blocks < (1L << 31), "gemm_tn_grouped: grid too large");
+  }
+  grp.red_first = (int)blocks;
+  for (int i = 0; i < nred; ++i) {
+    const bool ln = red_kind[i] == kColsumLn;
+    RFN_REQUIRE(ln || red_kind[i] == kColsumDw, "%s: column sum %d: kind %d (0 = LayerNorm, 1 = depthwise 3x3)", who, i, red_kind[i]);
+    RFN_REQUIRE(red_ws[i] && red_dst0[i] && (red_dst1[i] || !ln), "%s: null pointer in column sum %d", who, i);
+    RFN_REQUIRE(red_C[i] > 0 && red_C[i] < (1 << 24) && red_rows[i] > 0 && red_rows[i] <= (ln ? kLnMaxBlocks : kMaxStripes),
+                "%s: column sum %d: C=%d rows=%d", who, i, red_C[i], red_rows[i]);
+    const int nblk = ln ? ln_reduce_grid(red_C[i]) : dw_reduce_grid(red_C[i]);
+    RFN_REQUIRE(blocks + nblk < (1L << 31), "%s: grid too large", who);
+    grp.r[i] = TnColsum{red_ws[i], red_dst0[i], red_dst1[i], red_kind[i], red_C[i], red_rows[i], red_flags[i], (int)blocks, nblk};
+    blocks += nblk;
   }
   const void* zero = zero_page();
-  if (zero == nullptr) return fail(RFN_ELAUNCH, "gemm_tn_grouped: zero page symbol");
+  if (zero == nullptr) return fail(RFN_ELAUNCH, "%s: zero page symbol", who);
   hipStream_t s = (hipStream_t)stream;
   dim3 grid((unsigned)blocks), block(256);
   if (dtype == 1) {
@@ -1138,4 +1180,21 @@
   return check_launch("gemm_tn_group_kernel");
 }
 
-}
+int rfn_gemm_tn_grouped(int count, const void* const* G, const void* const* X, float* const* P, float* const* grad_bias,
+                        const float* const* rowscale, const long* T, const long* N, const long* K, const long* ldg,
+                        const long* ldx, const int* rows_per_slab, const int* rows_per_sample, int dtype, rfn_stream_t stream) {
+  RFN_REQUIRE(count > 0, "rfn_gemm_tn_grouped: 1 .. 8 problems (got %d)", count);
+  return gemm_tn_grouped_impl("rfn_gemm_tn_grouped", count, G, X, P, grad_bias, rowscale, T, N, K, ldg, ldx, rows_per_slab,
+                              rows_per_sample, 0, nullptr, nullptr, nullptr, nullptr, nullptr, nullptr, nullptr, dtype, stream);
+}
+
+int rfn_gemm_tn_grouped_colsum(int count, const void* const* G, const void* const* X, float* const* P, float* const* grad_bias,
+                               const float* const* rowscale, const long* T, const long* N, const long* K, const long* ldg,
+                               const long* ldx, const int* rows_per_slab, const int* rows_per_sample, int nred, const int* red_kind,
+                               const float* const* red_ws, float* const* red_dst0, float* const* red_dst1, const int* red_C,
+                               const int* red_rows, const int* red_flags, int dtype, rfn_stream_t stream) {
+  return gemm_tn_grouped_impl("rfn_gemm_tn_grouped_colsum", count, G, X, P, grad_bias, rowscale, T, N, K, ldg, ldx, rows_per_slab,
+                              rows_per_sample, nred, red_kind, red_ws, red_dst0, red_dst1, red_C, red_rows, red_flags, dtype, stream);
+}
+
+}
diff --git a/refign_amd/dwconv.py b/refign_amd/dwconv.py
--- a/refign_amd/dwconv.py
+++ b/refign_amd/dwconv.py
@@ -2,7 +2,7 @@
 
 import torch
 
-from . import _lib, determinism
+from . import _lib, determinism, mfma
 from ._tensor import DTYPE_CODE, ptr, require_device_tensor, workspace
 from .params import as_dtype, derived, grad_sink
 
@@ -105,6 +105,15 @@
         else:
             dw = torch.empty((9, C), dtype=torch.float32, device=x.device)
             db = torch.empty((C,), dtype=torch.float32, device=x.device) if ctx.has_bias else None
+        if direct and mfma.colsums_deferred():
+            want_gx = ctx.needs_input_grad[0]
+            nrows = _lib.load_library().rfn_dwconv3x3_bwd_partial_rows(B, H, W, C, ctx.dilation, DTYPE_CODE[x.dtype])
+            part = torch.empty(nrows * 10 * C, dtype=torch.float32, device=x.device)
+            gx = torch.empty_like(x) if want_gx else None
+            _lib.call("rfn_dwconv3x3_nhwc_bwd_partial", x.device, ptr(x), ptr(gy), ptr(w_tap) if want_gx else None, ptr(gx), ptr(part),
+                      B, H, W, C, ctx.dilation, DTYPE_CODE[x.dtype])
+            mfma.defer_colsum(mfma.COLSUM_DW, part, dw, db, C, nrows, 3)
+            return gx, None, None, None
         ws = workspace(_DW_WS_STRIPES * 10 * C * 4, x.device)
         tail = (ptr(dw), ptr(db), ptr(ws), B, H, W, C, ctx.dilation, DTYPE_CODE[x.dtype], 3 if direct else 0)
         if ctx.needs_input_grad[0]:
diff --git a/refign_amd/layernorm.py b/refign_amd/layernorm.py
--- a/refign_amd/layernorm.py
+++ b/refign_amd/layernorm.py
@@ -2,7 +2,7 @@
 import torch.nn as nn
 import torch.nn.functional as F
 
-from . import _lib
+from . import _lib, mfma
 from ._tensor import DTYPE_CODE, ptr, workspace
 from .params import as_dtype, grad_sink
 
@@ -54,6 +54,13 @@
         direct = sg is not None and sb is not None
         dg = sg if direct else torch.empty(C, dtype=torch.float32, device=x2.device)
         db = sb if direct else torch.empty(C, dtype=torch.float32, device=x2.device)
+        if direct and mfma.colsums_deferred() and (C % 8 == 0 or (gy_b is None and add is None)):
+            nrows = _lib.load_library().rfn_layernorm_bwd_partial_rows(rows, C)
+            part = torch.empty(nrows * 2 * C, dtype=torch.float32, device=x2.device)
+            _lib.call("rfn_layernorm_bwd_partial", x2.device, ptr(x2), ptr(gy2), ptr(gy_b), ptr(add), ptr(w32), ptr(mean), ptr(rstd),
+                      ptr(dx), ptr(part), rows, C, DTYPE_CODE[x2.dtype], DTYPE_CODE[gy2.dtype])
+            mfma.defer_colsum(mfma.COLSUM_LN, part, dg, db, C, nrows, 1)
+            return dx.view(ctx.shape), None, None, None, None
         ws = workspace(_LN_WS_ROWS * 2 * C * 4, x2.device)
         tail = (ptr(w32), ptr(mean), ptr(rstd), ptr(dx), ptr(dg), ptr(db), ptr(ws), rows, C, DTYPE_CODE[x2.dtype],
                 DTYPE_CODE[gy2.dtype], 1 if direct else 0)
diff --git a/refign_amd/mfma.py b/refign_amd/mfma.py
--- a/refign_amd/mfma.py
+++ b/refign_amd/mfma.py
@@ -230,54 +230,107 @@
     return True
 
 
+GROUP_COLSUMS = True
+COLSUM_LN, COLSUM_DW = 0, 1
+_COLSUM_QUEUE = None
+
+
+def defer_colsum(kind, ws, dst0, dst1, C, rows, flags):
+    q = _COLSUM_QUEUE
+    if q is None or not GROUP_COLSUMS or determinism.enabled():
+        return False
+    q.append((int(kind), ws, dst0, dst1, int(C), int(rows), int(flags)))
+    return True
+
+
+def colsums_deferred():
+    return _COLSUM_QUEUE is not None and GROUP_COLSUMS and not determinism.enabled()
+
+
+def _colsum_chunks(reds):
+    chunks = []
+    for r in reds:
+        if not chunks or len(chunks[-1]) >= _TN_GROUP_MAX or any(r[2].data_ptr() == o[2].data_ptr() for o in chunks[-1]):
+            chunks.append([])
+        chunks[-1].append(r)
+    return chunks
+
+
 def flush_wgrads():
-    q = _WGRAD_QUEUE
-    if not q:
+    q, cq = _WGRAD_QUEUE, _COLSUM_QUEUE
+    if not q and not cq:
         return
-    items, q[:] = list(q), []
+    items, reds = list(q or ()), list(cq or ())
+    if q:
+        q[:] = []
+    if cq:
+        cq[:] = []
     classes = {}
     for it in items:
         classes.setdefault((it[4] is not None, it[0].dtype, it[0].device), []).append(it)
-    vp, lg, it_ = ctypes.c_void_p, ctypes.c_long, ctypes.c_int
+    launches = []
     for (seg, dt, dev), lst in classes.items():
         for a in range(0, len(lst), _TN_GROUP_MAX):
-            grp = lst[a:a + _TN_GROUP_MAX]
-            n = len(grp)
-            arr = lambda ty, vals: (ty * n)(*vals)
-            G = arr(vp, [t[0].data_ptr() for t in grp])
-            X = arr(vp, [t[1].data_ptr() for t in grp])
-            P = arr(vp, [t[2].data_ptr() for t in grp])
-            Bv = arr(vp, [None if t[3] is None else t[3].data_ptr() for t in grp])
-            R = arr(vp, [None if t[4] is None else t[4].data_ptr() for t in grp])
-            T = arr(lg, [t[0].shape[0] for t in grp])
-            N = arr(lg, [t[0].shape[1] for t in grp])
-            K = arr(lg, [t[1].shape[1] for t in grp])
-            ldg = arr(lg, [t[0].stride(0) for t in grp])
-            ldx = arr(lg, [t[1].stride(0) for t in grp])
-            rps = arr(it_, [t[6] for t in grp])
-            rsa = arr(it_, [t[5] for t in grp])
-            cast = lambda a_: ctypes.cast(a_, vp)
-            _lib.call("rfn_gemm_tn_grouped", dev, n, cast(G), cast(X), cast(P), cast(Bv), cast(R), cast(T), cast(N), cast(K),
-                      cast(ldg), cast(ldx), cast(rps), cast(rsa), _DT16[dt])
+            launches.append([dev, dt, lst[a:a + _TN_GROUP_MAX], []])
+    by_dev = {}
+    for r in reds:
+        by_dev.setdefault(r[1].device, []).append(r)
+    for dev, lst in by_dev.items():
+        hosts = [l for l in launches if l[0] == dev]
+        for k, chunk in enumerate(_colsum_chunks(lst)):
+            if k < len(hosts):
+                hosts[k][3] = chunk
+            else:
+                launches.append([dev, torch.bfloat16, [], chunk])
+    vp, lg, it_ = ctypes.c_void_p, ctypes.c_long, ctypes.c_int
+    cast = lambda a_: None if a_ is None else ctypes.cast(a_, vp)
+    for dev, dt, grp, red in launches:
+        n, m = len(grp), len(red)
+        arr = lambda ty, vals: (ty * len(vals))(*vals) if vals else None
+        G = arr(vp, [t[0].data_ptr() for t in grp])
+        X = arr(vp, [t[1].data_ptr() for t in grp])
+        P = arr(vp, [t[2].data_ptr() for t in grp])
+        Bv = arr(vp, [None if t[3] is None else t[3].data_ptr() for t in grp])
+        R = arr(vp, [None if t[4] is None else t[4].data_ptr() for t in grp])
+        T = arr(lg, [t[0].shape[0] for t in grp])
+        N = arr(lg, [t[0].shape[1] for t in grp])
+        K = arr(lg, [t[1].shape[1] for t in grp])
+        ldg = arr(lg, [t[0].stride(0) for t in grp])
+        ldx = arr(lg, [t[1].stride(0) for t in grp])
+        rps = arr(it_, [t[6] for t in grp])
+        rsa = arr(it_, [t[5] for t in grp])
+        gemm = (n, cast(G), cast(X), cast(P), cast(Bv), cast(R), cast(T), cast(N), cast(K), cast(ldg), cast(ldx), cast(rps), cast(rsa))
+        if m == 0:
+            _lib.call("rfn_gemm_tn_grouped", dev, *gemm, _DT16[dt])
+            continue
+        kind = arr(it_, [r[0] for r in red])
+        ws = arr(vp, [r[1].data_ptr() for r in red])
+        d0 = arr(vp, [r[2].data_ptr() for r in red])
+        d1 = arr(vp, [None if r[3] is None else r[3].data_ptr() for r in red])
+        Cs = arr(it_, [r[4] for r in red])
+        rows = arr(it_, [r[5] for r in red])
+        flags = arr(it_, [r[6] for r in red])
+        _lib.call("rfn_gemm_tn_grouped_colsum", dev, *gemm, m, cast(kind), cast(ws), cast(d0), cast(d1), cast(Cs), cast(rows),
+                  cast(flags), _DT16[dt])
 
 
 class deferred_wgrads:
 
     def __enter__(self):
-        global _WGRAD_QUEUE
+        global _WGRAD_QUEUE, _COLSUM_QUEUE
         self._outer = _WGRAD_QUEUE
         if GROUP_WGRADS and ENABLED and self._outer is None:
-            _WGRAD_QUEUE = []
+            _WGRAD_QUEUE, _COLSUM_QUEUE = [], []
         return self
 
     def __exit__(self, *exc):
-        global _WGRAD_QUEUE
+        global _WGRAD_QUEUE, _COLSUM_QUEUE
         if self._outer is None and _WGRAD_QUEUE is not None:
             try:
                 if exc[0] is None:
                     flush_wgrads()
             finally:
-                _WGRAD_QUEUE = None
+                _WGRAD_QUEUE = _COLSUM_QUEUE = None
         return False
 
 
@@ -300,12 +353,16 @@
 _PACK_BLOCK = 4096
 
 
-def _pack(src, batch_stride, row_stride, B, heads, nrows, nblk, want_r=True, want_t=True, src2=None):
+def _pack(src, batch_stride, row_stride, B, heads, nrows, nblk, want_r=True, want_t=True, src2=None, zero=None):
     dev = src.device
     nbytes = B * heads * nblk * _PACK_BLOCK
     new = lambda want: torch.empty(nbytes, dtype=torch.uint8, device=dev) if want else None
     r, t = new(want_r), new(want_t)
     r2, t2 = (new(want_r), new(want_t)) if src2 is not None else (None, None)
+    if zero is not None:
+        _lib.call("rfn_attn_pack_zero", dev, ptr(src), batch_stride, row_stride, B, heads, nrows, nblk, ptr(r), ptr(t), ptr(src2),
+                  ptr(r2), ptr(t2), ptr(zero), zero.numel() * zero.element_size())
+        return (r, t), (r2, t2)
     _lib.call("rfn_attn_pack", dev, ptr(src), batch_stride, row_stride, B, heads, nrows, nblk, ptr(r), ptr(t), ptr(src2),
               ptr(r2), ptr(t2))
     return (r, t), (r2, t2)
@@ -373,15 +430,15 @@
         _lib.call("rfn_attn_bwd_dq", dev, ptr(q), q.stride(0), q.stride(1), ptr(do), ptr(o), o.stride(0), o.stride(1),
                   kvr.data_ptr(), kvr.data_ptr() + voff, kvt.data_ptr(), ptr(lse2), ptr(delta), ptr(dq), dq.stride(0),
                   dq.stride(1), B, heads, N, Nkv, nkblk, nqpad, float(scale), 2 * heads, dt)
-        (qr, qt), (gr, gt) = _pack(q, q.stride(0), q.stride(1), B, heads, N, nqblk, src2=do)
         nkpad = -(-Nkv // 32) * 32
         chunk = _chunk_blocks(nqblk, Nkv, B * heads)
         det = determinism.enabled()
         images = -(-nqblk // chunk) if det else 1
         accT = torch.empty(images * B * heads * 2 * 64 * nkpad, dtype=torch.float32, device=dev)
+        (qr, qt), (gr, gt) = _pack(q, q.stride(0), q.stride(1), B, heads, N, nqblk, src2=do, zero=None if det else accT)
         dkv = torch.empty_like(kv)
         k_view, v_view = kv[:, :, :C], kv[:, :, C:]
-        _lib.call("rfn_attn_bwd_dkv_det" if det else "rfn_attn_bwd_dkv", dev, ptr(k_view), ptr(v_view), kv.stride(0), kv.stride(1),
+        _lib.call("rfn_attn_bwd_dkv_det" if det else "rfn_attn_bwd_dkv_zeroed", dev, ptr(k_view), ptr(v_view), kv.stride(0), kv.stride(1),
                   ptr(qr), ptr(qt), ptr(gr), ptr(gt), ptr(lse2), ptr(delta), ptr(accT), ptr(dkv), B, heads, N, Nkv, nqblk, nqpad,
                   nkpad, chunk, float(scale), dt)
         return dq, dkv, None, None
diff --git a/refign_amd/seg.py b/refign_amd/seg.py
--- a/refign_amd/seg.py
+++ b/refign_amd/seg.py
@@ -45,6 +45,7 @@
 
     @staticmethod
     def backward(ctx, g):
+        mfma.flush_wgrads()
         cb = _GRAD_READY_CB
         if cb is not None:
             cb(ctx.tag)
```

Result: no change. 17.04, median of 6 (+0.7%).
